# Bioconductor/SparseArray

Hardware: AMD Instinct MI355X
Metric: GNZ/s, SVT crossprod(svt, dense) 1e6x1e4 @1% nnz (higher is better)
Workload: dtype f64

## Files before the change

### sparsearray_amd/csrc/kernels_mult_pbc.hip

```cpp
#include "svt_common.h"

#include <string.h>

#include <mutex>

#include "svt_scan.h"

typedef double d16 __attribute__((ext_vector_type(16)));
typedef double d8 __attribute__((ext_vector_type(8)));

struct svt_dev_pbc {
	int64_t nrow, ncol, nnz, nrec;
	int CBW, WPB, logR;
	int kind;
	int64_t ngroups, nblocks, npanels;
	uint4 *rec;
	int64_t *tile_ptr;
	int *col_has_na;
	int64_t max_leaf_nnz;
	mutable hipStream_t use_s[4];
	mutable int nuse;
	mutable bool use_overflow;
	int device;
};
// ... 997 lines not shown
		bl = Lr % nblocks; kh = u % kt; split = nfull + u / kt;
	}
	const int b = bl + block0;
	const int64_t pa = (int64_t) split * panels_per_split;
	const int64_t pb = pa + panels_per_split < npanels ? pa + panels_per_split : npanels;
	if (pa >= pb)
		return;
	const int k0 = kh * 64;
	const int64_t wv = (int64_t) b * 16 + w;
	const int64_t *__restrict__ tb = tile_ptr + (wv * npanels + pa);

	d16 acc[NV > 2 ? 2 : NV];
	d8 acc8 = 0.0;
#pragma unroll
	for (int i = 0; i < (NV > 2 ? 2 : NV); i++) acc[i] = 0.0;
	const bool partial = (nrow & 127) != 0;

	const int wd = w;
	u32x4 PA;
	u32x16 PB;
	{
		const uint64_t recp = (uint64_t) (uintptr_t) rec + (uint64_t) tb[0] * 12u;
		PA[0] = (uint32_t) recp; PA[1] = (uint32_t) (recp >> 32);
		PA[2] = 0;
		PA[3] = (uint32_t) pa;
		PB[0] = (uint32_t) pb;
		PB[1] = PBC_DMA_BUF;
		PB[2] = (uint32_t) (wd * 4 * PBC_DMA_ROW + PBC_DMA_BUF);
		PB[3] = (uint32_t) (w >> 2);
		PB[4] = partial ? (uint32_t) (npanels - 1) : 0xFFFFFFFFu;
		PB[5] = partial ? (uint32_t) ((128 - (nrow & 127)) * 8) : 0u;
		PB[6] = 0;
		{
			const int chunk = (8192 + nblocks - 1) / nblocks;
			PB[7] = (uint32_t) ((chunk + 1023) / 1024 - 1);
		}
#pragma unroll
		for (int q = 0; q < 4; q++) {
			int kk = k0 + wd * 4 + q;
			if (kk > K - 1) kk = K - 1;
			const uint64_t src = (uint64_t) (uintptr_t) (Y + (int64_t) kk * ldY + pa * 128);
			PB[8 + 2 * q] = (uint32_t) src; PB[9 + 2 * q] = (uint32_t) (src >> 32);
		}
	}
	u32x16 V0 = 0, V1 = 0;
	u32x4 V2 = 0;
	{
		const int lane = tid & 63;
		V0[0] = (uint32_t) lane * PBC_DMA_ROW;
		V0[1] = (uint32_t) lane * 16u;
		V0[2] = (uint32_t) (lane < rt_lines ? lane : rt_lines - 1) * 128u + (uint32_t) rt_ahead;
		V0[11] = (uint32_t) lane * 16u + 1024u;
		const int chunk = (8192 + nblocks - 1) / nblocks;
		const int nit = (chunk + 1023) / 1024;
		int e0 = bl * chunk;
		if (e0 > 8192 - nit * 1024) e0 = 8192 - nit * 1024;
		const int e = e0 + tid;
		V0[3] = (uint32_t) ((e >> 7) * PBC_DMA_ROW + (e & 127) * 8);
		V0[7] = lane == 0 ? (uint32_t) nit :
			lane == 1 ? (partial ? (uint32_t) (npanels - 1) : 0xFFFFFFFFu) :
				    (partial ? (uint32_t) ((128 - (nrow & 127)) * 8) : 0u);
	}
	{
		const int lane = tid & 63;
		const bool clampme = partial && pa == npanels - 1;
#pragma unroll
		for (int q = 0; q < 4; q++) {
			int kk = k0 + wd * 4 + q;
			if (kk > K - 1) kk = K - 1;
			const int64_t r0 = clampme ? nrow - 128 : pa * 128;
			const double *src = Y + (int64_t) kk * ldY + r0 + lane * 2;
			double *dst = ylds + (wd * 4 + q) * 129;
			__builtin_amdgcn_global_load_lds((const __attribute__((address_space(1))) void *) src,
							 (__attribute__((address_space(3))) void *) dst, 16, 0, 0);
		}
		{
			uint32_t sink;
			const char *ptr = (const char *) rec + tb[0] * 12 + (int64_t) (lane < 32 ? lane : 31) * 128;
			asm volatile("global_load_dword %0, %1, off\n\ts_waitcnt vmcnt(0)"
				     : "=v"(sink) : "v"(ptr) : "memory");
		}
	}
#ifdef SVT_TUNING
	if (PROF) t_loop = __builtin_readcyclecounter();
#endif
#if PBC_DMA_YSETS == 2
	u32x8 V3 = 0;
#define PBC_DMA_STATE "+{v[0:15]}"(V0), "+{v[16:31]}"(V1), "+{v[32:39]}"(V3), "+{v[40:43]}"(V2), "+{s[8:11]}"(PA), "+{s[12:27]}"(PB)
#define PBC_ACC0 "+{v[44:75]}"
#define PBC_ACC1 "+{v[76:107]}"
#define PBC_ACC2 "+{v[108:123]}"
// ... 871 lines not shown
```

### sparsearray_amd/csrc/pbc_dma_asm.inc

```
#define PBC_DMA_ROW 1032
#define PBC_DMA_BUF 66048
#define PBC_DMA_BATCH_BYTES 96
#define PBC_DMA_YSETS 2
#define PBC_DMA_ASM_TEXT \
	"v_mov_b32 v10, 0x207\n\t" \
	"s_load_dwordx8 s[28:35], s[8:9], s10\n\t" \
	"s_load_dwordx16 s[36:51], s[8:9], s10 offset:32\n\t" \
	"s_load_dwordx8 s[52:59], s[8:9], s10 offset:96\n\t" \
	"s_load_dwordx16 s[60:75], s[8:9], s10 offset:128\n\t" \
	"s_add_u32 s10, s10, 192\n\t" \
	"s_waitcnt lgkmcnt(0)\n\t" \
	"s_branch 55f\n\t" \
	"20:\n" \
	"s_load_dwordx8 s[76:83], s[8:9], s10\n\t" \
	"s_load_dwordx16 s[84:99], s[8:9], s10 offset:32\n\t" \
	"s_and_b32 vcc_lo, s28, 0xc000\n\t" \
	"s_cbranch_scc1 70f\n\t" \
	"v_add_u32_sdwa v28, s52, v4 dst_sel:DWORD dst_unused:UNUSED_PAD src0_sel:WORD_1 src1_sel:DWORD\n\t" \
	"v_add_u32_sdwa v30, s53, v4 dst_sel:DWORD dst_unused:UNUSED_PAD src0_sel:WORD_1 src1_sel:DWORD\n\t" \
	"v_add_u32_sdwa v32, s54, v4 dst_sel:DWORD dst_unused:UNUSED_PAD src0_sel:WORD_1 src1_sel:DWORD\n\t" \
	"v_add_u32_sdwa v34, s55, v4 dst_sel:DWORD dst_unused:UNUSED_PAD src0_sel:WORD_1 src1_sel:DWORD\n\t" \
	"v_add_u32_sdwa v36, s56, v4 dst_sel:DWORD dst_unused:UNUSED_PAD src0_sel:WORD_1 src1_sel:DWORD\n\t" \
	"v_add_u32_sdwa v38, s57, v4 dst_sel:DWORD dst_unused:UNUSED_PAD src0_sel:WORD_1 src1_sel:DWORD\n\t" \
	"v_add_u32_sdwa v40, s58, v4 dst_sel:DWORD dst_unused:UNUSED_PAD src0_sel:WORD_1 src1_sel:DWORD\n\t" \
	"v_add_u32_sdwa v42, s59, v4 dst_sel:DWORD dst_unused:UNUSED_PAD src0_sel:WORD_1 src1_sel:DWORD\n\t" \
	"ds_read_b64 v[28:29], v28\n\t" \
	"ds_read_b64 v[30:31], v30\n\t" \
	"ds_read_b64 v[32:33], v32\n\t" \
	"ds_read_b64 v[34:35], v34\n\t" \
	"ds_read_b64 v[36:37], v36\n\t" \
	"ds_read_b64 v[38:39], v38\n\t" \
	"ds_read_b64 v[40:41], v40\n\t" \
	"ds_read_b64 v[42:43], v42\n\t" \
	"s_set_gpr_idx_on s28, gpr_idx(SRC2,DST)\n\t" \
	"v_fma_f64 v[44:45], s[36:37], v[12:13], v[44:45]\n\t" \
	"s_set_gpr_idx_idx s29\n\t" \
// ... 225 lines not shown
	"ds_read_b64 v[32:33], v32\n\t" \
	"ds_read_b64 v[34:35], v34\n\t" \
	"ds_read_b64 v[36:37], v36\n\t" \
	"ds_read_b64 v[38:39], v38\n\t" \
	"ds_read_b64 v[40:41], v40\n\t" \
	"ds_read_b64 v[42:43], v42\n\t" \
	"s_set_gpr_idx_on s28, gpr_idx(SRC2,DST)\n\t" \
	"v_fma_f64 v[44:45], s[36:37], v[12:13], v[44:45]\n\t" \
	"s_set_gpr_idx_idx s29\n\t" \
	"v_fma_f64 v[44:45], s[38:39], v[14:15], v[44:45]\n\t" \
	"s_set_gpr_idx_idx s30\n\t" \
	"v_fma_f64 v[44:45], s[40:41], v[16:17], v[44:45]\n\t" \
	"s_set_gpr_idx_idx s31\n\t" \
	"v_fma_f64 v[44:45], s[42:43], v[18:19], v[44:45]\n\t" \
	"s_set_gpr_idx_idx s32\n\t" \
	"v_fma_f64 v[44:45], s[44:45], v[20:21], v[44:45]\n\t" \
	"s_set_gpr_idx_idx s33\n\t" \
	"v_fma_f64 v[44:45], s[46:47], v[22:23], v[44:45]\n\t" \
	"s_set_gpr_idx_idx s34\n\t" \
	"v_fma_f64 v[44:45], s[48:49], v[24:25], v[44:45]\n\t" \
	"s_set_gpr_idx_idx s35\n\t" \
	"v_fma_f64 v[44:45], s[50:51], v[26:27], v[44:45]\n\t" \
	"s_set_gpr_idx_off\n\t" \
	"s_waitcnt lgkmcnt(0)\n\t" \
	"s_cmp_ge_u32 s11, s12\n\t" \
	"s_cbranch_scc1 61f\n\t" \
	"s_cmp_lg_u32 s11, s16\n\t" \
	"s_cbranch_scc1 15f\n\t" \
	"v_subrev_u32 v11, s17, v11\n\t" \
	"15:\n" \
	"s_sub_u32 m0, s14, s13\n\t" \
	"s_nop 0\n\t" \
	"global_load_lds_dwordx4 v11, s[20:21]\n\t" \
	"s_add_u32 m0, m0, 1032\n\t" \
	"s_nop 0\n\t" \
	"global_load_lds_dwordx4 v11, s[22:23]\n\t" \
	"s_add_u32 m0, m0, 1032\n\t" \
	"s_nop 0\n\t" \
	"global_load_lds_dwordx4 v11, s[24:25]\n\t" \
	"s_add_u32 m0, m0, 1032\n\t" \
	"s_nop 0\n\t" \
	"global_load_lds_dwordx4 v11, s[26:27]\n\t" \
	"s_nop 1\n\t" \
	"v_add_u32 v11, 1024, v11\n\t" \
	"v_add_u32 v6, s10, v2\n\t" \
	"global_load_dword v5, v6, s[8:9]\n\t" \
	"61:\n" \
	"s_branch 21b\n\t" \
	"80:\n" \
	"s_bitcmp1_b32 s28, 14\n\t" \
	"s_cbranch_scc0 30f\n\t" \
	"s_cmp_ge_u32 s11, s12\n\t" \
	"s_cbranch_scc1 61f\n\t" \
	"s_cmp_lg_u32 s11, s16\n\t" \
	"s_cbranch_scc1 15f\n\t" \
	"v_subrev_u32 v11, s17, v11\n\t" \
	"15:\n" \
	"s_sub_u32 m0, s14, s13\n\t" \
	"s_nop 0\n\t" \
	"global_load_lds_dwordx4 v11, s[20:21]\n\t" \
	"s_add_u32 m0, m0, 1032\n\t" \
	"s_nop 0\n\t" \
	"global_load_lds_dwordx4 v11, s[22:23]\n\t" \
	"s_add_u32 m0, m0, 1032\n\t" \
	"s_nop 0\n\t" \
	"global_load_lds_dwordx4 v11, s[24:25]\n\t" \
	"s_add_u32 m0, m0, 1032\n\t" \
	"s_nop 0\n\t" \
	"global_load_lds_dwordx4 v11, s[26:27]\n\t" \
	"s_nop 1\n\t" \
	"v_add_u32 v11, 1024, v11\n\t" \
	"v_add_u32 v6, s10, v2\n\t" \
	"global_load_dword v5, v6, s[8:9]\n\t" \
	"61:\n" \
	"s_branch 30f\n\t" \
	"71:\n" \
	"s_bitcmp1_b32 s52, 15\n\t" \
	"s_cbranch_scc1 81f\n\t" \
	"v_add_u32_sdwa v12, s76, v4 dst_sel:DWORD dst_unused:UNUSED_PAD src0_sel:WORD_1 src1_sel:DWORD\n\t" \
	"v_add_u32_sdwa v14, s77, v4 dst_sel:DWORD dst_unused:UNUSED_PAD src0_sel:WORD_1 src1_sel:DWORD\n\t" \
	"v_add_u32_sdwa v16, s78, v4 dst_sel:DWORD dst_unused:UNUSED_PAD src0_sel:WORD_1 src1_sel:DWORD\n\t" \
	"v_add_u32_sdwa v18, s79, v4 dst_sel:DWORD dst_unused:UNUSED_PAD src0_sel:WORD_1 src1_sel:DWORD\n\t" \
	"v_add_u32_sdwa v20, s80, v4 dst_sel:DWORD dst_unused:UNUSED_PAD src0_sel:WORD_1 src1_sel:DWORD\n\t" \
	"v_add_u32_sdwa v22, s81, v4 dst_sel:DWORD dst_unused:UNUSED_PAD src0_sel:WORD_1 src1_sel:DWORD\n\t" \
	"v_add_u32_sdwa v24, s82, v4 dst_sel:DWORD dst_unused:UNUSED_PAD src0_sel:WORD_1 src1_sel:DWORD\n\t" \
	"v_add_u32_sdwa v26, s83, v4 dst_sel:DWORD dst_unused:UNUSED_PAD src0_sel:WORD_1 src1_sel:DWORD\n\t" \
	"ds_read_b64 v[12:13], v12\n\t" \
	"ds_read_b64 v[14:15], v14\n\t" \
	"ds_read_b64 v[16:17], v16\n\t" \
	"ds_read_b64 v[18:19], v18\n\t" \
	"ds_read_b64 v[20:21], v20\n\t" \
	"ds_read_b64 v[22:23], v22\n\t" \
	"ds_read_b64 v[24:25], v24\n\t" \
	"ds_read_b64 v[26:27], v26\n\t" \
	"s_set_gpr_idx_on s52, gpr_idx(SRC2,DST)\n\t" \
	"v_fma_f64 v[44:45], s[60:61], v[28:29], v[44:45]\n\t" \
	"s_set_gpr_idx_idx s53\n\t" \
	"v_fma_f64 v[44:45], s[62:63], v[30:31], v[44:45]\n\t" \
	"s_set_gpr_idx_idx s54\n\t" \
	"v_fma_f64 v[44:45], s[64:65], v[32:33], v[44:45]\n\t" \
	"s_set_gpr_idx_idx s55\n\t" \
	"v_fma_f64 v[44:45], s[66:67], v[34:35], v[44:45]\n\t" \
	"s_set_gpr_idx_idx s56\n\t" \
	"v_fma_f64 v[44:45], s[68:69], v[36:37], v[44:45]\n\t" \
	"s_set_gpr_idx_idx s57\n\t" \
	"v_fma_f64 v[44:45], s[70:71], v[38:39], v[44:45]\n\t" \
	"s_set_gpr_idx_idx s58\n\t" \
	"v_fma_f64 v[44:45], s[72:73], v[40:41], v[44:45]\n\t" \
	"s_set_gpr_idx_idx s59\n\t" \
	"v_fma_f64 v[44:45], s[74:75], v[42:43], v[44:45]\n\t" \
	"s_set_gpr_idx_off\n\t" \
	"s_waitcnt lgkmcnt(0)\n\t" \
	"s_cmp_ge_u32 s11, s12\n\t" \
	"s_cbranch_scc1 61f\n\t" \
	"s_cmp_lg_u32 s11, s16\n\t" \
	"s_cbranch_scc1 15f\n\t" \
	"v_subrev_u32 v11, s17, v11\n\t" \
	"15:\n" \
	"s_sub_u32 m0, s14, s13\n\t" \
	"s_nop 0\n\t" \
	"global_load_lds_dwordx4 v11, s[20:21]\n\t" \
	"s_add_u32 m0, m0, 1032\n\t" \
	"s_nop 0\n\t" \
	"global_load_lds_dwordx4 v11, s[22:23]\n\t" \
	"s_add_u32 m0, m0, 1032\n\t" \
	"s_nop 0\n\t" \
	"global_load_lds_dwordx4 v11, s[24:25]\n\t" \
	"s_add_u32 m0, m0, 1032\n\t" \
	"s_nop 0\n\t" \
	"global_load_lds_dwordx4 v11, s[26:27]\n\t" \
	"s_nop 1\n\t" \
	"v_add_u32 v11, 1024, v11\n\t" \
	"v_add_u32 v6, s10, v2\n\t" \
	"global_load_dword v5, v6, s[8:9]\n\t" \
	"61:\n" \
	"s_branch 22b\n\t" \
	"81:\n" \
	"s_bitcmp1_b32 s52, 14\n\t" \
	"s_cbranch_scc0 31f\n\t" \
	"s_cmp_ge_u32 s11, s12\n\t" \
	"s_cbranch_scc1 61f\n\t" \
	"s_cmp_lg_u32 s11, s16\n\t" \
	"s_cbranch_scc1 15f\n\t" \
	"v_subrev_u32 v11, s17, v11\n\t" \
	"15:\n" \
	"s_sub_u32 m0, s14, s13\n\t" \
	"s_nop 0\n\t" \
	"global_load_lds_dwordx4 v11, s[20:21]\n\t" \
	"s_add_u32 m0, m0, 1032\n\t" \
	"s_nop 0\n\t" \
	"global_load_lds_dwordx4 v11, s[22:23]\n\t" \
	"s_add_u32 m0, m0, 1032\n\t" \
	"s_nop 0\n\t" \
	"global_load_lds_dwordx4 v11, s[24:25]\n\t" \
	"s_add_u32 m0, m0, 1032\n\t" \
	"s_nop 0\n\t" \
	"global_load_lds_dwordx4 v11, s[26:27]\n\t" \
	"s_nop 1\n\t" \
	"v_add_u32 v11, 1024, v11\n\t" \
	"v_add_u32 v6, s10, v2\n\t" \
	"global_load_dword v5, v6, s[8:9]\n\t" \
	"61:\n" \
	"s_branch 31f\n\t" \
	"72:\n" \
	"s_bitcmp1_b32 s76, 15\n\t" \
	"s_cbranch_scc1 82f\n\t" \
	"v_add_u32_sdwa v28, s28, v4 dst_sel:DWORD dst_unused:UNUSED_PAD src0_sel:WORD_1 src1_sel:DWORD\n\t" \
	"v_add_u32_sdwa v30, s29, v4 dst_sel:DWORD dst_unused:UNUSED_PAD src0_sel:WORD_1 src1_sel:DWORD\n\t" \
	"v_add_u32_sdwa v32, s30, v4 dst_sel:DWORD dst_unused:UNUSED_PAD src0_sel:WORD_1 src1_sel:DWORD\n\t" \
	"v_add_u32_sdwa v34, s31, v4 dst_sel:DWORD dst_unused:UNUSED_PAD src0_sel:WORD_1 src1_sel:DWORD\n\t" \
	"v_add_u32_sdwa v36, s32, v4 dst_sel:DWORD dst_unused:UNUSED_PAD src0_sel:WORD_1 src1_sel:DWORD\n\t" \
	"v_add_u32_sdwa v38, s33, v4 dst_sel:DWORD dst_unused:UNUSED_PAD src0_sel:WORD_1 src1_sel:DWORD\n\t" \
	"v_add_u32_sdwa v40, s34, v4 dst_sel:DWORD dst_unused:UNUSED_PAD src0_sel:WORD_1 src1_sel:DWORD\n\t" \
	"v_add_u32_sdwa v42, s35, v4 dst_sel:DWORD dst_unused:UNUSED_PAD src0_sel:WORD_1 src1_sel:DWORD\n\t" \
	"ds_read_b64 v[28:29], v28\n\t" \
	"ds_read_b64 v[30:31], v30\n\t" \
	"ds_read_b64 v[32:33], v32\n\t" \
	"ds_read_b64 v[34:35], v34\n\t" \
	"ds_read_b64 v[36:37], v36\n\t" \
	"ds_read_b64 v[38:39], v38\n\t" \
	"ds_read_b64 v[40:41], v40\n\t" \
	"ds_read_b64 v[42:43], v42\n\t" \
	"s_set_gpr_idx_on s76, gpr_idx(SRC2,DST)\n\t" \
	"v_fma_f64 v[44:45], s[84:85], v[12:13], v[44:45]\n\t" \
	"s_set_gpr_idx_idx s77\n\t" \
	"v_fma_f64 v[44:45], s[86:87], v[14:15], v[44:45]\n\t" \
	"s_set_gpr_idx_idx s78\n\t" \
	"v_fma_f64 v[44:45], s[88:89], v[16:17], v[44:45]\n\t" \
	"s_set_gpr_idx_idx s79\n\t" \
	"v_fma_f64 v[44:45], s[90:91], v[18:19], v[44:45]\n\t" \
	"s_set_gpr_idx_idx s80\n\t" \
	"v_fma_f64 v[44:45], s[92:93], v[20:21], v[44:45]\n\t" \
	"s_set_gpr_idx_idx s81\n\t" \
	"v_fma_f64 v[44:45], s[94:95], v[22:23], v[44:45]\n\t" \
	"s_set_gpr_idx_idx s82\n\t" \
	"v_fma_f64 v[44:45], s[96:97], v[24:25], v[44:45]\n\t" \
	"s_set_gpr_idx_idx s83\n\t" \
	"v_fma_f64 v[44:45], s[98:99], v[26:27], v[44:45]\n\t" \
	"s_set_gpr_idx_off\n\t" \
	"s_waitcnt lgkmcnt(0)\n\t" \
	"s_cmp_ge_u32 s11, s12\n\t" \
	"s_cbranch_scc1 61f\n\t" \
	"s_cmp_lg_u32 s11, s16\n\t" \
	"s_cbranch_scc1 15f\n\t" \
	"v_subrev_u32 v11, s17, v11\n\t" \
	"15:\n" \
	"s_sub_u32 m0, s14, s13\n\t" \
	"s_nop 0\n\t" \
	"global_load_lds_dwordx4 v11, s[20:21]\n\t" \
	"s_add_u32 m0, m0, 1032\n\t" \
	"s_nop 0\n\t" \
	"global_load_lds_dwordx4 v11, s[22:23]\n\t" \
	"s_add_u32 m0, m0, 1032\n\t" \
	"s_nop 0\n\t" \
	"global_load_lds_dwordx4 v11, s[24:25]\n\t" \
	"s_add_u32 m0, m0, 1032\n\t" \
	"s_nop 0\n\t" \
	"global_load_lds_dwordx4 v11, s[26:27]\n\t" \
	"s_nop 1\n\t" \
	"v_add_u32 v11, 1024, v11\n\t" \
	"v_add_u32 v6, s10, v2\n\t" \
	"global_load_dword v5, v6, s[8:9]\n\t" \
	"61:\n" \
	"s_branch 23b\n\t" \
	"82:\n" \
	"s_bitcmp1_b32 s76, 14\n\t" \
	"s_cbranch_scc0 32f\n\t" \
	"s_cmp_ge_u32 s11, s12\n\t" \
	"s_cbranch_scc1 61f\n\t" \
	"s_cmp_lg_u32 s11, s16\n\t" \
	"s_cbranch_scc1 15f\n\t" \
	"v_subrev_u32 v11, s17, v11\n\t" \
	"15:\n" \
	"s_sub_u32 m0, s14, s13\n\t" \
	"s_nop 0\n\t" \
	"global_load_lds_dwordx4 v11, s[20:21]\n\t" \
	"s_add_u32 m0, m0, 1032\n\t" \
	"s_nop 0\n\t" \
	"global_load_lds_dwordx4 v11, s[22:23]\n\t" \
	"s_add_u32 m0, m0, 1032\n\t" \
	"s_nop 0\n\t" \
	"global_load_lds_dwordx4 v11, s[24:25]\n\t" \
	"s_add_u32 m0, m0, 1032\n\t" \
	"s_nop 0\n\t" \
	"global_load_lds_dwordx4 v11, s[26:27]\n\t" \
	"s_nop 1\n\t" \
	"v_add_u32 v11, 1024, v11\n\t" \
	"v_add_u32 v6, s10, v2\n\t" \
	"global_load_dword v5, v6, s[8:9]\n\t" \
	"61:\n" \
	"s_branch 32f\n\t" \
	"73:\n" \
	"s_bitcmp1_b32 s28, 15\n\t" \
	"s_cbranch_scc1 83f\n\t" \
	"v_add_u32_sdwa v12, s52, v4 dst_sel:DWORD dst_unused:UNUSED_PAD src0_sel:WORD_1 src1_sel:DWORD\n\t" \
	"v_add_u32_sdwa v14, s53, v4 dst_sel:DWORD dst_unused:UNUSED_PAD src0_sel:WORD_1 src1_sel:DWORD\n\t" \
	"v_add_u32_sdwa v16, s54, v4 dst_sel:DWORD dst_unused:UNUSED_PAD src0_sel:WORD_1 src1_sel:DWORD\n\t" \
	"v_add_u32_sdwa v18, s55, v4 dst_sel:DWORD dst_unused:UNUSED_PAD src0_sel:WORD_1 src1_sel:DWORD\n\t" \
	"v_add_u32_sdwa v20, s56, v4 dst_sel:DWORD dst_unused:UNUSED_PAD src0_sel:WORD_1 src1_sel:DWORD\n\t" \
	"v_add_u32_sdwa v22, s57, v4 dst_sel:DWORD dst_unused:UNUSED_PAD src0_sel:WORD_1 src1_sel:DWORD\n\t" \
	"v_add_u32_sdwa v24, s58, v4 dst_sel:DWORD dst_unused:UNUSED_PAD src0_sel:WORD_1 src1_sel:DWORD\n\t" \
	"v_add_u32_sdwa v26, s59, v4 dst_sel:DWORD dst_unused:UNUSED_PAD src0_sel:WORD_1 src1_sel:DWORD\n\t" \
	"ds_read_b64 v[12:13], v12\n\t" \
	"ds_read_b64 v[14:15], v14\n\t" \
	"ds_read_b64 v[16:17], v16\n\t" \
	"ds_read_b64 v[18:19], v18\n\t" \
	"ds_read_b64 v[20:21], v20\n\t" \
	"ds_read_b64 v[22:23], v22\n\t" \
	"ds_read_b64 v[24:25], v24\n\t" \
	"ds_read_b64 v[26:27], v26\n\t" \
	"s_set_gpr_idx_on s28, gpr_idx(SRC2,DST)\n\t" \
	"v_fma_f64 v[44:45], s[36:37], v[28:29], v[44:45]\n\t" \
	"s_set_gpr_idx_idx s29\n\t" \
	"v_fma_f64 v[44:45], s[38:39], v[30:31], v[44:45]\n\t" \
	"s_set_gpr_idx_idx s30\n\t" \
	"v_fma_f64 v[44:45], s[40:41], v[32:33], v[44:45]\n\t" \
	"s_set_gpr_idx_idx s31\n\t" \
	"v_fma_f64 v[44:45], s[42:43], v[34:35], v[44:45]\n\t" \
	"s_set_gpr_idx_idx s32\n\t" \
	"v_fma_f64 v[44:45], s[44:45], v[36:37], v[44:45]\n\t" \
	"s_set_gpr_idx_idx s33\n\t" \
	"v_fma_f64 v[44:45], s[46:47], v[38:39], v[44:45]\n\t" \
	"s_set_gpr_idx_idx s34\n\t" \
	"v_fma_f64 v[44:45], s[48:49], v[40:41], v[44:45]\n\t" \
	"s_set_gpr_idx_idx s35\n\t" \
	"v_fma_f64 v[44:45], s[50:51], v[42:43], v[44:45]\n\t" \
	"s_set_gpr_idx_off\n\t" \
	"s_waitcnt lgkmcnt(0)\n\t" \
	"s_cmp_ge_u32 s11, s12\n\t" \
	"s_cbranch_scc1 61f\n\t" \
	"s_cmp_lg_u32 s11, s16\n\t" \
	"s_cbranch_scc1 15f\n\t" \
	"v_subrev_u32 v11, s17, v11\n\t" \
	"15:\n" \
	"s_sub_u32 m0, s14, s13\n\t" \
	"s_nop 0\n\t" \
	"global_load_lds_dwordx4 v11, s[20:21]\n\t" \
	"s_add_u32 m0, m0, 1032\n\t" \
	"s_nop 0\n\t" \
	"global_load_lds_dwordx4 v11, s[22:23]\n\t" \
	"s_add_u32 m0, m0, 1032\n\t" \
	"s_nop 0\n\t" \
	"global_load_lds_dwordx4 v11, s[24:25]\n\t" \
	"s_add_u32 m0, m0, 1032\n\t" \
	"s_nop 0\n\t" \
	"global_load_lds_dwordx4 v11, s[26:27]\n\t" \
	"s_nop 1\n\t" \
	"v_add_u32 v11, 1024, v11\n\t" \
	"v_add_u32 v6, s10, v2\n\t" \
	"global_load_dword v5, v6, s[8:9]\n\t" \
	"61:\n" \
	"s_branch 24b\n\t" \
	"83:\n" \
	"s_bitcmp1_b32 s28, 14\n\t" \
	"s_cbranch_scc0 33f\n\t" \
	"s_cmp_ge_u32 s11, s12\n\t" \
	"s_cbranch_scc1 61f\n\t" \
	"s_cmp_lg_u32 s11, s16\n\t" \
	"s_cbranch_scc1 15f\n\t" \
	"v_subrev_u32 v11, s17, v11\n\t" \
	"15:\n" \
	"s_sub_u32 m0, s14, s13\n\t" \
	"s_nop 0\n\t" \
	"global_load_lds_dwordx4 v11, s[20:21]\n\t" \
	"s_add_u32 m0, m0, 1032\n\t" \
	"s_nop 0\n\t" \
	"global_load_lds_dwordx4 v11, s[22:23]\n\t" \
	"s_add_u32 m0, m0, 1032\n\t" \
	"s_nop 0\n\t" \
	"global_load_lds_dwordx4 v11, s[24:25]\n\t" \
	"s_add_u32 m0, m0, 1032\n\t" \
	"s_nop 0\n\t" \
	"global_load_lds_dwordx4 v11, s[26:27]\n\t" \
	"s_nop 1\n\t" \
	"v_add_u32 v11, 1024, v11\n\t" \
	"v_add_u32 v6, s10, v2\n\t" \
	"global_load_dword v5, v6, s[8:9]\n\t" \
	"61:\n" \
	"s_branch 33f\n\t" \
	"74:\n" \
	"s_bitcmp1_b32 s52, 15\n\t" \
	"s_cbranch_scc1 84f\n\t" \
	"v_add_u32_sdwa v28, s76, v4 dst_sel:DWORD dst_unused:UNUSED_PAD src0_sel:WORD_1 src1_sel:DWORD\n\t" \
	"v_add_u32_sdwa v30, s77, v4 dst_sel:DWORD dst_unused:UNUSED_PAD src0_sel:WORD_1 src1_sel:DWORD\n\t" \
	"v_add_u32_sdwa v32, s78, v4 dst_sel:DWORD dst_unused:UNUSED_PAD src0_sel:WORD_1 src1_sel:DWORD\n\t" \
	"v_add_u32_sdwa v34, s79, v4 dst_sel:DWORD dst_unused:UNUSED_PAD src0_sel:WORD_1 src1_sel:DWORD\n\t" \
	"v_add_u32_sdwa v36, s80, v4 dst_sel:DWORD dst_unused:UNUSED_PAD src0_sel:WORD_1 src1_sel:DWORD\n\t" \
	"v_add_u32_sdwa v38, s81, v4 dst_sel:DWORD dst_unused:UNUSED_PAD src0_sel:WORD_1 src1_sel:DWORD\n\t" \
	"v_add_u32_sdwa v40, s82, v4 dst_sel:DWORD dst_unused:UNUSED_PAD src0_sel:WORD_1 src1_sel:DWORD\n\t" \
	"v_add_u32_sdwa v42, s83, v4 dst_sel:DWORD dst_unused:UNUSED_PAD src0_sel:WORD_1 src1_sel:DWORD\n\t" \
	"ds_read_b64 v[28:29], v28\n\t" \
	"ds_read_b64 v[30:31], v30\n\t" \
	"ds_read_b64 v[32:33], v32\n\t" \
	"ds_read_b64 v[34:35], v34\n\t" \
	"ds_read_b64 v[36:37], v36\n\t" \
	"ds_read_b64 v[38:39], v38\n\t" \
	"ds_read_b64 v[40:41], v40\n\t" \
	"ds_read_b64 v[42:43], v42\n\t" \
	"s_set_gpr_idx_on s52, gpr_idx(SRC2,DST)\n\t" \
	"v_fma_f64 v[44:45], s[60:61], v[12:13], v[44:45]\n\t" \
	"s_set_gpr_idx_idx s53\n\t" \
	"v_fma_f64 v[44:45], s[62:63], v[14:15], v[44:45]\n\t" \
	"s_set_gpr_idx_idx s54\n\t" \
	"v_fma_f64 v[44:45], s[64:65], v[16:17], v[44:45]\n\t" \
	"s_set_gpr_idx_idx s55\n\t" \
	"v_fma_f64 v[44:45], s[66:67], v[18:19], v[44:45]\n\t" \
	"s_set_gpr_idx_idx s56\n\t" \
	"v_fma_f64 v[44:45], s[68:69], v[20:21], v[44:45]\n\t" \
	"s_set_gpr_idx_idx s57\n\t" \
	"v_fma_f64 v[44:45], s[70:71], v[22:23], v[44:45]\n\t" \
	"s_set_gpr_idx_idx s58\n\t" \
	"v_fma_f64 v[44:45], s[72:73], v[24:25], v[44:45]\n\t" \
	"s_set_gpr_idx_idx s59\n\t" \
	"v_fma_f64 v[44:45], s[74:75], v[26:27], v[44:45]\n\t" \
	"s_set_gpr_idx_off\n\t" \
	"s_waitcnt lgkmcnt(0)\n\t" \
	"s_cmp_ge_u32 s11, s12\n\t" \
	"s_cbranch_scc1 61f\n\t" \
	"s_cmp_lg_u32 s11, s16\n\t" \
	"s_cbranch_scc1 15f\n\t" \
	"v_subrev_u32 v11, s17, v11\n\t" \
	"15:\n" \
	"s_sub_u32 m0, s14, s13\n\t" \
	"s_nop 0\n\t" \
	"global_load_lds_dwordx4 v11, s[20:21]\n\t" \
	"s_add_u32 m0, m0, 1032\n\t" \
	"s_nop 0\n\t" \
	"global_load_lds_dwordx4 v11, s[22:23]\n\t" \
	"s_add_u32 m0, m0, 1032\n\t" \
	"s_nop 0\n\t" \
	"global_load_lds_dwordx4 v11, s[24:25]\n\t" \
	"s_add_u32 m0, m0, 1032\n\t" \
	"s_nop 0\n\t" \
	"global_load_lds_dwordx4 v11, s[26:27]\n\t" \
	"s_nop 1\n\t" \
	"v_add_u32 v11, 1024, v11\n\t" \
	"v_add_u32 v6, s10, v2\n\t" \
	"global_load_dword v5, v6, s[8:9]\n\t" \
	"61:\n" \
	"s_branch 25b\n\t" \
	"84:\n" \
	"s_bitcmp1_b32 s52, 14\n\t" \
	"s_cbranch_scc0 34f\n\t" \
	"s_cmp_ge_u32 s11, s12\n\t" \
	"s_cbranch_scc1 61f\n\t" \
	"s_cmp_lg_u32 s11, s16\n\t" \
	"s_cbranch_scc1 15f\n\t" \
	"v_subrev_u32 v11, s17, v11\n\t" \
	"15:\n" \
	"s_sub_u32 m0, s14, s13\n\t" \
	"s_nop 0\n\t" \
	"global_load_lds_dwordx4 v11, s[20:21]\n\t" \
	"s_add_u32 m0, m0, 1032\n\t" \
	"s_nop 0\n\t" \
	"global_load_lds_dwordx4 v11, s[22:23]\n\t" \
	"s_add_u32 m0, m0, 1032\n\t" \
	"s_nop 0\n\t" \
	"global_load_lds_dwordx4 v11, s[24:25]\n\t" \
	"s_add_u32 m0, m0, 1032\n\t" \
	"s_nop 0\n\t" \
	"global_load_lds_dwordx4 v11, s[26:27]\n\t" \
	"s_nop 1\n\t" \
	"v_add_u32 v11, 1024, v11\n\t" \
	"v_add_u32 v6, s10, v2\n\t" \
	"global_load_dword v5, v6, s[8:9]\n\t" \
	"61:\n" \
	"s_branch 34f\n\t" \
	"75:\n" \
	"s_bitcmp1_b32 s76, 15\n\t" \
	"s_cbranch_scc1 85f\n\t" \
	"v_add_u32_sdwa v12, s28, v4 dst_sel:DWORD dst_unused:UNUSED_PAD src0_sel:WORD_1 src1_sel:DWORD\n\t" \
	"v_add_u32_sdwa v14, s29, v4 dst_sel:DWORD dst_unused:UNUSED_PAD src0_sel:WORD_1 src1_sel:DWORD\n\t" \
	"v_add_u32_sdwa v16, s30, v4 dst_sel:DWORD dst_unused:UNUSED_PAD src0_sel:WORD_1 src1_sel:DWORD\n\t" \
	"v_add_u32_sdwa v18, s31, v4 dst_sel:DWORD dst_unused:UNUSED_PAD src0_sel:WORD_1 src1_sel:DWORD\n\t" \
	"v_add_u32_sdwa v20, s32, v4 dst_sel:DWORD dst_unused:UNUSED_PAD src0_sel:WORD_1 src1_sel:DWORD\n\t" \
	"v_add_u32_sdwa v22, s33, v4 dst_sel:DWORD dst_unused:UNUSED_PAD src0_sel:WORD_1 src1_sel:DWORD\n\t" \
	"v_add_u32_sdwa v24, s34, v4 dst_sel:DWORD dst_unused:UNUSED_PAD src0_sel:WORD_1 src1_sel:DWORD\n\t" \
	"v_add_u32_sdwa v26, s35, v4 dst_sel:DWORD dst_unused:UNUSED_PAD src0_sel:WORD_1 src1_sel:DWORD\n\t" \
	"ds_read_b64 v[12:13], v12\n\t" \
	"ds_read_b64 v[14:15], v14\n\t" \
	"ds_read_b64 v[16:17], v16\n\t" \
	"ds_read_b64 v[18:19], v18\n\t" \
	"ds_read_b64 v[20:21], v20\n\t" \
	"ds_read_b64 v[22:23], v22\n\t" \
	"ds_read_b64 v[24:25], v24\n\t" \
	"ds_read_b64 v[26:27], v26\n\t" \
	"s_set_gpr_idx_on s76, gpr_idx(SRC2,DST)\n\t" \
	"v_fma_f64 v[44:45], s[84:85], v[28:29], v[44:45]\n\t" \
	"s_set_gpr_idx_idx s77\n\t" \
	"v_fma_f64 v[44:45], s[86:87], v[30:31], v[44:45]\n\t" \
	"s_set_gpr_idx_idx s78\n\t" \
	"v_fma_f64 v[44:45], s[88:89], v[32:33], v[44:45]\n\t" \
	"s_set_gpr_idx_idx s79\n\t" \
	"v_fma_f64 v[44:45], s[90:91], v[34:35], v[44:45]\n\t" \
	"s_set_gpr_idx_idx s80\n\t" \
	"v_fma_f64 v[44:45], s[92:93], v[36:37], v[44:45]\n\t" \
	"s_set_gpr_idx_idx s81\n\t" \
	"v_fma_f64 v[44:45], s[94:95], v[38:39], v[44:45]\n\t" \
	"s_set_gpr_idx_idx s82\n\t" \
	"v_fma_f64 v[44:45], s[96:97], v[40:41], v[44:45]\n\t" \
	"s_set_gpr_idx_idx s83\n\t" \
	"v_fma_f64 v[44:45], s[98:99], v[42:43], v[44:45]\n\t" \
	"s_set_gpr_idx_off\n\t" \
	"s_waitcnt lgkmcnt(0)\n\t" \
	"s_cmp_ge_u32 s11, s12\n\t" \
	"s_cbranch_scc1 61f\n\t" \
	"s_cmp_lg_u32 s11, s16\n\t" \
	"s_cbranch_scc1 15f\n\t" \
	"v_subrev_u32 v11, s17, v11\n\t" \
	"15:\n" \
	"s_sub_u32 m0, s14, s13\n\t" \
	"s_nop 0\n\t" \
	"global_load_lds_dwordx4 v11, s[20:21]\n\t" \
	"s_add_u32 m0, m0, 1032\n\t" \
	"s_nop 0\n\t" \
	"global_load_lds_dwordx4 v11, s[22:23]\n\t" \
	"s_add_u32 m0, m0, 1032\n\t" \
	"s_nop 0\n\t" \
	"global_load_lds_dwordx4 v11, s[24:25]\n\t" \
	"s_add_u32 m0, m0, 1032\n\t" \
	"s_nop 0\n\t" \
	"global_load_lds_dwordx4 v11, s[26:27]\n\t" \
	"s_nop 1\n\t" \
	"v_add_u32 v11, 1024, v11\n\t" \
	"v_add_u32 v6, s10, v2\n\t" \
	"global_load_dword v5, v6, s[8:9]\n\t" \
	"61:\n" \
	"s_branch 20b\n\t" \
	"85:\n" \
	"s_bitcmp1_b32 s76, 14\n\t" \
	"s_cbranch_scc0 35f\n\t" \
	"s_cmp_ge_u32 s11, s12\n\t" \
	"s_cbranch_scc1 61f\n\t" \
	"s_cmp_lg_u32 s11, s16\n\t" \
	"s_cbranch_scc1 15f\n\t" \
	"v_subrev_u32 v11, s17, v11\n\t" \
	"15:\n" \
	"s_sub_u32 m0, s14, s13\n\t" \
	"s_nop 0\n\t" \
	"global_load_lds_dwordx4 v11, s[20:21]\n\t" \
	"s_add_u32 m0, m0, 1032\n\t" \
	"s_nop 0\n\t" \
	"global_load_lds_dwordx4 v11, s[22:23]\n\t" \
	"s_add_u32 m0, m0, 1032\n\t" \
	"s_nop 0\n\t" \
	"global_load_lds_dwordx4 v11, s[24:25]\n\t" \
	"s_add_u32 m0, m0, 1032\n\t" \
	"s_nop 0\n\t" \
	"global_load_lds_dwordx4 v11, s[26:27]\n\t" \
	"s_nop 1\n\t" \
	"v_add_u32 v11, 1024, v11\n\t" \
	"v_add_u32 v6, s10, v2\n\t" \
	"global_load_dword v5, v6, s[8:9]\n\t" \
	"61:\n" \
	"s_branch 35f\n\t" \
	"30:\n" \
	"s_cmp_ge_u32 s11, s12\n\t" \
	"s_cbranch_scc1 40f\n\t" \
	"s_xor_b32 s13, s13, 66048\n\t" \
	"v_add_u32 v4, s13, v0\n\t" \
	"s_cmp_lg_u32 s11, s16\n\t" \
	"s_cbranch_scc1 16f\n\t" \
	"v_add_u32 v4, s17, v4\n\t" \
	"16:\n" \
	"s_add_u32 s11, s11, 1\n\t" \
	"v_add_u32 v6, s13, v3\n\t" \
	"v_add_u32_sdwa v28, s52, v4 dst_sel:DWORD dst_unused:UNUSED_PAD src0_sel:WORD_1 src1_sel:DWORD\n\t" \
	"v_add_u32_sdwa v30, s53, v4 dst_sel:DWORD dst_unused:UNUSED_PAD src0_sel:WORD_1 src1_sel:DWORD\n\t" \
	"v_add_u32_sdwa v32, s54, v4 dst_sel:DWORD dst_unused:UNUSED_PAD src0_sel:WORD_1 src1_sel:DWORD\n\t" \
	"v_add_u32_sdwa v34, s55, v4 dst_sel:DWORD dst_unused:UNUSED_PAD src0_sel:WORD_1 src1_sel:DWORD\n\t" \
	"v_add_u32_sdwa v36, s56, v4 dst_sel:DWORD dst_unused:UNUSED_PAD src0_sel:WORD_1 src1_sel:DWORD\n\t" \
	"v_add_u32_sdwa v38, s57, v4 dst_sel:DWORD dst_unused:UNUSED_PAD src0_sel:WORD_1 src1_sel:DWORD\n\t" \
	"v_add_u32_sdwa v40, s58, v4 dst_sel:DWORD dst_unused:UNUSED_PAD src0_sel:WORD_1 src1_sel:DWORD\n\t" \
	"v_add_u32_sdwa v42, s59, v4 dst_sel:DWORD dst_unused:UNUSED_PAD src0_sel:WORD_1 src1_sel:DWORD\n\t" \
	"s_waitcnt vmcnt(1)\n\t" \
	"s_barrier\n\t" \
	"ds_read_b64 v[28:29], v28\n\t" \
	"ds_read_b64 v[30:31], v30\n\t" \
	"ds_read_b64 v[32:33], v32\n\t" \
	"ds_read_b64 v[34:35], v34\n\t" \
	"ds_read_b64 v[36:37], v36\n\t" \
	"ds_read_b64 v[38:39], v38\n\t" \
	"ds_read_b64 v[40:41], v40\n\t" \
	"ds_read_b64 v[42:43], v42\n\t" \
	"s_set_gpr_idx_on s28, gpr_idx(SRC2,DST)\n\t" \
	"v_fma_f64 v[44:45], s[36:37], v[12:13], v[44:45]\n\t" \
	"s_set_gpr_idx_idx s29\n\t" \
	"v_fma_f64 v[44:45], s[38:39], v[14:15], v[44:45]\n\t" \
	"s_set_gpr_idx_idx s30\n\t" \
	"v_fma_f64 v[44:45], s[40:41], v[16:17], v[44:45]\n\t" \
	"s_set_gpr_idx_idx s31\n\t" \
	"v_fma_f64 v[44:45], s[42:43], v[18:19], v[44:45]\n\t" \
	"s_set_gpr_idx_idx s32\n\t" \
	"v_fma_f64 v[44:45], s[44:45], v[20:21], v[44:45]\n\t" \
	"s_set_gpr_idx_idx s33\n\t" \
	"v_fma_f64 v[44:45], s[46:47], v[22:23], v[44:45]\n\t" \
	"s_set_gpr_idx_idx s34\n\t" \
	"v_fma_f64 v[44:45], s[48:49], v[24:25], v[44:45]\n\t" \
	"s_set_gpr_idx_idx s35\n\t" \
	"v_fma_f64 v[44:45], s[50:51], v[26:27], v[44:45]\n\t" \
	"s_set_gpr_idx_off\n\t" \
	"s_mov_b32 m0, s19\n\t" \
	"12:\n" \
	"ds_read_b64 v[8:9], v6\n\t" \
	"v_add_u32 v6, 8256, v6\n\t" \
	"s_waitcnt lgkmcnt(0)\n\t" \
	"v_cmp_class_f64 vcc, v[8:9], v10\n\t" \
	"s_or_b32 s18, s18, vcc_lo\n\t" \
	"s_or_b32 s18, s18, vcc_hi\n\t" \
	"s_sub_u32 m0, m0, 1\n\t" \
	"s_cbranch_scc0 12b\n\t" \
	"s_branch 21b\n\t" \
	"31:\n" \
	"s_cmp_ge_u32 s11, s12\n\t" \
	"s_cbranch_scc1 41f\n\t" \
	"s_xor_b32 s13, s13, 66048\n\t" \
	"v_add_u32 v4, s13, v0\n\t" \
	"s_cmp_lg_u32 s11, s16\n\t" \
	"s_cbranch_scc1 16f\n\t" \
	"v_add_u32 v4, s17, v4\n\t" \
	"16:\n" \
	"s_add_u32 s11, s11, 1\n\t" \
	"v_add_u32 v6, s13, v3\n\t" \
	"v_add_u32_sdwa v12, s76, v4 dst_sel:DWORD dst_unused:UNUSED_PAD src0_sel:WORD_1 src1_sel:DWORD\n\t" \
	"v_add_u32_sdwa v14, s77, v4 dst_sel:DWORD dst_unused:UNUSED_PAD src0_sel:WORD_1 src1_sel:DWORD\n\t" \
	"v_add_u32_sdwa v16, s78, v4 dst_sel:DWORD dst_unused:UNUSED_PAD src0_sel:WORD_1 src1_sel:DWORD\n\t" \
	"v_add_u32_sdwa v18, s79, v4 dst_sel:DWORD dst_unused:UNUSED_PAD src0_sel:WORD_1 src1_sel:DWORD\n\t" \
	"v_add_u32_sdwa v20, s80, v4 dst_sel:DWORD dst_unused:UNUSED_PAD src0_sel:WORD_1 src1_sel:DWORD\n\t" \
	"v_add_u32_sdwa v22, s81, v4 dst_sel:DWORD dst_unused:UNUSED_PAD src0_sel:WORD_1 src1_sel:DWORD\n\t" \
	"v_add_u32_sdwa v24, s82, v4 dst_sel:DWORD dst_unused:UNUSED_PAD src0_sel:WORD_1 src1_sel:DWORD\n\t" \
	"v_add_u32_sdwa v26, s83, v4 dst_sel:DWORD dst_unused:UNUSED_PAD src0_sel:WORD_1 src1_sel:DWORD\n\t" \
	"s_waitcnt vmcnt(1)\n\t" \
	"s_barrier\n\t" \
	"ds_read_b64 v[12:13], v12\n\t" \
	"ds_read_b64 v[14:15], v14\n\t" \
	"ds_read_b64 v[16:17], v16\n\t" \
	"ds_read_b64 v[18:19], v18\n\t" \
	"ds_read_b64 v[20:21], v20\n\t" \
	"ds_read_b64 v[22:23], v22\n\t" \
	"ds_read_b64 v[24:25], v24\n\t" \
	"ds_read_b64 v[26:27], v26\n\t" \
	"s_set_gpr_idx_on s52, gpr_idx(SRC2,DST)\n\t" \
	"v_fma_f64 v[44:45], s[60:61], v[28:29], v[44:45]\n\t" \
	"s_set_gpr_idx_idx s53\n\t" \
	"v_fma_f64 v[44:45], s[62:63], v[30:31], v[44:45]\n\t" \
	"s_set_gpr_idx_idx s54\n\t" \
	"v_fma_f64 v[44:45], s[64:65], v[32:33], v[44:45]\n\t" \
	"s_set_gpr_idx_idx s55\n\t" \
	"v_fma_f64 v[44:45], s[66:67], v[34:35], v[44:45]\n\t" \
	"s_set_gpr_idx_idx s56\n\t" \
	"v_fma_f64 v[44:45], s[68:69], v[36:37], v[44:45]\n\t" \
	"s_set_gpr_idx_idx s57\n\t" \
	"v_fma_f64 v[44:45], s[70:71], v[38:39], v[44:45]\n\t" \
	"s_set_gpr_idx_idx s58\n\t" \
	"v_fma_f64 v[44:45], s[72:73], v[40:41], v[44:45]\n\t" \
	"s_set_gpr_idx_idx s59\n\t" \
	"v_fma_f64 v[44:45], s[74:75], v[42:43], v[44:45]\n\t" \
	"s_set_gpr_idx_off\n\t" \
	"s_mov_b32 m0, s19\n\t" \
	"12:\n" \
	"ds_read_b64 v[8:9], v6\n\t" \
	"v_add_u32 v6, 8256, v6\n\t" \
	"s_waitcnt lgkmcnt(0)\n\t" \
	"v_cmp_class_f64 vcc, v[8:9], v10\n\t" \
	"s_or_b32 s18, s18, vcc_lo\n\t" \
	"s_or_b32 s18, s18, vcc_hi\n\t" \
	"s_sub_u32 m0, m0, 1\n\t" \
	"s_cbranch_scc0 12b\n\t" \
	"s_branch 22b\n\t" \
	"32:\n" \
	"s_cmp_ge_u32 s11, s12\n\t" \
	"s_cbranch_scc1 42f\n\t" \
	"s_xor_b32 s13, s13, 66048\n\t" \
	"v_add_u32 v4, s13, v0\n\t" \
	"s_cmp_lg_u32 s11, s16\n\t" \
	"s_cbranch_scc1 16f\n\t" \
	"v_add_u32 v4, s17, v4\n\t" \
	"16:\n" \
	"s_add_u32 s11, s11, 1\n\t" \
	"v_add_u32 v6, s13, v3\n\t" \
	"v_add_u32_sdwa v28, s28, v4 dst_sel:DWORD dst_unused:UNUSED_PAD src0_sel:WORD_1 src1_sel:DWORD\n\t" \
	"v_add_u32_sdwa v30, s29, v4 dst_sel:DWORD dst_unused:UNUSED_PAD src0_sel:WORD_1 src1_sel:DWORD\n\t" \
	"v_add_u32_sdwa v32, s30, v4 dst_sel:DWORD dst_unused:UNUSED_PAD src0_sel:WORD_1 src1_sel:DWORD\n\t" \
	"v_add_u32_sdwa v34, s31, v4 dst_sel:DWORD dst_unused:UNUSED_PAD src0_sel:WORD_1 src1_sel:DWORD\n\t" \
	"v_add_u32_sdwa v36, s32, v4 dst_sel:DWORD dst_unused:UNUSED_PAD src0_sel:WORD_1 src1_sel:DWORD\n\t" \
	"v_add_u32_sdwa v38, s33, v4 dst_sel:DWORD dst_unused:UNUSED_PAD src0_sel:WORD_1 src1_sel:DWORD\n\t" \
	"v_add_u32_sdwa v40, s34, v4 dst_sel:DWORD dst_unused:UNUSED_PAD src0_sel:WORD_1 src1_sel:DWORD\n\t" \
	"v_add_u32_sdwa v42, s35, v4 dst_sel:DWORD dst_unused:UNUSED_PAD src0_sel:WORD_1 src1_sel:DWORD\n\t" \
	"s_waitcnt vmcnt(1)\n\t" \
	"s_barrier\n\t" \
	"ds_read_b64 v[28:29], v28\n\t" \
	"ds_read_b64 v[30:31], v30\n\t" \
	"ds_read_b64 v[32:33], v32\n\t" \
	"ds_read_b64 v[34:35], v34\n\t" \
	"ds_read_b64 v[36:37], v36\n\t" \
	"ds_read_b64 v[38:39], v38\n\t" \
	"ds_read_b64 v[40:41], v40\n\t" \
	"ds_read_b64 v[42:43], v42\n\t" \
	"s_set_gpr_idx_on s76, gpr_idx(SRC2,DST)\n\t" \
	"v_fma_f64 v[44:45], s[84:85], v[12:13], v[44:45]\n\t" \
	"s_set_gpr_idx_idx s77\n\t" \
	"v_fma_f64 v[44:45], s[86:87], v[14:15], v[44:45]\n\t" \
	"s_set_gpr_idx_idx s78\n\t" \
	"v_fma_f64 v[44:45], s[88:89], v[16:17], v[44:45]\n\t" \
	"s_set_gpr_idx_idx s79\n\t" \
	"v_fma_f64 v[44:45], s[90:91], v[18:19], v[44:45]\n\t" \
	"s_set_gpr_idx_idx s80\n\t" \
	"v_fma_f64 v[44:45], s[92:93], v[20:21], v[44:45]\n\t" \
	"s_set_gpr_idx_idx s81\n\t" \
	"v_fma_f64 v[44:45], s[94:95], v[22:23], v[44:45]\n\t" \
	"s_set_gpr_idx_idx s82\n\t" \
	"v_fma_f64 v[44:45], s[96:97], v[24:25], v[44:45]\n\t" \
	"s_set_gpr_idx_idx s83\n\t" \
	"v_fma_f64 v[44:45], s[98:99], v[26:27], v[44:45]\n\t" \
	"s_set_gpr_idx_off\n\t" \
	"s_mov_b32 m0, s19\n\t" \
	"12:\n" \
	"ds_read_b64 v[8:9], v6\n\t" \
	"v_add_u32 v6, 8256, v6\n\t" \
	"s_waitcnt lgkmcnt(0)\n\t" \
	"v_cmp_class_f64 vcc, v[8:9], v10\n\t" \
	"s_or_b32 s18, s18, vcc_lo\n\t" \
	"s_or_b32 s18, s18, vcc_hi\n\t" \
	"s_sub_u32 m0, m0, 1\n\t" \
	"s_cbranch_scc0 12b\n\t" \
	"s_branch 23b\n\t" \
	"33:\n" \
	"s_cmp_ge_u32 s11, s12\n\t" \
	"s_cbranch_scc1 43f\n\t" \
	"s_xor_b32 s13, s13, 66048\n\t" \
	"v_add_u32 v4, s13, v0\n\t" \
	"s_cmp_lg_u32 s11, s16\n\t" \
	"s_cbranch_scc1 16f\n\t" \
	"v_add_u32 v4, s17, v4\n\t" \
	"16:\n" \
	"s_add_u32 s11, s11, 1\n\t" \
	"v_add_u32 v6, s13, v3\n\t" \
	"v_add_u32_sdwa v12, s52, v4 dst_sel:DWORD dst_unused:UNUSED_PAD src0_sel:WORD_1 src1_sel:DWORD\n\t" \
	"v_add_u32_sdwa v14, s53, v4 dst_sel:DWORD dst_unused:UNUSED_PAD src0_sel:WORD_1 src1_sel:DWORD\n\t" \
	"v_add_u32_sdwa v16, s54, v4 dst_sel:DWORD dst_unused:UNUSED_PAD src0_sel:WORD_1 src1_sel:DWORD\n\t" \
	"v_add_u32_sdwa v18, s55, v4 dst_sel:DWORD dst_unused:UNUSED_PAD src0_sel:WORD_1 src1_sel:DWORD\n\t" \
	"v_add_u32_sdwa v20, s56, v4 dst_sel:DWORD dst_unused:UNUSED_PAD src0_sel:WORD_1 src1_sel:DWORD\n\t" \
	"v_add_u32_sdwa v22, s57, v4 dst_sel:DWORD dst_unused:UNUSED_PAD src0_sel:WORD_1 src1_sel:DWORD\n\t" \
	"v_add_u32_sdwa v24, s58, v4 dst_sel:DWORD dst_unused:UNUSED_PAD src0_sel:WORD_1 src1_sel:DWORD\n\t" \
	"v_add_u32_sdwa v26, s59, v4 dst_sel:DWORD dst_unused:UNUSED_PAD src0_sel:WORD_1 src1_sel:DWORD\n\t" \
	"s_waitcnt vmcnt(1)\n\t" \
	"s_barrier\n\t" \
	"ds_read_b64 v[12:13], v12\n\t" \
	"ds_read_b64 v[14:15], v14\n\t" \
	"ds_read_b64 v[16:17], v16\n\t" \
	"ds_read_b64 v[18:19], v18\n\t" \
	"ds_read_b64 v[20:21], v20\n\t" \
	"ds_read_b64 v[22:23], v22\n\t" \
	"ds_read_b64 v[24:25], v24\n\t" \
	"ds_read_b64 v[26:27], v26\n\t" \
	"s_set_gpr_idx_on s28, gpr_idx(SRC2,DST)\n\t" \
	"v_fma_f64 v[44:45], s[36:37], v[28:29], v[44:45]\n\t" \
	"s_set_gpr_idx_idx s29\n\t" \
	"v_fma_f64 v[44:45], s[38:39], v[30:31], v[44:45]\n\t" \
	"s_set_gpr_idx_idx s30\n\t" \
	"v_fma_f64 v[44:45], s[40:41], v[32:33], v[44:45]\n\t" \
	"s_set_gpr_idx_idx s31\n\t" \
	"v_fma_f64 v[44:45], s[42:43], v[34:35], v[44:45]\n\t" \
	"s_set_gpr_idx_idx s32\n\t" \
	"v_fma_f64 v[44:45], s[44:45], v[36:37], v[44:45]\n\t" \
	"s_set_gpr_idx_idx s33\n\t" \
	"v_fma_f64 v[44:45], s[46:47], v[38:39], v[44:45]\n\t" \
	"s_set_gpr_idx_idx s34\n\t" \
	"v_fma_f64 v[44:45], s[48:49], v[40:41], v[44:45]\n\t" \
	"s_set_gpr_idx_idx s35\n\t" \
	"v_fma_f64 v[44:45], s[50:51], v[42:43], v[44:45]\n\t" \
	"s_set_gpr_idx_off\n\t" \
	"s_mov_b32 m0, s19\n\t" \
	"12:\n" \
	"ds_read_b64 v[8:9], v6\n\t" \
	"v_add_u32 v6, 8256, v6\n\t" \
	"s_waitcnt lgkmcnt(0)\n\t" \
	"v_cmp_class_f64 vcc, v[8:9], v10\n\t" \
	"s_or_b32 s18, s18, vcc_lo\n\t" \
	"s_or_b32 s18, s18, vcc_hi\n\t" \
	"s_sub_u32 m0, m0, 1\n\t" \
	"s_cbranch_scc0 12b\n\t" \
	"s_branch 24b\n\t" \
	"34:\n" \
	"s_cmp_ge_u32 s11, s12\n\t" \
	"s_cbranch_scc1 44f\n\t" \
	"s_xor_b32 s13, s13, 66048\n\t" \
	"v_add_u32 v4, s13, v0\n\t" \
	"s_cmp_lg_u32 s11, s16\n\t" \
	"s_cbranch_scc1 16f\n\t" \
	"v_add_u32 v4, s17, v4\n\t" \
	"16:\n" \
	"s_add_u32 s11, s11, 1\n\t" \
	"v_add_u32 v6, s13, v3\n\t" \
	"v_add_u32_sdwa v28, s76, v4 dst_sel:DWORD dst_unused:UNUSED_PAD src0_sel:WORD_1 src1_sel:DWORD\n\t" \
	"v_add_u32_sdwa v30, s77, v4 dst_sel:DWORD dst_unused:UNUSED_PAD src0_sel:WORD_1 src1_sel:DWORD\n\t" \
	"v_add_u32_sdwa v32, s78, v4 dst_sel:DWORD dst_unused:UNUSED_PAD src0_sel:WORD_1 src1_sel:DWORD\n\t" \
	"v_add_u32_sdwa v34, s79, v4 dst_sel:DWORD dst_unused:UNUSED_PAD src0_sel:WORD_1 src1_sel:DWORD\n\t" \
	"v_add_u32_sdwa v36, s80, v4 dst_sel:DWORD dst_unused:UNUSED_PAD src0_sel:WORD_1 src1_sel:DWORD\n\t" \
	"v_add_u32_sdwa v38, s81, v4 dst_sel:DWORD dst_unused:UNUSED_PAD src0_sel:WORD_1 src1_sel:DWORD\n\t" \
	"v_add_u32_sdwa v40, s82, v4 dst_sel:DWORD dst_unused:UNUSED_PAD src0_sel:WORD_1 src1_sel:DWORD\n\t" \
	"v_add_u32_sdwa v42, s83, v4 dst_sel:DWORD dst_unused:UNUSED_PAD src0_sel:WORD_1 src1_sel:DWORD\n\t" \
	"s_waitcnt vmcnt(1)\n\t" \
	"s_barrier\n\t" \
	"ds_read_b64 v[28:29], v28\n\t" \
	"ds_read_b64 v[30:31], v30\n\t" \
	"ds_read_b64 v[32:33], v32\n\t" \
	"ds_read_b64 v[34:35], v34\n\t" \
	"ds_read_b64 v[36:37], v36\n\t" \
	"ds_read_b64 v[38:39], v38\n\t" \
	"ds_read_b64 v[40:41], v40\n\t" \
	"ds_read_b64 v[42:43], v42\n\t" \
	"s_set_gpr_idx_on s52, gpr_idx(SRC2,DST)\n\t" \
	"v_fma_f64 v[44:45], s[60:61], v[12:13], v[44:45]\n\t" \
	"s_set_gpr_idx_idx s53\n\t" \
	"v_fma_f64 v[44:45], s[62:63], v[14:15], v[44:45]\n\t" \
	"s_set_gpr_idx_idx s54\n\t" \
	"v_fma_f64 v[44:45], s[64:65], v[16:17], v[44:45]\n\t" \
	"s_set_gpr_idx_idx s55\n\t" \
	"v_fma_f64 v[44:45], s[66:67], v[18:19], v[44:45]\n\t" \
	"s_set_gpr_idx_idx s56\n\t" \
	"v_fma_f64 v[44:45], s[68:69], v[20:21], v[44:45]\n\t" \
	"s_set_gpr_idx_idx s57\n\t" \
	"v_fma_f64 v[44:45], s[70:71], v[22:23], v[44:45]\n\t" \
	"s_set_gpr_idx_idx s58\n\t" \
	"v_fma_f64 v[44:45], s[72:73], v[24:25], v[44:45]\n\t" \
	"s_set_gpr_idx_idx s59\n\t" \
	"v_fma_f64 v[44:45], s[74:75], v[26:27], v[44:45]\n\t" \
	"s_set_gpr_idx_off\n\t" \
	"s_mov_b32 m0, s19\n\t" \
	"12:\n" \
	"ds_read_b64 v[8:9], v6\n\t" \
	"v_add_u32 v6, 8256, v6\n\t" \
	"s_waitcnt lgkmcnt(0)\n\t" \
	"v_cmp_class_f64 vcc, v[8:9], v10\n\t" \
	"s_or_b32 s18, s18, vcc_lo\n\t" \
	"s_or_b32 s18, s18, vcc_hi\n\t" \
	"s_sub_u32 m0, m0, 1\n\t" \
	"s_cbranch_scc0 12b\n\t" \
	"s_branch 25b\n\t" \
	"35:\n" \
	"s_cmp_ge_u32 s11, s12\n\t" \
	"s_cbranch_scc1 45f\n\t" \
	"s_xor_b32 s13, s13, 66048\n\t" \
	"v_add_u32 v4, s13, v0\n\t" \
	"s_cmp_lg_u32 s11, s16\n\t" \
	"s_cbranch_scc1 16f\n\t" \
	"v_add_u32 v4, s17, v4\n\t" \
	"16:\n" \
	"s_add_u32 s11, s11, 1\n\t" \
	"v_add_u32 v6, s13, v3\n\t" \
	"v_add_u32_sdwa v12, s28, v4 dst_sel:DWORD dst_unused:UNUSED_PAD src0_sel:WORD_1 src1_sel:DWORD\n\t" \
	"v_add_u32_sdwa v14, s29, v4 dst_sel:DWORD dst_unused:UNUSED_PAD src0_sel:WORD_1 src1_sel:DWORD\n\t" \
	"v_add_u32_sdwa v16, s30, v4 dst_sel:DWORD dst_unused:UNUSED_PAD src0_sel:WORD_1 src1_sel:DWORD\n\t" \
	"v_add_u32_sdwa v18, s31, v4 dst_sel:DWORD dst_unused:UNUSED_PAD src0_sel:WORD_1 src1_sel:DWORD\n\t" \
	"v_add_u32_sdwa v20, s32, v4 dst_sel:DWORD dst_unused:UNUSED_PAD src0_sel:WORD_1 src1_sel:DWORD\n\t" \
	"v_add_u32_sdwa v22, s33, v4 dst_sel:DWORD dst_unused:UNUSED_PAD src0_sel:WORD_1 src1_sel:DWORD\n\t" \
	"v_add_u32_sdwa v24, s34, v4 dst_sel:DWORD dst_unused:UNUSED_PAD src0_sel:WORD_1 src1_sel:DWORD\n\t" \
	"v_add_u32_sdwa v26, s35, v4 dst_sel:DWORD dst_unused:UNUSED_PAD src0_sel:WORD_1 src1_sel:DWORD\n\t" \
	"s_waitcnt vmcnt(1)\n\t" \
	"s_barrier\n\t" \
	"ds_read_b64 v[12:13], v12\n\t" \
	"ds_read_b64 v[14:15], v14\n\t" \
	"ds_read_b64 v[16:17], v16\n\t" \
	"ds_read_b64 v[18:19], v18\n\t" \
	"ds_read_b64 v[20:21], v20\n\t" \
	"ds_read_b64 v[22:23], v22\n\t" \
	"ds_read_b64 v[24:25], v24\n\t" \
	"ds_read_b64 v[26:27], v26\n\t" \
	"s_set_gpr_idx_on s76, gpr_idx(SRC2,DST)\n\t" \
	"v_fma_f64 v[44:45], s[84:85], v[28:29], v[44:45]\n\t" \
	"s_set_gpr_idx_idx s77\n\t" \
	"v_fma_f64 v[44:45], s[86:87], v[30:31], v[44:45]\n\t" \
	"s_set_gpr_idx_idx s78\n\t" \
	"v_fma_f64 v[44:45], s[88:89], v[32:33], v[44:45]\n\t" \
	"s_set_gpr_idx_idx s79\n\t" \
	"v_fma_f64 v[44:45], s[90:91], v[34:35], v[44:45]\n\t" \
	"s_set_gpr_idx_idx s80\n\t" \
	"v_fma_f64 v[44:45], s[92:93], v[36:37], v[44:45]\n\t" \
	"s_set_gpr_idx_idx s81\n\t" \
	"v_fma_f64 v[44:45], s[94:95], v[38:39], v[44:45]\n\t" \
	"s_set_gpr_idx_idx s82\n\t" \
	"v_fma_f64 v[44:45], s[96:97], v[40:41], v[44:45]\n\t" \
	"s_set_gpr_idx_idx s83\n\t" \
	"v_fma_f64 v[44:45], s[98:99], v[42:43], v[44:45]\n\t" \
	"s_set_gpr_idx_off\n\t" \
	"s_mov_b32 m0, s19\n\t" \
	"12:\n" \
	"ds_read_b64 v[8:9], v6\n\t" \
	"v_add_u32 v6, 8256, v6\n\t" \
	"s_waitcnt lgkmcnt(0)\n\t" \
	"v_cmp_class_f64 vcc, v[8:9], v10\n\t" \
	"s_or_b32 s18, s18, vcc_lo\n\t" \
	"s_or_b32 s18, s18, vcc_hi\n\t" \
	"s_sub_u32 m0, m0, 1\n\t" \
	"s_cbranch_scc0 12b\n\t" \
	"s_branch 20b\n\t" \
	"55:\n" \
	"s_cmp_ge_u32 s11, s12\n\t" \
	"s_cbranch_scc1 90f\n\t" \
	"s_xor_b32 s13, s13, 66048\n\t" \
	"v_add_u32 v4, s13, v0\n\t" \
	"s_cmp_lg_u32 s11, s16\n\t" \
	"s_cbranch_scc1 16f\n\t" \
	"v_add_u32 v4, s17, v4\n\t" \
	"16:\n" \
	"s_add_u32 s11, s11, 1\n\t" \
	"v_add_u32 v6, s13, v3\n\t" \
	"v_add_u32_sdwa v12, s28, v4 dst_sel:DWORD dst_unused:UNUSED_PAD src0_sel:WORD_1 src1_sel:DWORD\n\t" \
	"v_add_u32_sdwa v14, s29, v4 dst_sel:DWORD dst_unused:UNUSED_PAD src0_sel:WORD_1 src1_sel:DWORD\n\t" \
	"v_add_u32_sdwa v16, s30, v4 dst_sel:DWORD dst_unused:UNUSED_PAD src0_sel:WORD_1 src1_sel:DWORD\n\t" \
	"v_add_u32_sdwa v18, s31, v4 dst_sel:DWORD dst_unused:UNUSED_PAD src0_sel:WORD_1 src1_sel:DWORD\n\t" \
	"v_add_u32_sdwa v20, s32, v4 dst_sel:DWORD dst_unused:UNUSED_PAD src0_sel:WORD_1 src1_sel:DWORD\n\t" \
	"v_add_u32_sdwa v22, s33, v4 dst_sel:DWORD dst_unused:UNUSED_PAD src0_sel:WORD_1 src1_sel:DWORD\n\t" \
	"v_add_u32_sdwa v24, s34, v4 dst_sel:DWORD dst_unused:UNUSED_PAD src0_sel:WORD_1 src1_sel:DWORD\n\t" \
	"v_add_u32_sdwa v26, s35, v4 dst_sel:DWORD dst_unused:UNUSED_PAD src0_sel:WORD_1 src1_sel:DWORD\n\t" \
	"s_waitcnt vmcnt(1)\n\t" \
	"s_barrier\n\t" \
	"ds_read_b64 v[12:13], v12\n\t" \
	"ds_read_b64 v[14:15], v14\n\t" \
	"ds_read_b64 v[16:17], v16\n\t" \
	"ds_read_b64 v[18:19], v18\n\t" \
	"ds_read_b64 v[20:21], v20\n\t" \
	"ds_read_b64 v[22:23], v22\n\t" \
	"ds_read_b64 v[24:25], v24\n\t" \
	"ds_read_b64 v[26:27], v26\n\t" \
	"s_mov_b32 m0, s19\n\t" \
	"12:\n" \
	"ds_read_b64 v[8:9], v6\n\t" \
	"v_add_u32 v6, 8256, v6\n\t" \
	"s_waitcnt lgkmcnt(0)\n\t" \
	"v_cmp_class_f64 vcc, v[8:9], v10\n\t" \
	"s_or_b32 s18, s18, vcc_lo\n\t" \
	"s_or_b32 s18, s18, vcc_hi\n\t" \
	"s_sub_u32 m0, m0, 1\n\t" \
	"s_cbranch_scc0 12b\n\t" \
	"s_branch 20b\n\t" \
	"40:\n" \
	"s_set_gpr_idx_on s28, gpr_idx(SRC2,DST)\n\t" \
	"v_fma_f64 v[44:45], s[36:37], v[12:13], v[44:45]\n\t" \
	"s_set_gpr_idx_idx s29\n\t" \
	"v_fma_f64 v[44:45], s[38:39], v[14:15], v[44:45]\n\t" \
	"s_set_gpr_idx_idx s30\n\t" \
	"v_fma_f64 v[44:45], s[40:41], v[16:17], v[44:45]\n\t" \
	"s_set_gpr_idx_idx s31\n\t" \
	"v_fma_f64 v[44:45], s[42:43], v[18:19], v[44:45]\n\t" \
	"s_set_gpr_idx_idx s32\n\t" \
	"v_fma_f64 v[44:45], s[44:45], v[20:21], v[44:45]\n\t" \
	"s_set_gpr_idx_idx s33\n\t" \
	"v_fma_f64 v[44:45], s[46:47], v[22:23], v[44:45]\n\t" \
	"s_set_gpr_idx_idx s34\n\t" \
	"v_fma_f64 v[44:45], s[48:49], v[24:25], v[44:45]\n\t" \
	"s_set_gpr_idx_idx s35\n\t" \
	"v_fma_f64 v[44:45], s[50:51], v[26:27], v[44:45]\n\t" \
	"s_set_gpr_idx_off\n\t" \
	"s_branch 90f\n\t" \
	"41:\n" \
	"s_set_gpr_idx_on s52, gpr_idx(SRC2,DST)\n\t" \
	"v_fma_f64 v[44:45], s[60:61], v[28:29], v[44:45]\n\t" \
	"s_set_gpr_idx_idx s53\n\t" \
	"v_fma_f64 v[44:45], s[62:63], v[30:31], v[44:45]\n\t" \
	"s_set_gpr_idx_idx s54\n\t" \
	"v_fma_f64 v[44:45], s[64:65], v[32:33], v[44:45]\n\t" \
	"s_set_gpr_idx_idx s55\n\t" \
	"v_fma_f64 v[44:45], s[66:67], v[34:35], v[44:45]\n\t" \
	"s_set_gpr_idx_idx s56\n\t" \
	"v_fma_f64 v[44:45], s[68:69], v[36:37], v[44:45]\n\t" \
	"s_set_gpr_idx_idx s57\n\t" \
	"v_fma_f64 v[44:45], s[70:71], v[38:39], v[44:45]\n\t" \
// ... 352 lines not shown
	"ds_read_b64 v[42:43], v42\n\t" \
	"s_set_gpr_idx_on s28, gpr_idx(SRC2,DST)\n\t" \
	"v_fma_f64 v[44:45], s[36:37], v[12:13], v[44:45]\n\t" \
	"s_set_gpr_idx_idx s29\n\t" \
	"v_fma_f64 v[44:45], s[38:39], v[14:15], v[44:45]\n\t" \
	"s_set_gpr_idx_idx s30\n\t" \
	"v_fma_f64 v[44:45], s[40:41], v[16:17], v[44:45]\n\t" \
	"s_set_gpr_idx_idx s31\n\t" \
	"v_fma_f64 v[44:45], s[42:43], v[18:19], v[44:45]\n\t" \
	"s_set_gpr_idx_idx s32\n\t" \
	"v_fma_f64 v[44:45], s[44:45], v[20:21], v[44:45]\n\t" \
	"s_set_gpr_idx_idx s33\n\t" \
	"v_fma_f64 v[44:45], s[46:47], v[22:23], v[44:45]\n\t" \
	"s_set_gpr_idx_idx s34\n\t" \
	"v_fma_f64 v[44:45], s[48:49], v[24:25], v[44:45]\n\t" \
	"s_set_gpr_idx_idx s35\n\t" \
	"v_fma_f64 v[44:45], s[50:51], v[26:27], v[44:45]\n\t" \
	"s_set_gpr_idx_off\n\t" \
	"s_waitcnt lgkmcnt(0)\n\t" \
	"s_memtime s[100:101]\n\t" \
	"s_waitcnt lgkmcnt(0)\n\t" \
	"v_sub_u32 v127, s100, v126\n\t" \
	"v_add_u32 v123, v127, v123\n\t" \
	"v_mov_b32 v126, s100\n\t" \
	"s_cmp_ge_u32 s11, s12\n\t" \
	"s_cbranch_scc1 61f\n\t" \
	"s_cmp_lg_u32 s11, s16\n\t" \
	"s_cbranch_scc1 15f\n\t" \
	"v_subrev_u32 v11, s17, v11\n\t" \
	"15:\n" \
	"s_sub_u32 m0, s14, s13\n\t" \
	"s_nop 0\n\t" \
	"global_load_lds_dwordx4 v11, s[20:21]\n\t" \
	"s_add_u32 m0, m0, 1032\n\t" \
	"s_nop 0\n\t" \
	"global_load_lds_dwordx4 v11, s[22:23]\n\t" \
	"s_add_u32 m0, m0, 1032\n\t" \
	"s_nop 0\n\t" \
	"global_load_lds_dwordx4 v11, s[24:25]\n\t" \
	"s_add_u32 m0, m0, 1032\n\t" \
	"s_nop 0\n\t" \
	"global_load_lds_dwordx4 v11, s[26:27]\n\t" \
	"s_nop 1\n\t" \
	"v_add_u32 v11, 1024, v11\n\t" \
	"v_add_u32 v6, s10, v2\n\t" \
	"global_load_dword v5, v6, s[8:9]\n\t" \
	"61:\n" \
	"s_memtime s[100:101]\n\t" \
	"s_waitcnt lgkmcnt(0)\n\t" \
	"v_sub_u32 v127, s100, v126\n\t" \
	"v_add_u32 v119, v127, v119\n\t" \
	"v_mov_b32 v126, s100\n\t" \
	"s_branch 21b\n\t" \
	"80:\n" \
	"s_bitcmp1_b32 s28, 14\n\t" \
	"s_cbranch_scc0 30f\n\t" \
	"s_memtime s[100:101]\n\t" \
	"s_waitcnt lgkmcnt(0)\n\t" \
	"v_sub_u32 v127, s100, v126\n\t" \
	"v_add_u32 v123, v127, v123\n\t" \
	"v_mov_b32 v126, s100\n\t" \
	"s_cmp_ge_u32 s11, s12\n\t" \
	"s_cbranch_scc1 61f\n\t" \
	"s_cmp_lg_u32 s11, s16\n\t" \
	"s_cbranch_scc1 15f\n\t" \
	"v_subrev_u32 v11, s17, v11\n\t" \
	"15:\n" \
	"s_sub_u32 m0, s14, s13\n\t" \
	"s_nop 0\n\t" \
	"global_load_lds_dwordx4 v11, s[20:21]\n\t" \
	"s_add_u32 m0, m0, 1032\n\t" \
	"s_nop 0\n\t" \
	"global_load_lds_dwordx4 v11, s[22:23]\n\t" \
	"s_add_u32 m0, m0, 1032\n\t" \
	"s_nop 0\n\t" \
	"global_load_lds_dwordx4 v11, s[24:25]\n\t" \
	"s_add_u32 m0, m0, 1032\n\t" \
	"s_nop 0\n\t" \
	"global_load_lds_dwordx4 v11, s[26:27]\n\t" \
	"s_nop 1\n\t" \
	"v_add_u32 v11, 1024, v11\n\t" \
	"v_add_u32 v6, s10, v2\n\t" \
	"global_load_dword v5, v6, s[8:9]\n\t" \
	"61:\n" \
	"s_memtime s[100:101]\n\t" \
	"s_waitcnt lgkmcnt(0)\n\t" \
	"v_sub_u32 v127, s100, v126\n\t" \
	"v_add_u32 v119, v127, v119\n\t" \
	"v_mov_b32 v126, s100\n\t" \
	"s_branch 30f\n\t" \
	"71:\n" \
	"s_bitcmp1_b32 s52, 15\n\t" \
	"s_cbranch_scc1 81f\n\t" \
	"v_add_u32_sdwa v12, s76, v4 dst_sel:DWORD dst_unused:UNUSED_PAD src0_sel:WORD_1 src1_sel:DWORD\n\t" \
	"v_add_u32_sdwa v14, s77, v4 dst_sel:DWORD dst_unused:UNUSED_PAD src0_sel:WORD_1 src1_sel:DWORD\n\t" \
	"v_add_u32_sdwa v16, s78, v4 dst_sel:DWORD dst_unused:UNUSED_PAD src0_sel:WORD_1 src1_sel:DWORD\n\t" \
	"v_add_u32_sdwa v18, s79, v4 dst_sel:DWORD dst_unused:UNUSED_PAD src0_sel:WORD_1 src1_sel:DWORD\n\t" \
	"v_add_u32_sdwa v20, s80, v4 dst_sel:DWORD dst_unused:UNUSED_PAD src0_sel:WORD_1 src1_sel:DWORD\n\t" \
	"v_add_u32_sdwa v22, s81, v4 dst_sel:DWORD dst_unused:UNUSED_PAD src0_sel:WORD_1 src1_sel:DWORD\n\t" \
	"v_add_u32_sdwa v24, s82, v4 dst_sel:DWORD dst_unused:UNUSED_PAD src0_sel:WORD_1 src1_sel:DWORD\n\t" \
	"v_add_u32_sdwa v26, s83, v4 dst_sel:DWORD dst_unused:UNUSED_PAD src0_sel:WORD_1 src1_sel:DWORD\n\t" \
	"ds_read_b64 v[12:13], v12\n\t" \
	"ds_read_b64 v[14:15], v14\n\t" \
	"ds_read_b64 v[16:17], v16\n\t" \
	"ds_read_b64 v[18:19], v18\n\t" \
	"ds_read_b64 v[20:21], v20\n\t" \
	"ds_read_b64 v[22:23], v22\n\t" \
	"ds_read_b64 v[24:25], v24\n\t" \
	"ds_read_b64 v[26:27], v26\n\t" \
	"s_set_gpr_idx_on s52, gpr_idx(SRC2,DST)\n\t" \
	"v_fma_f64 v[44:45], s[60:61], v[28:29], v[44:45]\n\t" \
	"s_set_gpr_idx_idx s53\n\t" \
	"v_fma_f64 v[44:45], s[62:63], v[30:31], v[44:45]\n\t" \
	"s_set_gpr_idx_idx s54\n\t" \
	"v_fma_f64 v[44:45], s[64:65], v[32:33], v[44:45]\n\t" \
	"s_set_gpr_idx_idx s55\n\t" \
	"v_fma_f64 v[44:45], s[66:67], v[34:35], v[44:45]\n\t" \
	"s_set_gpr_idx_idx s56\n\t" \
	"v_fma_f64 v[44:45], s[68:69], v[36:37], v[44:45]\n\t" \
	"s_set_gpr_idx_idx s57\n\t" \
	"v_fma_f64 v[44:45], s[70:71], v[38:39], v[44:45]\n\t" \
	"s_set_gpr_idx_idx s58\n\t" \
	"v_fma_f64 v[44:45], s[72:73], v[40:41], v[44:45]\n\t" \
	"s_set_gpr_idx_idx s59\n\t" \
	"v_fma_f64 v[44:45], s[74:75], v[42:43], v[44:45]\n\t" \
	"s_set_gpr_idx_off\n\t" \
	"s_waitcnt lgkmcnt(0)\n\t" \
	"s_memtime s[100:101]\n\t" \
	"s_waitcnt lgkmcnt(0)\n\t" \
	"v_sub_u32 v127, s100, v126\n\t" \
	"v_add_u32 v123, v127, v123\n\t" \
	"v_mov_b32 v126, s100\n\t" \
	"s_cmp_ge_u32 s11, s12\n\t" \
	"s_cbranch_scc1 61f\n\t" \
	"s_cmp_lg_u32 s11, s16\n\t" \
	"s_cbranch_scc1 15f\n\t" \
	"v_subrev_u32 v11, s17, v11\n\t" \
	"15:\n" \
	"s_sub_u32 m0, s14, s13\n\t" \
	"s_nop 0\n\t" \
	"global_load_lds_dwordx4 v11, s[20:21]\n\t" \
	"s_add_u32 m0, m0, 1032\n\t" \
	"s_nop 0\n\t" \
	"global_load_lds_dwordx4 v11, s[22:23]\n\t" \
	"s_add_u32 m0, m0, 1032\n\t" \
	"s_nop 0\n\t" \
	"global_load_lds_dwordx4 v11, s[24:25]\n\t" \
	"s_add_u32 m0, m0, 1032\n\t" \
	"s_nop 0\n\t" \
	"global_load_lds_dwordx4 v11, s[26:27]\n\t" \
	"s_nop 1\n\t" \
	"v_add_u32 v11, 1024, v11\n\t" \
	"v_add_u32 v6, s10, v2\n\t" \
	"global_load_dword v5, v6, s[8:9]\n\t" \
	"61:\n" \
	"s_memtime s[100:101]\n\t" \
	"s_waitcnt lgkmcnt(0)\n\t" \
	"v_sub_u32 v127, s100, v126\n\t" \
	"v_add_u32 v119, v127, v119\n\t" \
	"v_mov_b32 v126, s100\n\t" \
	"s_branch 22b\n\t" \
	"81:\n" \
	"s_bitcmp1_b32 s52, 14\n\t" \
	"s_cbranch_scc0 31f\n\t" \
	"s_memtime s[100:101]\n\t" \
	"s_waitcnt lgkmcnt(0)\n\t" \
	"v_sub_u32 v127, s100, v126\n\t" \
	"v_add_u32 v123, v127, v123\n\t" \
	"v_mov_b32 v126, s100\n\t" \
	"s_cmp_ge_u32 s11, s12\n\t" \
	"s_cbranch_scc1 61f\n\t" \
	"s_cmp_lg_u32 s11, s16\n\t" \
	"s_cbranch_scc1 15f\n\t" \
	"v_subrev_u32 v11, s17, v11\n\t" \
	"15:\n" \
	"s_sub_u32 m0, s14, s13\n\t" \
	"s_nop 0\n\t" \
	"global_load_lds_dwordx4 v11, s[20:21]\n\t" \
	"s_add_u32 m0, m0, 1032\n\t" \
	"s_nop 0\n\t" \
	"global_load_lds_dwordx4 v11, s[22:23]\n\t" \
	"s_add_u32 m0, m0, 1032\n\t" \
	"s_nop 0\n\t" \
	"global_load_lds_dwordx4 v11, s[24:25]\n\t" \
	"s_add_u32 m0, m0, 1032\n\t" \
	"s_nop 0\n\t" \
	"global_load_lds_dwordx4 v11, s[26:27]\n\t" \
	"s_nop 1\n\t" \
	"v_add_u32 v11, 1024, v11\n\t" \
	"v_add_u32 v6, s10, v2\n\t" \
	"global_load_dword v5, v6, s[8:9]\n\t" \
	"61:\n" \
	"s_memtime s[100:101]\n\t" \
	"s_waitcnt lgkmcnt(0)\n\t" \
	"v_sub_u32 v127, s100, v126\n\t" \
	"v_add_u32 v119, v127, v119\n\t" \
	"v_mov_b32 v126, s100\n\t" \
	"s_branch 31f\n\t" \
	"72:\n" \
	"s_bitcmp1_b32 s76, 15\n\t" \
	"s_cbranch_scc1 82f\n\t" \
	"v_add_u32_sdwa v28, s28, v4 dst_sel:DWORD dst_unused:UNUSED_PAD src0_sel:WORD_1 src1_sel:DWORD\n\t" \
	"v_add_u32_sdwa v30, s29, v4 dst_sel:DWORD dst_unused:UNUSED_PAD src0_sel:WORD_1 src1_sel:DWORD\n\t" \
	"v_add_u32_sdwa v32, s30, v4 dst_sel:DWORD dst_unused:UNUSED_PAD src0_sel:WORD_1 src1_sel:DWORD\n\t" \
	"v_add_u32_sdwa v34, s31, v4 dst_sel:DWORD dst_unused:UNUSED_PAD src0_sel:WORD_1 src1_sel:DWORD\n\t" \
	"v_add_u32_sdwa v36, s32, v4 dst_sel:DWORD dst_unused:UNUSED_PAD src0_sel:WORD_1 src1_sel:DWORD\n\t" \
	"v_add_u32_sdwa v38, s33, v4 dst_sel:DWORD dst_unused:UNUSED_PAD src0_sel:WORD_1 src1_sel:DWORD\n\t" \
	"v_add_u32_sdwa v40, s34, v4 dst_sel:DWORD dst_unused:UNUSED_PAD src0_sel:WORD_1 src1_sel:DWORD\n\t" \
	"v_add_u32_sdwa v42, s35, v4 dst_sel:DWORD dst_unused:UNUSED_PAD src0_sel:WORD_1 src1_sel:DWORD\n\t" \
	"ds_read_b64 v[28:29], v28\n\t" \
	"ds_read_b64 v[30:31], v30\n\t" \
	"ds_read_b64 v[32:33], v32\n\t" \
	"ds_read_b64 v[34:35], v34\n\t" \
	"ds_read_b64 v[36:37], v36\n\t" \
	"ds_read_b64 v[38:39], v38\n\t" \
	"ds_read_b64 v[40:41], v40\n\t" \
	"ds_read_b64 v[42:43], v42\n\t" \
	"s_set_gpr_idx_on s76, gpr_idx(SRC2,DST)\n\t" \
	"v_fma_f64 v[44:45], s[84:85], v[12:13], v[44:45]\n\t" \
	"s_set_gpr_idx_idx s77\n\t" \
	"v_fma_f64 v[44:45], s[86:87], v[14:15], v[44:45]\n\t" \
	"s_set_gpr_idx_idx s78\n\t" \
	"v_fma_f64 v[44:45], s[88:89], v[16:17], v[44:45]\n\t" \
	"s_set_gpr_idx_idx s79\n\t" \
	"v_fma_f64 v[44:45], s[90:91], v[18:19], v[44:45]\n\t" \
	"s_set_gpr_idx_idx s80\n\t" \
	"v_fma_f64 v[44:45], s[92:93], v[20:21], v[44:45]\n\t" \
	"s_set_gpr_idx_idx s81\n\t" \
	"v_fma_f64 v[44:45], s[94:95], v[22:23], v[44:45]\n\t" \
	"s_set_gpr_idx_idx s82\n\t" \
	"v_fma_f64 v[44:45], s[96:97], v[24:25], v[44:45]\n\t" \
	"s_set_gpr_idx_idx s83\n\t" \
	"v_fma_f64 v[44:45], s[98:99], v[26:27], v[44:45]\n\t" \
	"s_set_gpr_idx_off\n\t" \
	"s_waitcnt lgkmcnt(0)\n\t" \
	"s_memtime s[100:101]\n\t" \
	"s_waitcnt lgkmcnt(0)\n\t" \
	"v_sub_u32 v127, s100, v126\n\t" \
	"v_add_u32 v123, v127, v123\n\t" \
	"v_mov_b32 v126, s100\n\t" \
	"s_cmp_ge_u32 s11, s12\n\t" \
	"s_cbranch_scc1 61f\n\t" \
	"s_cmp_lg_u32 s11, s16\n\t" \
	"s_cbranch_scc1 15f\n\t" \
	"v_subrev_u32 v11, s17, v11\n\t" \
	"15:\n" \
	"s_sub_u32 m0, s14, s13\n\t" \
	"s_nop 0\n\t" \
	"global_load_lds_dwordx4 v11, s[20:21]\n\t" \
	"s_add_u32 m0, m0, 1032\n\t" \
	"s_nop 0\n\t" \
	"global_load_lds_dwordx4 v11, s[22:23]\n\t" \
	"s_add_u32 m0, m0, 1032\n\t" \
	"s_nop 0\n\t" \
	"global_load_lds_dwordx4 v11, s[24:25]\n\t" \
	"s_add_u32 m0, m0, 1032\n\t" \
	"s_nop 0\n\t" \
	"global_load_lds_dwordx4 v11, s[26:27]\n\t" \
	"s_nop 1\n\t" \
	"v_add_u32 v11, 1024, v11\n\t" \
	"v_add_u32 v6, s10, v2\n\t" \
	"global_load_dword v5, v6, s[8:9]\n\t" \
	"61:\n" \
	"s_memtime s[100:101]\n\t" \
	"s_waitcnt lgkmcnt(0)\n\t" \
	"v_sub_u32 v127, s100, v126\n\t" \
	"v_add_u32 v119, v127, v119\n\t" \
	"v_mov_b32 v126, s100\n\t" \
	"s_branch 23b\n\t" \
	"82:\n" \
	"s_bitcmp1_b32 s76, 14\n\t" \
	"s_cbranch_scc0 32f\n\t" \
	"s_memtime s[100:101]\n\t" \
	"s_waitcnt lgkmcnt(0)\n\t" \
	"v_sub_u32 v127, s100, v126\n\t" \
	"v_add_u32 v123, v127, v123\n\t" \
	"v_mov_b32 v126, s100\n\t" \
	"s_cmp_ge_u32 s11, s12\n\t" \
	"s_cbranch_scc1 61f\n\t" \
	"s_cmp_lg_u32 s11, s16\n\t" \
	"s_cbranch_scc1 15f\n\t" \
	"v_subrev_u32 v11, s17, v11\n\t" \
	"15:\n" \
	"s_sub_u32 m0, s14, s13\n\t" \
	"s_nop 0\n\t" \
	"global_load_lds_dwordx4 v11, s[20:21]\n\t" \
	"s_add_u32 m0, m0, 1032\n\t" \
	"s_nop 0\n\t" \
	"global_load_lds_dwordx4 v11, s[22:23]\n\t" \
	"s_add_u32 m0, m0, 1032\n\t" \
	"s_nop 0\n\t" \
	"global_load_lds_dwordx4 v11, s[24:25]\n\t" \
	"s_add_u32 m0, m0, 1032\n\t" \
	"s_nop 0\n\t" \
	"global_load_lds_dwordx4 v11, s[26:27]\n\t" \
	"s_nop 1\n\t" \
	"v_add_u32 v11, 1024, v11\n\t" \
	"v_add_u32 v6, s10, v2\n\t" \
	"global_load_dword v5, v6, s[8:9]\n\t" \
	"61:\n" \
	"s_memtime s[100:101]\n\t" \
	"s_waitcnt lgkmcnt(0)\n\t" \
	"v_sub_u32 v127, s100, v126\n\t" \
	"v_add_u32 v119, v127, v119\n\t" \
	"v_mov_b32 v126, s100\n\t" \
	"s_branch 32f\n\t" \
	"73:\n" \
	"s_bitcmp1_b32 s28, 15\n\t" \
	"s_cbranch_scc1 83f\n\t" \
	"v_add_u32_sdwa v12, s52, v4 dst_sel:DWORD dst_unused:UNUSED_PAD src0_sel:WORD_1 src1_sel:DWORD\n\t" \
	"v_add_u32_sdwa v14, s53, v4 dst_sel:DWORD dst_unused:UNUSED_PAD src0_sel:WORD_1 src1_sel:DWORD\n\t" \
	"v_add_u32_sdwa v16, s54, v4 dst_sel:DWORD dst_unused:UNUSED_PAD src0_sel:WORD_1 src1_sel:DWORD\n\t" \
	"v_add_u32_sdwa v18, s55, v4 dst_sel:DWORD dst_unused:UNUSED_PAD src0_sel:WORD_1 src1_sel:DWORD\n\t" \
	"v_add_u32_sdwa v20, s56, v4 dst_sel:DWORD dst_unused:UNUSED_PAD src0_sel:WORD_1 src1_sel:DWORD\n\t" \
	"v_add_u32_sdwa v22, s57, v4 dst_sel:DWORD dst_unused:UNUSED_PAD src0_sel:WORD_1 src1_sel:DWORD\n\t" \
	"v_add_u32_sdwa v24, s58, v4 dst_sel:DWORD dst_unused:UNUSED_PAD src0_sel:WORD_1 src1_sel:DWORD\n\t" \
	"v_add_u32_sdwa v26, s59, v4 dst_sel:DWORD dst_unused:UNUSED_PAD src0_sel:WORD_1 src1_sel:DWORD\n\t" \
	"ds_read_b64 v[12:13], v12\n\t" \
	"ds_read_b64 v[14:15], v14\n\t" \
	"ds_read_b64 v[16:17], v16\n\t" \
	"ds_read_b64 v[18:19], v18\n\t" \
	"ds_read_b64 v[20:21], v20\n\t" \
	"ds_read_b64 v[22:23], v22\n\t" \
	"ds_read_b64 v[24:25], v24\n\t" \
	"ds_read_b64 v[26:27], v26\n\t" \
	"s_set_gpr_idx_on s28, gpr_idx(SRC2,DST)\n\t" \
	"v_fma_f64 v[44:45], s[36:37], v[28:29], v[44:45]\n\t" \
	"s_set_gpr_idx_idx s29\n\t" \
	"v_fma_f64 v[44:45], s[38:39], v[30:31], v[44:45]\n\t" \
	"s_set_gpr_idx_idx s30\n\t" \
	"v_fma_f64 v[44:45], s[40:41], v[32:33], v[44:45]\n\t" \
	"s_set_gpr_idx_idx s31\n\t" \
	"v_fma_f64 v[44:45], s[42:43], v[34:35], v[44:45]\n\t" \
	"s_set_gpr_idx_idx s32\n\t" \
	"v_fma_f64 v[44:45], s[44:45], v[36:37], v[44:45]\n\t" \
	"s_set_gpr_idx_idx s33\n\t" \
	"v_fma_f64 v[44:45], s[46:47], v[38:39], v[44:45]\n\t" \
	"s_set_gpr_idx_idx s34\n\t" \
	"v_fma_f64 v[44:45], s[48:49], v[40:41], v[44:45]\n\t" \
	"s_set_gpr_idx_idx s35\n\t" \
	"v_fma_f64 v[44:45], s[50:51], v[42:43], v[44:45]\n\t" \
	"s_set_gpr_idx_off\n\t" \
	"s_waitcnt lgkmcnt(0)\n\t" \
	"s_memtime s[100:101]\n\t" \
	"s_waitcnt lgkmcnt(0)\n\t" \
	"v_sub_u32 v127, s100, v126\n\t" \
	"v_add_u32 v123, v127, v123\n\t" \
	"v_mov_b32 v126, s100\n\t" \
	"s_cmp_ge_u32 s11, s12\n\t" \
	"s_cbranch_scc1 61f\n\t" \
	"s_cmp_lg_u32 s11, s16\n\t" \
	"s_cbranch_scc1 15f\n\t" \
	"v_subrev_u32 v11, s17, v11\n\t" \
	"15:\n" \
	"s_sub_u32 m0, s14, s13\n\t" \
	"s_nop 0\n\t" \
	"global_load_lds_dwordx4 v11, s[20:21]\n\t" \
	"s_add_u32 m0, m0, 1032\n\t" \
	"s_nop 0\n\t" \
	"global_load_lds_dwordx4 v11, s[22:23]\n\t" \
	"s_add_u32 m0, m0, 1032\n\t" \
	"s_nop 0\n\t" \
	"global_load_lds_dwordx4 v11, s[24:25]\n\t" \
	"s_add_u32 m0, m0, 1032\n\t" \
	"s_nop 0\n\t" \
	"global_load_lds_dwordx4 v11, s[26:27]\n\t" \
	"s_nop 1\n\t" \
	"v_add_u32 v11, 1024, v11\n\t" \
	"v_add_u32 v6, s10, v2\n\t" \
	"global_load_dword v5, v6, s[8:9]\n\t" \
	"61:\n" \
	"s_memtime s[100:101]\n\t" \
	"s_waitcnt lgkmcnt(0)\n\t" \
	"v_sub_u32 v127, s100, v126\n\t" \
	"v_add_u32 v119, v127, v119\n\t" \
	"v_mov_b32 v126, s100\n\t" \
	"s_branch 24b\n\t" \
	"83:\n" \
	"s_bitcmp1_b32 s28, 14\n\t" \
	"s_cbranch_scc0 33f\n\t" \
	"s_memtime s[100:101]\n\t" \
	"s_waitcnt lgkmcnt(0)\n\t" \
	"v_sub_u32 v127, s100, v126\n\t" \
	"v_add_u32 v123, v127, v123\n\t" \
	"v_mov_b32 v126, s100\n\t" \
	"s_cmp_ge_u32 s11, s12\n\t" \
	"s_cbranch_scc1 61f\n\t" \
	"s_cmp_lg_u32 s11, s16\n\t" \
	"s_cbranch_scc1 15f\n\t" \
	"v_subrev_u32 v11, s17, v11\n\t" \
	"15:\n" \
	"s_sub_u32 m0, s14, s13\n\t" \
	"s_nop 0\n\t" \
	"global_load_lds_dwordx4 v11, s[20:21]\n\t" \
	"s_add_u32 m0, m0, 1032\n\t" \
	"s_nop 0\n\t" \
	"global_load_lds_dwordx4 v11, s[22:23]\n\t" \
	"s_add_u32 m0, m0, 1032\n\t" \
	"s_nop 0\n\t" \
	"global_load_lds_dwordx4 v11, s[24:25]\n\t" \
	"s_add_u32 m0, m0, 1032\n\t" \
	"s_nop 0\n\t" \
	"global_load_lds_dwordx4 v11, s[26:27]\n\t" \
	"s_nop 1\n\t" \
	"v_add_u32 v11, 1024, v11\n\t" \
	"v_add_u32 v6, s10, v2\n\t" \
	"global_load_dword v5, v6, s[8:9]\n\t" \
	"61:\n" \
	"s_memtime s[100:101]\n\t" \
	"s_waitcnt lgkmcnt(0)\n\t" \
	"v_sub_u32 v127, s100, v126\n\t" \
	"v_add_u32 v119, v127, v119\n\t" \
	"v_mov_b32 v126, s100\n\t" \
	"s_branch 33f\n\t" \
	"74:\n" \
	"s_bitcmp1_b32 s52, 15\n\t" \
	"s_cbranch_scc1 84f\n\t" \
	"v_add_u32_sdwa v28, s76, v4 dst_sel:DWORD dst_unused:UNUSED_PAD src0_sel:WORD_1 src1_sel:DWORD\n\t" \
	"v_add_u32_sdwa v30, s77, v4 dst_sel:DWORD dst_unused:UNUSED_PAD src0_sel:WORD_1 src1_sel:DWORD\n\t" \
	"v_add_u32_sdwa v32, s78, v4 dst_sel:DWORD dst_unused:UNUSED_PAD src0_sel:WORD_1 src1_sel:DWORD\n\t" \
	"v_add_u32_sdwa v34, s79, v4 dst_sel:DWORD dst_unused:UNUSED_PAD src0_sel:WORD_1 src1_sel:DWORD\n\t" \
	"v_add_u32_sdwa v36, s80, v4 dst_sel:DWORD dst_unused:UNUSED_PAD src0_sel:WORD_1 src1_sel:DWORD\n\t" \
	"v_add_u32_sdwa v38, s81, v4 dst_sel:DWORD dst_unused:UNUSED_PAD src0_sel:WORD_1 src1_sel:DWORD\n\t" \
	"v_add_u32_sdwa v40, s82, v4 dst_sel:DWORD dst_unused:UNUSED_PAD src0_sel:WORD_1 src1_sel:DWORD\n\t" \
	"v_add_u32_sdwa v42, s83, v4 dst_sel:DWORD dst_unused:UNUSED_PAD src0_sel:WORD_1 src1_sel:DWORD\n\t" \
	"ds_read_b64 v[28:29], v28\n\t" \
	"ds_read_b64 v[30:31], v30\n\t" \
	"ds_read_b64 v[32:33], v32\n\t" \
	"ds_read_b64 v[34:35], v34\n\t" \
	"ds_read_b64 v[36:37], v36\n\t" \
	"ds_read_b64 v[38:39], v38\n\t" \
	"ds_read_b64 v[40:41], v40\n\t" \
	"ds_read_b64 v[42:43], v42\n\t" \
	"s_set_gpr_idx_on s52, gpr_idx(SRC2,DST)\n\t" \
	"v_fma_f64 v[44:45], s[60:61], v[12:13], v[44:45]\n\t" \
	"s_set_gpr_idx_idx s53\n\t" \
	"v_fma_f64 v[44:45], s[62:63], v[14:15], v[44:45]\n\t" \
	"s_set_gpr_idx_idx s54\n\t" \
	"v_fma_f64 v[44:45], s[64:65], v[16:17], v[44:45]\n\t" \
	"s_set_gpr_idx_idx s55\n\t" \
	"v_fma_f64 v[44:45], s[66:67], v[18:19], v[44:45]\n\t" \
	"s_set_gpr_idx_idx s56\n\t" \
	"v_fma_f64 v[44:45], s[68:69], v[20:21], v[44:45]\n\t" \
	"s_set_gpr_idx_idx s57\n\t" \
	"v_fma_f64 v[44:45], s[70:71], v[22:23], v[44:45]\n\t" \
	"s_set_gpr_idx_idx s58\n\t" \
	"v_fma_f64 v[44:45], s[72:73], v[24:25], v[44:45]\n\t" \
	"s_set_gpr_idx_idx s59\n\t" \
	"v_fma_f64 v[44:45], s[74:75], v[26:27], v[44:45]\n\t" \
	"s_set_gpr_idx_off\n\t" \
	"s_waitcnt lgkmcnt(0)\n\t" \
	"s_memtime s[100:101]\n\t" \
	"s_waitcnt lgkmcnt(0)\n\t" \
	"v_sub_u32 v127, s100, v126\n\t" \
	"v_add_u32 v123, v127, v123\n\t" \
	"v_mov_b32 v126, s100\n\t" \
	"s_cmp_ge_u32 s11, s12\n\t" \
	"s_cbranch_scc1 61f\n\t" \
	"s_cmp_lg_u32 s11, s16\n\t" \
	"s_cbranch_scc1 15f\n\t" \
	"v_subrev_u32 v11, s17, v11\n\t" \
	"15:\n" \
	"s_sub_u32 m0, s14, s13\n\t" \
	"s_nop 0\n\t" \
	"global_load_lds_dwordx4 v11, s[20:21]\n\t" \
	"s_add_u32 m0, m0, 1032\n\t" \
	"s_nop 0\n\t" \
	"global_load_lds_dwordx4 v11, s[22:23]\n\t" \
	"s_add_u32 m0, m0, 1032\n\t" \
	"s_nop 0\n\t" \
	"global_load_lds_dwordx4 v11, s[24:25]\n\t" \
	"s_add_u32 m0, m0, 1032\n\t" \
	"s_nop 0\n\t" \
	"global_load_lds_dwordx4 v11, s[26:27]\n\t" \
	"s_nop 1\n\t" \
	"v_add_u32 v11, 1024, v11\n\t" \
	"v_add_u32 v6, s10, v2\n\t" \
	"global_load_dword v5, v6, s[8:9]\n\t" \
	"61:\n" \
	"s_memtime s[100:101]\n\t" \
	"s_waitcnt lgkmcnt(0)\n\t" \
	"v_sub_u32 v127, s100, v126\n\t" \
	"v_add_u32 v119, v127, v119\n\t" \
	"v_mov_b32 v126, s100\n\t" \
	"s_branch 25b\n\t" \
	"84:\n" \
	"s_bitcmp1_b32 s52, 14\n\t" \
	"s_cbranch_scc0 34f\n\t" \
	"s_memtime s[100:101]\n\t" \
	"s_waitcnt lgkmcnt(0)\n\t" \
	"v_sub_u32 v127, s100, v126\n\t" \
	"v_add_u32 v123, v127, v123\n\t" \
	"v_mov_b32 v126, s100\n\t" \
	"s_cmp_ge_u32 s11, s12\n\t" \
	"s_cbranch_scc1 61f\n\t" \
	"s_cmp_lg_u32 s11, s16\n\t" \
	"s_cbranch_scc1 15f\n\t" \
	"v_subrev_u32 v11, s17, v11\n\t" \
	"15:\n" \
	"s_sub_u32 m0, s14, s13\n\t" \
	"s_nop 0\n\t" \
	"global_load_lds_dwordx4 v11, s[20:21]\n\t" \
	"s_add_u32 m0, m0, 1032\n\t" \
	"s_nop 0\n\t" \
	"global_load_lds_dwordx4 v11, s[22:23]\n\t" \
	"s_add_u32 m0, m0, 1032\n\t" \
	"s_nop 0\n\t" \
	"global_load_lds_dwordx4 v11, s[24:25]\n\t" \
	"s_add_u32 m0, m0, 1032\n\t" \
	"s_nop 0\n\t" \
	"global_load_lds_dwordx4 v11, s[26:27]\n\t" \
	"s_nop 1\n\t" \
	"v_add_u32 v11, 1024, v11\n\t" \
	"v_add_u32 v6, s10, v2\n\t" \
	"global_load_dword v5, v6, s[8:9]\n\t" \
	"61:\n" \
	"s_memtime s[100:101]\n\t" \
	"s_waitcnt lgkmcnt(0)\n\t" \
	"v_sub_u32 v127, s100, v126\n\t" \
	"v_add_u32 v119, v127, v119\n\t" \
	"v_mov_b32 v126, s100\n\t" \
	"s_branch 34f\n\t" \
	"75:\n" \
	"s_bitcmp1_b32 s76, 15\n\t" \
	"s_cbranch_scc1 85f\n\t" \
	"v_add_u32_sdwa v12, s28, v4 dst_sel:DWORD dst_unused:UNUSED_PAD src0_sel:WORD_1 src1_sel:DWORD\n\t" \
	"v_add_u32_sdwa v14, s29, v4 dst_sel:DWORD dst_unused:UNUSED_PAD src0_sel:WORD_1 src1_sel:DWORD\n\t" \
	"v_add_u32_sdwa v16, s30, v4 dst_sel:DWORD dst_unused:UNUSED_PAD src0_sel:WORD_1 src1_sel:DWORD\n\t" \
	"v_add_u32_sdwa v18, s31, v4 dst_sel:DWORD dst_unused:UNUSED_PAD src0_sel:WORD_1 src1_sel:DWORD\n\t" \
	"v_add_u32_sdwa v20, s32, v4 dst_sel:DWORD dst_unused:UNUSED_PAD src0_sel:WORD_1 src1_sel:DWORD\n\t" \
	"v_add_u32_sdwa v22, s33, v4 dst_sel:DWORD dst_unused:UNUSED_PAD src0_sel:WORD_1 src1_sel:DWORD\n\t" \
	"v_add_u32_sdwa v24, s34, v4 dst_sel:DWORD dst_unused:UNUSED_PAD src0_sel:WORD_1 src1_sel:DWORD\n\t" \
	"v_add_u32_sdwa v26, s35, v4 dst_sel:DWORD dst_unused:UNUSED_PAD src0_sel:WORD_1 src1_sel:DWORD\n\t" \
	"ds_read_b64 v[12:13], v12\n\t" \
	"ds_read_b64 v[14:15], v14\n\t" \
	"ds_read_b64 v[16:17], v16\n\t" \
	"ds_read_b64 v[18:19], v18\n\t" \
	"ds_read_b64 v[20:21], v20\n\t" \
	"ds_read_b64 v[22:23], v22\n\t" \
	"ds_read_b64 v[24:25], v24\n\t" \
	"ds_read_b64 v[26:27], v26\n\t" \
	"s_set_gpr_idx_on s76, gpr_idx(SRC2,DST)\n\t" \
	"v_fma_f64 v[44:45], s[84:85], v[28:29], v[44:45]\n\t" \
	"s_set_gpr_idx_idx s77\n\t" \
	"v_fma_f64 v[44:45], s[86:87], v[30:31], v[44:45]\n\t" \
	"s_set_gpr_idx_idx s78\n\t" \
	"v_fma_f64 v[44:45], s[88:89], v[32:33], v[44:45]\n\t" \
	"s_set_gpr_idx_idx s79\n\t" \
	"v_fma_f64 v[44:45], s[90:91], v[34:35], v[44:45]\n\t" \
	"s_set_gpr_idx_idx s80\n\t" \
	"v_fma_f64 v[44:45], s[92:93], v[36:37], v[44:45]\n\t" \
	"s_set_gpr_idx_idx s81\n\t" \
	"v_fma_f64 v[44:45], s[94:95], v[38:39], v[44:45]\n\t" \
	"s_set_gpr_idx_idx s82\n\t" \
	"v_fma_f64 v[44:45], s[96:97], v[40:41], v[44:45]\n\t" \
	"s_set_gpr_idx_idx s83\n\t" \
	"v_fma_f64 v[44:45], s[98:99], v[42:43], v[44:45]\n\t" \
	"s_set_gpr_idx_off\n\t" \
	"s_waitcnt lgkmcnt(0)\n\t" \
	"s_memtime s[100:101]\n\t" \
	"s_waitcnt lgkmcnt(0)\n\t" \
	"v_sub_u32 v127, s100, v126\n\t" \
	"v_add_u32 v123, v127, v123\n\t" \
	"v_mov_b32 v126, s100\n\t" \
	"s_cmp_ge_u32 s11, s12\n\t" \
	"s_cbranch_scc1 61f\n\t" \
	"s_cmp_lg_u32 s11, s16\n\t" \
	"s_cbranch_scc1 15f\n\t" \
	"v_subrev_u32 v11, s17, v11\n\t" \
	"15:\n" \
	"s_sub_u32 m0, s14, s13\n\t" \
	"s_nop 0\n\t" \
	"global_load_lds_dwordx4 v11, s[20:21]\n\t" \
	"s_add_u32 m0, m0, 1032\n\t" \
	"s_nop 0\n\t" \
	"global_load_lds_dwordx4 v11, s[22:23]\n\t" \
	"s_add_u32 m0, m0, 1032\n\t" \
	"s_nop 0\n\t" \
	"global_load_lds_dwordx4 v11, s[24:25]\n\t" \
	"s_add_u32 m0, m0, 1032\n\t" \
	"s_nop 0\n\t" \
	"global_load_lds_dwordx4 v11, s[26:27]\n\t" \
	"s_nop 1\n\t" \
	"v_add_u32 v11, 1024, v11\n\t" \
	"v_add_u32 v6, s10, v2\n\t" \
	"global_load_dword v5, v6, s[8:9]\n\t" \
	"61:\n" \
	"s_memtime s[100:101]\n\t" \
	"s_waitcnt lgkmcnt(0)\n\t" \
	"v_sub_u32 v127, s100, v126\n\t" \
	"v_add_u32 v119, v127, v119\n\t" \
	"v_mov_b32 v126, s100\n\t" \
	"s_branch 20b\n\t" \
	"85:\n" \
	"s_bitcmp1_b32 s76, 14\n\t" \
	"s_cbranch_scc0 35f\n\t" \
	"s_memtime s[100:101]\n\t" \
	"s_waitcnt lgkmcnt(0)\n\t" \
	"v_sub_u32 v127, s100, v126\n\t" \
	"v_add_u32 v123, v127, v123\n\t" \
	"v_mov_b32 v126, s100\n\t" \
	"s_cmp_ge_u32 s11, s12\n\t" \
	"s_cbranch_scc1 61f\n\t" \
	"s_cmp_lg_u32 s11, s16\n\t" \
	"s_cbranch_scc1 15f\n\t" \
	"v_subrev_u32 v11, s17, v11\n\t" \
	"15:\n" \
	"s_sub_u32 m0, s14, s13\n\t" \
	"s_nop 0\n\t" \
	"global_load_lds_dwordx4 v11, s[20:21]\n\t" \
	"s_add_u32 m0, m0, 1032\n\t" \
	"s_nop 0\n\t" \
	"global_load_lds_dwordx4 v11, s[22:23]\n\t" \
	"s_add_u32 m0, m0, 1032\n\t" \
	"s_nop 0\n\t" \
	"global_load_lds_dwordx4 v11, s[24:25]\n\t" \
	"s_add_u32 m0, m0, 1032\n\t" \
	"s_nop 0\n\t" \
	"global_load_lds_dwordx4 v11, s[26:27]\n\t" \
	"s_nop 1\n\t" \
	"v_add_u32 v11, 1024, v11\n\t" \
	"v_add_u32 v6, s10, v2\n\t" \
	"global_load_dword v5, v6, s[8:9]\n\t" \
	"61:\n" \
	"s_memtime s[100:101]\n\t" \
	"s_waitcnt lgkmcnt(0)\n\t" \
	"v_sub_u32 v127, s100, v126\n\t" \
	"v_add_u32 v119, v127, v119\n\t" \
	"v_mov_b32 v126, s100\n\t" \
	"s_branch 35f\n\t" \
	"30:\n" \
	"s_memtime s[100:101]\n\t" \
	"s_waitcnt lgkmcnt(0)\n\t" \
	"v_sub_u32 v127, s100, v126\n\t" \
	"v_add_u32 v123, v127, v123\n\t" \
	"v_mov_b32 v126, s100\n\t" \
	"s_cmp_ge_u32 s11, s12\n\t" \
	"s_cbranch_scc1 40f\n\t" \
	"s_xor_b32 s13, s13, 66048\n\t" \
	"v_add_u32 v4, s13, v0\n\t" \
	"s_cmp_lg_u32 s11, s16\n\t" \
	"s_cbranch_scc1 16f\n\t" \
	"v_add_u32 v4, s17, v4\n\t" \
	"16:\n" \
	"s_add_u32 s11, s11, 1\n\t" \
	"v_add_u32 v6, s13, v3\n\t" \
	"s_memtime s[100:101]\n\t" \
	"s_waitcnt lgkmcnt(0)\n\t" \
	"v_sub_u32 v127, s100, v126\n\t" \
	"v_add_u32 v120, v127, v120\n\t" \
	"v_mov_b32 v126, s100\n\t" \
	"v_add_u32_sdwa v28, s52, v4 dst_sel:DWORD dst_unused:UNUSED_PAD src0_sel:WORD_1 src1_sel:DWORD\n\t" \
	"v_add_u32_sdwa v30, s53, v4 dst_sel:DWORD dst_unused:UNUSED_PAD src0_sel:WORD_1 src1_sel:DWORD\n\t" \
	"v_add_u32_sdwa v32, s54, v4 dst_sel:DWORD dst_unused:UNUSED_PAD src0_sel:WORD_1 src1_sel:DWORD\n\t" \
	"v_add_u32_sdwa v34, s55, v4 dst_sel:DWORD dst_unused:UNUSED_PAD src0_sel:WORD_1 src1_sel:DWORD\n\t" \
	"v_add_u32_sdwa v36, s56, v4 dst_sel:DWORD dst_unused:UNUSED_PAD src0_sel:WORD_1 src1_sel:DWORD\n\t" \
	"v_add_u32_sdwa v38, s57, v4 dst_sel:DWORD dst_unused:UNUSED_PAD src0_sel:WORD_1 src1_sel:DWORD\n\t" \
	"v_add_u32_sdwa v40, s58, v4 dst_sel:DWORD dst_unused:UNUSED_PAD src0_sel:WORD_1 src1_sel:DWORD\n\t" \
	"v_add_u32_sdwa v42, s59, v4 dst_sel:DWORD dst_unused:UNUSED_PAD src0_sel:WORD_1 src1_sel:DWORD\n\t" \
	"s_waitcnt vmcnt(1)\n\t" \
	"s_memtime s[100:101]\n\t" \
	"s_waitcnt lgkmcnt(0)\n\t" \
	"v_sub_u32 v127, s100, v126\n\t" \
	"v_add_u32 v117, v127, v117\n\t" \
	"v_mov_b32 v126, s100\n\t" \
	"s_barrier\n\t" \
	"s_memtime s[100:101]\n\t" \
	"s_waitcnt lgkmcnt(0)\n\t" \
	"v_sub_u32 v127, s100, v126\n\t" \
	"v_add_u32 v118, v127, v118\n\t" \
	"v_mov_b32 v126, s100\n\t" \
	"ds_read_b64 v[28:29], v28\n\t" \
	"ds_read_b64 v[30:31], v30\n\t" \
	"ds_read_b64 v[32:33], v32\n\t" \
	"ds_read_b64 v[34:35], v34\n\t" \
	"ds_read_b64 v[36:37], v36\n\t" \
	"ds_read_b64 v[38:39], v38\n\t" \
	"ds_read_b64 v[40:41], v40\n\t" \
	"ds_read_b64 v[42:43], v42\n\t" \
	"s_set_gpr_idx_on s28, gpr_idx(SRC2,DST)\n\t" \
	"v_fma_f64 v[44:45], s[36:37], v[12:13], v[44:45]\n\t" \
	"s_set_gpr_idx_idx s29\n\t" \
	"v_fma_f64 v[44:45], s[38:39], v[14:15], v[44:45]\n\t" \
	"s_set_gpr_idx_idx s30\n\t" \
	"v_fma_f64 v[44:45], s[40:41], v[16:17], v[44:45]\n\t" \
	"s_set_gpr_idx_idx s31\n\t" \
	"v_fma_f64 v[44:45], s[42:43], v[18:19], v[44:45]\n\t" \
	"s_set_gpr_idx_idx s32\n\t" \
	"v_fma_f64 v[44:45], s[44:45], v[20:21], v[44:45]\n\t" \
	"s_set_gpr_idx_idx s33\n\t" \
	"v_fma_f64 v[44:45], s[46:47], v[22:23], v[44:45]\n\t" \
	"s_set_gpr_idx_idx s34\n\t" \
	"v_fma_f64 v[44:45], s[48:49], v[24:25], v[44:45]\n\t" \
	"s_set_gpr_idx_idx s35\n\t" \
	"v_fma_f64 v[44:45], s[50:51], v[26:27], v[44:45]\n\t" \
	"s_set_gpr_idx_off\n\t" \
	"s_mov_b32 m0, s19\n\t" \
	"s_memtime s[100:101]\n\t" \
	"s_waitcnt lgkmcnt(0)\n\t" \
	"v_sub_u32 v127, s100, v126\n\t" \
	"v_add_u32 v121, v127, v121\n\t" \
	"v_mov_b32 v126, s100\n\t" \
	"12:\n" \
	"ds_read_b64 v[8:9], v6\n\t" \
	"v_add_u32 v6, 8256, v6\n\t" \
	"s_waitcnt lgkmcnt(0)\n\t" \
	"v_cmp_class_f64 vcc, v[8:9], v10\n\t" \
	"s_or_b32 s18, s18, vcc_lo\n\t" \
	"s_or_b32 s18, s18, vcc_hi\n\t" \
	"s_sub_u32 m0, m0, 1\n\t" \
	"s_cbranch_scc0 12b\n\t" \
	"s_memtime s[100:101]\n\t" \
	"s_waitcnt lgkmcnt(0)\n\t" \
	"v_sub_u32 v127, s100, v126\n\t" \
	"v_add_u32 v122, v127, v122\n\t" \
	"v_mov_b32 v126, s100\n\t" \
	"s_branch 21b\n\t" \
	"31:\n" \
	"s_memtime s[100:101]\n\t" \
	"s_waitcnt lgkmcnt(0)\n\t" \
	"v_sub_u32 v127, s100, v126\n\t" \
	"v_add_u32 v123, v127, v123\n\t" \
	"v_mov_b32 v126, s100\n\t" \
	"s_cmp_ge_u32 s11, s12\n\t" \
	"s_cbranch_scc1 41f\n\t" \
	"s_xor_b32 s13, s13, 66048\n\t" \
	"v_add_u32 v4, s13, v0\n\t" \
	"s_cmp_lg_u32 s11, s16\n\t" \
	"s_cbranch_scc1 16f\n\t" \
	"v_add_u32 v4, s17, v4\n\t" \
	"16:\n" \
	"s_add_u32 s11, s11, 1\n\t" \
	"v_add_u32 v6, s13, v3\n\t" \
	"s_memtime s[100:101]\n\t" \
	"s_waitcnt lgkmcnt(0)\n\t" \
	"v_sub_u32 v127, s100, v126\n\t" \
	"v_add_u32 v120, v127, v120\n\t" \
	"v_mov_b32 v126, s100\n\t" \
	"v_add_u32_sdwa v12, s76, v4 dst_sel:DWORD dst_unused:UNUSED_PAD src0_sel:WORD_1 src1_sel:DWORD\n\t" \
	"v_add_u32_sdwa v14, s77, v4 dst_sel:DWORD dst_unused:UNUSED_PAD src0_sel:WORD_1 src1_sel:DWORD\n\t" \
	"v_add_u32_sdwa v16, s78, v4 dst_sel:DWORD dst_unused:UNUSED_PAD src0_sel:WORD_1 src1_sel:DWORD\n\t" \
	"v_add_u32_sdwa v18, s79, v4 dst_sel:DWORD dst_unused:UNUSED_PAD src0_sel:WORD_1 src1_sel:DWORD\n\t" \
	"v_add_u32_sdwa v20, s80, v4 dst_sel:DWORD dst_unused:UNUSED_PAD src0_sel:WORD_1 src1_sel:DWORD\n\t" \
	"v_add_u32_sdwa v22, s81, v4 dst_sel:DWORD dst_unused:UNUSED_PAD src0_sel:WORD_1 src1_sel:DWORD\n\t" \
	"v_add_u32_sdwa v24, s82, v4 dst_sel:DWORD dst_unused:UNUSED_PAD src0_sel:WORD_1 src1_sel:DWORD\n\t" \
	"v_add_u32_sdwa v26, s83, v4 dst_sel:DWORD dst_unused:UNUSED_PAD src0_sel:WORD_1 src1_sel:DWORD\n\t" \
	"s_waitcnt vmcnt(1)\n\t" \
	"s_memtime s[100:101]\n\t" \
	"s_waitcnt lgkmcnt(0)\n\t" \
	"v_sub_u32 v127, s100, v126\n\t" \
	"v_add_u32 v117, v127, v117\n\t" \
	"v_mov_b32 v126, s100\n\t" \
	"s_barrier\n\t" \
	"s_memtime s[100:101]\n\t" \
	"s_waitcnt lgkmcnt(0)\n\t" \
	"v_sub_u32 v127, s100, v126\n\t" \
	"v_add_u32 v118, v127, v118\n\t" \
	"v_mov_b32 v126, s100\n\t" \
	"ds_read_b64 v[12:13], v12\n\t" \
	"ds_read_b64 v[14:15], v14\n\t" \
	"ds_read_b64 v[16:17], v16\n\t" \
	"ds_read_b64 v[18:19], v18\n\t" \
	"ds_read_b64 v[20:21], v20\n\t" \
	"ds_read_b64 v[22:23], v22\n\t" \
	"ds_read_b64 v[24:25], v24\n\t" \
	"ds_read_b64 v[26:27], v26\n\t" \
	"s_set_gpr_idx_on s52, gpr_idx(SRC2,DST)\n\t" \
	"v_fma_f64 v[44:45], s[60:61], v[28:29], v[44:45]\n\t" \
	"s_set_gpr_idx_idx s53\n\t" \
	"v_fma_f64 v[44:45], s[62:63], v[30:31], v[44:45]\n\t" \
	"s_set_gpr_idx_idx s54\n\t" \
	"v_fma_f64 v[44:45], s[64:65], v[32:33], v[44:45]\n\t" \
	"s_set_gpr_idx_idx s55\n\t" \
	"v_fma_f64 v[44:45], s[66:67], v[34:35], v[44:45]\n\t" \
	"s_set_gpr_idx_idx s56\n\t" \
	"v_fma_f64 v[44:45], s[68:69], v[36:37], v[44:45]\n\t" \
	"s_set_gpr_idx_idx s57\n\t" \
	"v_fma_f64 v[44:45], s[70:71], v[38:39], v[44:45]\n\t" \
	"s_set_gpr_idx_idx s58\n\t" \
	"v_fma_f64 v[44:45], s[72:73], v[40:41], v[44:45]\n\t" \
	"s_set_gpr_idx_idx s59\n\t" \
	"v_fma_f64 v[44:45], s[74:75], v[42:43], v[44:45]\n\t" \
	"s_set_gpr_idx_off\n\t" \
	"s_mov_b32 m0, s19\n\t" \
	"s_memtime s[100:101]\n\t" \
	"s_waitcnt lgkmcnt(0)\n\t" \
	"v_sub_u32 v127, s100, v126\n\t" \
	"v_add_u32 v121, v127, v121\n\t" \
	"v_mov_b32 v126, s100\n\t" \
	"12:\n" \
	"ds_read_b64 v[8:9], v6\n\t" \
	"v_add_u32 v6, 8256, v6\n\t" \
	"s_waitcnt lgkmcnt(0)\n\t" \
	"v_cmp_class_f64 vcc, v[8:9], v10\n\t" \
	"s_or_b32 s18, s18, vcc_lo\n\t" \
	"s_or_b32 s18, s18, vcc_hi\n\t" \
	"s_sub_u32 m0, m0, 1\n\t" \
	"s_cbranch_scc0 12b\n\t" \
	"s_memtime s[100:101]\n\t" \
	"s_waitcnt lgkmcnt(0)\n\t" \
	"v_sub_u32 v127, s100, v126\n\t" \
	"v_add_u32 v122, v127, v122\n\t" \
	"v_mov_b32 v126, s100\n\t" \
	"s_branch 22b\n\t" \
	"32:\n" \
	"s_memtime s[100:101]\n\t" \
	"s_waitcnt lgkmcnt(0)\n\t" \
	"v_sub_u32 v127, s100, v126\n\t" \
	"v_add_u32 v123, v127, v123\n\t" \
	"v_mov_b32 v126, s100\n\t" \
	"s_cmp_ge_u32 s11, s12\n\t" \
	"s_cbranch_scc1 42f\n\t" \
	"s_xor_b32 s13, s13, 66048\n\t" \
	"v_add_u32 v4, s13, v0\n\t" \
	"s_cmp_lg_u32 s11, s16\n\t" \
	"s_cbranch_scc1 16f\n\t" \
	"v_add_u32 v4, s17, v4\n\t" \
	"16:\n" \
	"s_add_u32 s11, s11, 1\n\t" \
	"v_add_u32 v6, s13, v3\n\t" \
	"s_memtime s[100:101]\n\t" \
	"s_waitcnt lgkmcnt(0)\n\t" \
	"v_sub_u32 v127, s100, v126\n\t" \
	"v_add_u32 v120, v127, v120\n\t" \
	"v_mov_b32 v126, s100\n\t" \
	"v_add_u32_sdwa v28, s28, v4 dst_sel:DWORD dst_unused:UNUSED_PAD src0_sel:WORD_1 src1_sel:DWORD\n\t" \
	"v_add_u32_sdwa v30, s29, v4 dst_sel:DWORD dst_unused:UNUSED_PAD src0_sel:WORD_1 src1_sel:DWORD\n\t" \
	"v_add_u32_sdwa v32, s30, v4 dst_sel:DWORD dst_unused:UNUSED_PAD src0_sel:WORD_1 src1_sel:DWORD\n\t" \
	"v_add_u32_sdwa v34, s31, v4 dst_sel:DWORD dst_unused:UNUSED_PAD src0_sel:WORD_1 src1_sel:DWORD\n\t" \
	"v_add_u32_sdwa v36, s32, v4 dst_sel:DWORD dst_unused:UNUSED_PAD src0_sel:WORD_1 src1_sel:DWORD\n\t" \
	"v_add_u32_sdwa v38, s33, v4 dst_sel:DWORD dst_unused:UNUSED_PAD src0_sel:WORD_1 src1_sel:DWORD\n\t" \
	"v_add_u32_sdwa v40, s34, v4 dst_sel:DWORD dst_unused:UNUSED_PAD src0_sel:WORD_1 src1_sel:DWORD\n\t" \
	"v_add_u32_sdwa v42, s35, v4 dst_sel:DWORD dst_unused:UNUSED_PAD src0_sel:WORD_1 src1_sel:DWORD\n\t" \
	"s_waitcnt vmcnt(1)\n\t" \
	"s_memtime s[100:101]\n\t" \
	"s_waitcnt lgkmcnt(0)\n\t" \
	"v_sub_u32 v127, s100, v126\n\t" \
	"v_add_u32 v117, v127, v117\n\t" \
	"v_mov_b32 v126, s100\n\t" \
	"s_barrier\n\t" \
	"s_memtime s[100:101]\n\t" \
	"s_waitcnt lgkmcnt(0)\n\t" \
	"v_sub_u32 v127, s100, v126\n\t" \
	"v_add_u32 v118, v127, v118\n\t" \
	"v_mov_b32 v126, s100\n\t" \
	"ds_read_b64 v[28:29], v28\n\t" \
	"ds_read_b64 v[30:31], v30\n\t" \
	"ds_read_b64 v[32:33], v32\n\t" \
	"ds_read_b64 v[34:35], v34\n\t" \
	"ds_read_b64 v[36:37], v36\n\t" \
	"ds_read_b64 v[38:39], v38\n\t" \
	"ds_read_b64 v[40:41], v40\n\t" \
	"ds_read_b64 v[42:43], v42\n\t" \
	"s_set_gpr_idx_on s76, gpr_idx(SRC2,DST)\n\t" \
	"v_fma_f64 v[44:45], s[84:85], v[12:13], v[44:45]\n\t" \
	"s_set_gpr_idx_idx s77\n\t" \
	"v_fma_f64 v[44:45], s[86:87], v[14:15], v[44:45]\n\t" \
	"s_set_gpr_idx_idx s78\n\t" \
	"v_fma_f64 v[44:45], s[88:89], v[16:17], v[44:45]\n\t" \
	"s_set_gpr_idx_idx s79\n\t" \
	"v_fma_f64 v[44:45], s[90:91], v[18:19], v[44:45]\n\t" \
	"s_set_gpr_idx_idx s80\n\t" \
	"v_fma_f64 v[44:45], s[92:93], v[20:21], v[44:45]\n\t" \
	"s_set_gpr_idx_idx s81\n\t" \
	"v_fma_f64 v[44:45], s[94:95], v[22:23], v[44:45]\n\t" \
	"s_set_gpr_idx_idx s82\n\t" \
	"v_fma_f64 v[44:45], s[96:97], v[24:25], v[44:45]\n\t" \
	"s_set_gpr_idx_idx s83\n\t" \
	"v_fma_f64 v[44:45], s[98:99], v[26:27], v[44:45]\n\t" \
	"s_set_gpr_idx_off\n\t" \
	"s_mov_b32 m0, s19\n\t" \
	"s_memtime s[100:101]\n\t" \
	"s_waitcnt lgkmcnt(0)\n\t" \
	"v_sub_u32 v127, s100, v126\n\t" \
	"v_add_u32 v121, v127, v121\n\t" \
	"v_mov_b32 v126, s100\n\t" \
	"12:\n" \
	"ds_read_b64 v[8:9], v6\n\t" \
	"v_add_u32 v6, 8256, v6\n\t" \
	"s_waitcnt lgkmcnt(0)\n\t" \
	"v_cmp_class_f64 vcc, v[8:9], v10\n\t" \
	"s_or_b32 s18, s18, vcc_lo\n\t" \
	"s_or_b32 s18, s18, vcc_hi\n\t" \
	"s_sub_u32 m0, m0, 1\n\t" \
	"s_cbranch_scc0 12b\n\t" \
	"s_memtime s[100:101]\n\t" \
	"s_waitcnt lgkmcnt(0)\n\t" \
	"v_sub_u32 v127, s100, v126\n\t" \
	"v_add_u32 v122, v127, v122\n\t" \
	"v_mov_b32 v126, s100\n\t" \
	"s_branch 23b\n\t" \
	"33:\n" \
	"s_memtime s[100:101]\n\t" \
	"s_waitcnt lgkmcnt(0)\n\t" \
	"v_sub_u32 v127, s100, v126\n\t" \
	"v_add_u32 v123, v127, v123\n\t" \
	"v_mov_b32 v126, s100\n\t" \
	"s_cmp_ge_u32 s11, s12\n\t" \
	"s_cbranch_scc1 43f\n\t" \
	"s_xor_b32 s13, s13, 66048\n\t" \
	"v_add_u32 v4, s13, v0\n\t" \
	"s_cmp_lg_u32 s11, s16\n\t" \
	"s_cbranch_scc1 16f\n\t" \
	"v_add_u32 v4, s17, v4\n\t" \
	"16:\n" \
	"s_add_u32 s11, s11, 1\n\t" \
	"v_add_u32 v6, s13, v3\n\t" \
	"s_memtime s[100:101]\n\t" \
	"s_waitcnt lgkmcnt(0)\n\t" \
	"v_sub_u32 v127, s100, v126\n\t" \
	"v_add_u32 v120, v127, v120\n\t" \
	"v_mov_b32 v126, s100\n\t" \
	"v_add_u32_sdwa v12, s52, v4 dst_sel:DWORD dst_unused:UNUSED_PAD src0_sel:WORD_1 src1_sel:DWORD\n\t" \
	"v_add_u32_sdwa v14, s53, v4 dst_sel:DWORD dst_unused:UNUSED_PAD src0_sel:WORD_1 src1_sel:DWORD\n\t" \
	"v_add_u32_sdwa v16, s54, v4 dst_sel:DWORD dst_unused:UNUSED_PAD src0_sel:WORD_1 src1_sel:DWORD\n\t" \
	"v_add_u32_sdwa v18, s55, v4 dst_sel:DWORD dst_unused:UNUSED_PAD src0_sel:WORD_1 src1_sel:DWORD\n\t" \
	"v_add_u32_sdwa v20, s56, v4 dst_sel:DWORD dst_unused:UNUSED_PAD src0_sel:WORD_1 src1_sel:DWORD\n\t" \
	"v_add_u32_sdwa v22, s57, v4 dst_sel:DWORD dst_unused:UNUSED_PAD src0_sel:WORD_1 src1_sel:DWORD\n\t" \
	"v_add_u32_sdwa v24, s58, v4 dst_sel:DWORD dst_unused:UNUSED_PAD src0_sel:WORD_1 src1_sel:DWORD\n\t" \
	"v_add_u32_sdwa v26, s59, v4 dst_sel:DWORD dst_unused:UNUSED_PAD src0_sel:WORD_1 src1_sel:DWORD\n\t" \
	"s_waitcnt vmcnt(1)\n\t" \
	"s_memtime s[100:101]\n\t" \
	"s_waitcnt lgkmcnt(0)\n\t" \
	"v_sub_u32 v127, s100, v126\n\t" \
	"v_add_u32 v117, v127, v117\n\t" \
	"v_mov_b32 v126, s100\n\t" \
	"s_barrier\n\t" \
	"s_memtime s[100:101]\n\t" \
	"s_waitcnt lgkmcnt(0)\n\t" \
	"v_sub_u32 v127, s100, v126\n\t" \
	"v_add_u32 v118, v127, v118\n\t" \
	"v_mov_b32 v126, s100\n\t" \
	"ds_read_b64 v[12:13], v12\n\t" \
	"ds_read_b64 v[14:15], v14\n\t" \
	"ds_read_b64 v[16:17], v16\n\t" \
	"ds_read_b64 v[18:19], v18\n\t" \
	"ds_read_b64 v[20:21], v20\n\t" \
	"ds_read_b64 v[22:23], v22\n\t" \
	"ds_read_b64 v[24:25], v24\n\t" \
	"ds_read_b64 v[26:27], v26\n\t" \
	"s_set_gpr_idx_on s28, gpr_idx(SRC2,DST)\n\t" \
	"v_fma_f64 v[44:45], s[36:37], v[28:29], v[44:45]\n\t" \
	"s_set_gpr_idx_idx s29\n\t" \
	"v_fma_f64 v[44:45], s[38:39], v[30:31], v[44:45]\n\t" \
	"s_set_gpr_idx_idx s30\n\t" \
	"v_fma_f64 v[44:45], s[40:41], v[32:33], v[44:45]\n\t" \
	"s_set_gpr_idx_idx s31\n\t" \
	"v_fma_f64 v[44:45], s[42:43], v[34:35], v[44:45]\n\t" \
	"s_set_gpr_idx_idx s32\n\t" \
	"v_fma_f64 v[44:45], s[44:45], v[36:37], v[44:45]\n\t" \
	"s_set_gpr_idx_idx s33\n\t" \
	"v_fma_f64 v[44:45], s[46:47], v[38:39], v[44:45]\n\t" \
	"s_set_gpr_idx_idx s34\n\t" \
	"v_fma_f64 v[44:45], s[48:49], v[40:41], v[44:45]\n\t" \
	"s_set_gpr_idx_idx s35\n\t" \
	"v_fma_f64 v[44:45], s[50:51], v[42:43], v[44:45]\n\t" \
	"s_set_gpr_idx_off\n\t" \
	"s_mov_b32 m0, s19\n\t" \
	"s_memtime s[100:101]\n\t" \
	"s_waitcnt lgkmcnt(0)\n\t" \
	"v_sub_u32 v127, s100, v126\n\t" \
	"v_add_u32 v121, v127, v121\n\t" \
	"v_mov_b32 v126, s100\n\t" \
	"12:\n" \
	"ds_read_b64 v[8:9], v6\n\t" \
	"v_add_u32 v6, 8256, v6\n\t" \
	"s_waitcnt lgkmcnt(0)\n\t" \
	"v_cmp_class_f64 vcc, v[8:9], v10\n\t" \
	"s_or_b32 s18, s18, vcc_lo\n\t" \
	"s_or_b32 s18, s18, vcc_hi\n\t" \
	"s_sub_u32 m0, m0, 1\n\t" \
	"s_cbranch_scc0 12b\n\t" \
	"s_memtime s[100:101]\n\t" \
	"s_waitcnt lgkmcnt(0)\n\t" \
	"v_sub_u32 v127, s100, v126\n\t" \
	"v_add_u32 v122, v127, v122\n\t" \
	"v_mov_b32 v126, s100\n\t" \
	"s_branch 24b\n\t" \
	"34:\n" \
	"s_memtime s[100:101]\n\t" \
	"s_waitcnt lgkmcnt(0)\n\t" \
	"v_sub_u32 v127, s100, v126\n\t" \
	"v_add_u32 v123, v127, v123\n\t" \
	"v_mov_b32 v126, s100\n\t" \
	"s_cmp_ge_u32 s11, s12\n\t" \
	"s_cbranch_scc1 44f\n\t" \
	"s_xor_b32 s13, s13, 66048\n\t" \
	"v_add_u32 v4, s13, v0\n\t" \
	"s_cmp_lg_u32 s11, s16\n\t" \
	"s_cbranch_scc1 16f\n\t" \
	"v_add_u32 v4, s17, v4\n\t" \
	"16:\n" \
	"s_add_u32 s11, s11, 1\n\t" \
	"v_add_u32 v6, s13, v3\n\t" \
	"s_memtime s[100:101]\n\t" \
	"s_waitcnt lgkmcnt(0)\n\t" \
	"v_sub_u32 v127, s100, v126\n\t" \
	"v_add_u32 v120, v127, v120\n\t" \
	"v_mov_b32 v126, s100\n\t" \
	"v_add_u32_sdwa v28, s76, v4 dst_sel:DWORD dst_unused:UNUSED_PAD src0_sel:WORD_1 src1_sel:DWORD\n\t" \
	"v_add_u32_sdwa v30, s77, v4 dst_sel:DWORD dst_unused:UNUSED_PAD src0_sel:WORD_1 src1_sel:DWORD\n\t" \
	"v_add_u32_sdwa v32, s78, v4 dst_sel:DWORD dst_unused:UNUSED_PAD src0_sel:WORD_1 src1_sel:DWORD\n\t" \
	"v_add_u32_sdwa v34, s79, v4 dst_sel:DWORD dst_unused:UNUSED_PAD src0_sel:WORD_1 src1_sel:DWORD\n\t" \
	"v_add_u32_sdwa v36, s80, v4 dst_sel:DWORD dst_unused:UNUSED_PAD src0_sel:WORD_1 src1_sel:DWORD\n\t" \
	"v_add_u32_sdwa v38, s81, v4 dst_sel:DWORD dst_unused:UNUSED_PAD src0_sel:WORD_1 src1_sel:DWORD\n\t" \
	"v_add_u32_sdwa v40, s82, v4 dst_sel:DWORD dst_unused:UNUSED_PAD src0_sel:WORD_1 src1_sel:DWORD\n\t" \
	"v_add_u32_sdwa v42, s83, v4 dst_sel:DWORD dst_unused:UNUSED_PAD src0_sel:WORD_1 src1_sel:DWORD\n\t" \
	"s_waitcnt vmcnt(1)\n\t" \
	"s_memtime s[100:101]\n\t" \
	"s_waitcnt lgkmcnt(0)\n\t" \
	"v_sub_u32 v127, s100, v126\n\t" \
	"v_add_u32 v117, v127, v117\n\t" \
	"v_mov_b32 v126, s100\n\t" \
	"s_barrier\n\t" \
	"s_memtime s[100:101]\n\t" \
	"s_waitcnt lgkmcnt(0)\n\t" \
	"v_sub_u32 v127, s100, v126\n\t" \
	"v_add_u32 v118, v127, v118\n\t" \
	"v_mov_b32 v126, s100\n\t" \
	"ds_read_b64 v[28:29], v28\n\t" \
	"ds_read_b64 v[30:31], v30\n\t" \
	"ds_read_b64 v[32:33], v32\n\t" \
	"ds_read_b64 v[34:35], v34\n\t" \
	"ds_read_b64 v[36:37], v36\n\t" \
	"ds_read_b64 v[38:39], v38\n\t" \
	"ds_read_b64 v[40:41], v40\n\t" \
	"ds_read_b64 v[42:43], v42\n\t" \
	"s_set_gpr_idx_on s52, gpr_idx(SRC2,DST)\n\t" \
	"v_fma_f64 v[44:45], s[60:61], v[12:13], v[44:45]\n\t" \
	"s_set_gpr_idx_idx s53\n\t" \
	"v_fma_f64 v[44:45], s[62:63], v[14:15], v[44:45]\n\t" \
	"s_set_gpr_idx_idx s54\n\t" \
	"v_fma_f64 v[44:45], s[64:65], v[16:17], v[44:45]\n\t" \
	"s_set_gpr_idx_idx s55\n\t" \
	"v_fma_f64 v[44:45], s[66:67], v[18:19], v[44:45]\n\t" \
	"s_set_gpr_idx_idx s56\n\t" \
	"v_fma_f64 v[44:45], s[68:69], v[20:21], v[44:45]\n\t" \
	"s_set_gpr_idx_idx s57\n\t" \
	"v_fma_f64 v[44:45], s[70:71], v[22:23], v[44:45]\n\t" \
	"s_set_gpr_idx_idx s58\n\t" \
	"v_fma_f64 v[44:45], s[72:73], v[24:25], v[44:45]\n\t" \
	"s_set_gpr_idx_idx s59\n\t" \
	"v_fma_f64 v[44:45], s[74:75], v[26:27], v[44:45]\n\t" \
	"s_set_gpr_idx_off\n\t" \
	"s_mov_b32 m0, s19\n\t" \
	"s_memtime s[100:101]\n\t" \
	"s_waitcnt lgkmcnt(0)\n\t" \
	"v_sub_u32 v127, s100, v126\n\t" \
	"v_add_u32 v121, v127, v121\n\t" \
	"v_mov_b32 v126, s100\n\t" \
	"12:\n" \
	"ds_read_b64 v[8:9], v6\n\t" \
	"v_add_u32 v6, 8256, v6\n\t" \
	"s_waitcnt lgkmcnt(0)\n\t" \
	"v_cmp_class_f64 vcc, v[8:9], v10\n\t" \
	"s_or_b32 s18, s18, vcc_lo\n\t" \
	"s_or_b32 s18, s18, vcc_hi\n\t" \
	"s_sub_u32 m0, m0, 1\n\t" \
	"s_cbranch_scc0 12b\n\t" \
	"s_memtime s[100:101]\n\t" \
	"s_waitcnt lgkmcnt(0)\n\t" \
	"v_sub_u32 v127, s100, v126\n\t" \
	"v_add_u32 v122, v127, v122\n\t" \
	"v_mov_b32 v126, s100\n\t" \
	"s_branch 25b\n\t" \
	"35:\n" \
	"s_memtime s[100:101]\n\t" \
	"s_waitcnt lgkmcnt(0)\n\t" \
	"v_sub_u32 v127, s100, v126\n\t" \
	"v_add_u32 v123, v127, v123\n\t" \
	"v_mov_b32 v126, s100\n\t" \
	"s_cmp_ge_u32 s11, s12\n\t" \
	"s_cbranch_scc1 45f\n\t" \
	"s_xor_b32 s13, s13, 66048\n\t" \
	"v_add_u32 v4, s13, v0\n\t" \
	"s_cmp_lg_u32 s11, s16\n\t" \
	"s_cbranch_scc1 16f\n\t" \
	"v_add_u32 v4, s17, v4\n\t" \
	"16:\n" \
	"s_add_u32 s11, s11, 1\n\t" \
	"v_add_u32 v6, s13, v3\n\t" \
	"s_memtime s[100:101]\n\t" \
	"s_waitcnt lgkmcnt(0)\n\t" \
	"v_sub_u32 v127, s100, v126\n\t" \
	"v_add_u32 v120, v127, v120\n\t" \
	"v_mov_b32 v126, s100\n\t" \
	"v_add_u32_sdwa v12, s28, v4 dst_sel:DWORD dst_unused:UNUSED_PAD src0_sel:WORD_1 src1_sel:DWORD\n\t" \
	"v_add_u32_sdwa v14, s29, v4 dst_sel:DWORD dst_unused:UNUSED_PAD src0_sel:WORD_1 src1_sel:DWORD\n\t" \
	"v_add_u32_sdwa v16, s30, v4 dst_sel:DWORD dst_unused:UNUSED_PAD src0_sel:WORD_1 src1_sel:DWORD\n\t" \
	"v_add_u32_sdwa v18, s31, v4 dst_sel:DWORD dst_unused:UNUSED_PAD src0_sel:WORD_1 src1_sel:DWORD\n\t" \
	"v_add_u32_sdwa v20, s32, v4 dst_sel:DWORD dst_unused:UNUSED_PAD src0_sel:WORD_1 src1_sel:DWORD\n\t" \
	"v_add_u32_sdwa v22, s33, v4 dst_sel:DWORD dst_unused:UNUSED_PAD src0_sel:WORD_1 src1_sel:DWORD\n\t" \
	"v_add_u32_sdwa v24, s34, v4 dst_sel:DWORD dst_unused:UNUSED_PAD src0_sel:WORD_1 src1_sel:DWORD\n\t" \
	"v_add_u32_sdwa v26, s35, v4 dst_sel:DWORD dst_unused:UNUSED_PAD src0_sel:WORD_1 src1_sel:DWORD\n\t" \
	"s_waitcnt vmcnt(1)\n\t" \
	"s_memtime s[100:101]\n\t" \
	"s_waitcnt lgkmcnt(0)\n\t" \
	"v_sub_u32 v127, s100, v126\n\t" \
	"v_add_u32 v117, v127, v117\n\t" \
	"v_mov_b32 v126, s100\n\t" \
	"s_barrier\n\t" \
	"s_memtime s[100:101]\n\t" \
	"s_waitcnt lgkmcnt(0)\n\t" \
	"v_sub_u32 v127, s100, v126\n\t" \
	"v_add_u32 v118, v127, v118\n\t" \
	"v_mov_b32 v126, s100\n\t" \
	"ds_read_b64 v[12:13], v12\n\t" \
	"ds_read_b64 v[14:15], v14\n\t" \
	"ds_read_b64 v[16:17], v16\n\t" \
	"ds_read_b64 v[18:19], v18\n\t" \
	"ds_read_b64 v[20:21], v20\n\t" \
	"ds_read_b64 v[22:23], v22\n\t" \
	"ds_read_b64 v[24:25], v24\n\t" \
	"ds_read_b64 v[26:27], v26\n\t" \
	"s_set_gpr_idx_on s76, gpr_idx(SRC2,DST)\n\t" \
	"v_fma_f64 v[44:45], s[84:85], v[28:29], v[44:45]\n\t" \
	"s_set_gpr_idx_idx s77\n\t" \
	"v_fma_f64 v[44:45], s[86:87], v[30:31], v[44:45]\n\t" \
	"s_set_gpr_idx_idx s78\n\t" \
	"v_fma_f64 v[44:45], s[88:89], v[32:33], v[44:45]\n\t" \
	"s_set_gpr_idx_idx s79\n\t" \
	"v_fma_f64 v[44:45], s[90:91], v[34:35], v[44:45]\n\t" \
	"s_set_gpr_idx_idx s80\n\t" \
	"v_fma_f64 v[44:45], s[92:93], v[36:37], v[44:45]\n\t" \
	"s_set_gpr_idx_idx s81\n\t" \
	"v_fma_f64 v[44:45], s[94:95], v[38:39], v[44:45]\n\t" \
	"s_set_gpr_idx_idx s82\n\t" \
	"v_fma_f64 v[44:45], s[96:97], v[40:41], v[44:45]\n\t" \
	"s_set_gpr_idx_idx s83\n\t" \
	"v_fma_f64 v[44:45], s[98:99], v[42:43], v[44:45]\n\t" \
	"s_set_gpr_idx_off\n\t" \
	"s_mov_b32 m0, s19\n\t" \
	"s_memtime s[100:101]\n\t" \
	"s_waitcnt lgkmcnt(0)\n\t" \
	"v_sub_u32 v127, s100, v126\n\t" \
	"v_add_u32 v121, v127, v121\n\t" \
	"v_mov_b32 v126, s100\n\t" \
	"12:\n" \
	"ds_read_b64 v[8:9], v6\n\t" \
	"v_add_u32 v6, 8256, v6\n\t" \
	"s_waitcnt lgkmcnt(0)\n\t" \
	"v_cmp_class_f64 vcc, v[8:9], v10\n\t" \
	"s_or_b32 s18, s18, vcc_lo\n\t" \
	"s_or_b32 s18, s18, vcc_hi\n\t" \
	"s_sub_u32 m0, m0, 1\n\t" \
	"s_cbranch_scc0 12b\n\t" \
	"s_memtime s[100:101]\n\t" \
	"s_waitcnt lgkmcnt(0)\n\t" \
	"v_sub_u32 v127, s100, v126\n\t" \
	"v_add_u32 v122, v127, v122\n\t" \
	"v_mov_b32 v126, s100\n\t" \
	"s_branch 20b\n\t" \
	"55:\n" \
	"s_memtime s[100:101]\n\t" \
	"s_waitcnt lgkmcnt(0)\n\t" \
	"v_sub_u32 v127, s100, v126\n\t" \
	"v_add_u32 v123, v127, v123\n\t" \
	"v_mov_b32 v126, s100\n\t" \
	"s_cmp_ge_u32 s11, s12\n\t" \
	"s_cbranch_scc1 90f\n\t" \
	"s_xor_b32 s13, s13, 66048\n\t" \
	"v_add_u32 v4, s13, v0\n\t" \
	"s_cmp_lg_u32 s11, s16\n\t" \
	"s_cbranch_scc1 16f\n\t" \
	"v_add_u32 v4, s17, v4\n\t" \
	"16:\n" \
	"s_add_u32 s11, s11, 1\n\t" \
	"v_add_u32 v6, s13, v3\n\t" \
	"s_memtime s[100:101]\n\t" \
	"s_waitcnt lgkmcnt(0)\n\t" \
	"v_sub_u32 v127, s100, v126\n\t" \
	"v_add_u32 v120, v127, v120\n\t" \
	"v_mov_b32 v126, s100\n\t" \
	"v_add_u32_sdwa v12, s28, v4 dst_sel:DWORD dst_unused:UNUSED_PAD src0_sel:WORD_1 src1_sel:DWORD\n\t" \
	"v_add_u32_sdwa v14, s29, v4 dst_sel:DWORD dst_unused:UNUSED_PAD src0_sel:WORD_1 src1_sel:DWORD\n\t" \
	"v_add_u32_sdwa v16, s30, v4 dst_sel:DWORD dst_unused:UNUSED_PAD src0_sel:WORD_1 src1_sel:DWORD\n\t" \
	"v_add_u32_sdwa v18, s31, v4 dst_sel:DWORD dst_unused:UNUSED_PAD src0_sel:WORD_1 src1_sel:DWORD\n\t" \
	"v_add_u32_sdwa v20, s32, v4 dst_sel:DWORD dst_unused:UNUSED_PAD src0_sel:WORD_1 src1_sel:DWORD\n\t" \
	"v_add_u32_sdwa v22, s33, v4 dst_sel:DWORD dst_unused:UNUSED_PAD src0_sel:WORD_1 src1_sel:DWORD\n\t" \
	"v_add_u32_sdwa v24, s34, v4 dst_sel:DWORD dst_unused:UNUSED_PAD src0_sel:WORD_1 src1_sel:DWORD\n\t" \
	"v_add_u32_sdwa v26, s35, v4 dst_sel:DWORD dst_unused:UNUSED_PAD src0_sel:WORD_1 src1_sel:DWORD\n\t" \
	"s_waitcnt vmcnt(1)\n\t" \
	"s_memtime s[100:101]\n\t" \
	"s_waitcnt lgkmcnt(0)\n\t" \
	"v_sub_u32 v127, s100, v126\n\t" \
	"v_add_u32 v117, v127, v117\n\t" \
	"v_mov_b32 v126, s100\n\t" \
	"s_barrier\n\t" \
	"s_memtime s[100:101]\n\t" \
	"s_waitcnt lgkmcnt(0)\n\t" \
	"v_sub_u32 v127, s100, v126\n\t" \
	"v_add_u32 v118, v127, v118\n\t" \
	"v_mov_b32 v126, s100\n\t" \
	"ds_read_b64 v[12:13], v12\n\t" \
	"ds_read_b64 v[14:15], v14\n\t" \
	"ds_read_b64 v[16:17], v16\n\t" \
	"ds_read_b64 v[18:19], v18\n\t" \
	"ds_read_b64 v[20:21], v20\n\t" \
	"ds_read_b64 v[22:23], v22\n\t" \
	"ds_read_b64 v[24:25], v24\n\t" \
	"ds_read_b64 v[26:27], v26\n\t" \
	"s_mov_b32 m0, s19\n\t" \
	"s_memtime s[100:101]\n\t" \
	"s_waitcnt lgkmcnt(0)\n\t" \
	"v_sub_u32 v127, s100, v126\n\t" \
	"v_add_u32 v121, v127, v121\n\t" \
	"v_mov_b32 v126, s100\n\t" \
	"12:\n" \
	"ds_read_b64 v[8:9], v6\n\t" \
	"v_add_u32 v6, 8256, v6\n\t" \
	"s_waitcnt lgkmcnt(0)\n\t" \
	"v_cmp_class_f64 vcc, v[8:9], v10\n\t" \
	"s_or_b32 s18, s18, vcc_lo\n\t" \
	"s_or_b32 s18, s18, vcc_hi\n\t" \
	"s_sub_u32 m0, m0, 1\n\t" \
	"s_cbranch_scc0 12b\n\t" \
	"s_memtime s[100:101]\n\t" \
	"s_waitcnt lgkmcnt(0)\n\t" \
	"v_sub_u32 v127, s100, v126\n\t" \
	"v_add_u32 v122, v127, v122\n\t" \
	"v_mov_b32 v126, s100\n\t" \
	"s_branch 20b\n\t" \
	"40:\n" \
	"s_set_gpr_idx_on s28, gpr_idx(SRC2,DST)\n\t" \
	"v_fma_f64 v[44:45], s[36:37], v[12:13], v[44:45]\n\t" \
	"s_set_gpr_idx_idx s29\n\t" \
	"v_fma_f64 v[44:45], s[38:39], v[14:15], v[44:45]\n\t" \
	"s_set_gpr_idx_idx s30\n\t" \
	"v_fma_f64 v[44:45], s[40:41], v[16:17], v[44:45]\n\t" \
	"s_set_gpr_idx_idx s31\n\t" \
	"v_fma_f64 v[44:45], s[42:43], v[18:19], v[44:45]\n\t" \
	"s_set_gpr_idx_idx s32\n\t" \
	"v_fma_f64 v[44:45], s[44:45], v[20:21], v[44:45]\n\t" \
	"s_set_gpr_idx_idx s33\n\t" \
	"v_fma_f64 v[44:45], s[46:47], v[22:23], v[44:45]\n\t" \
	"s_set_gpr_idx_idx s34\n\t" \
	"v_fma_f64 v[44:45], s[48:49], v[24:25], v[44:45]\n\t" \
	"s_set_gpr_idx_idx s35\n\t" \
	"v_fma_f64 v[44:45], s[50:51], v[26:27], v[44:45]\n\t" \
	"s_set_gpr_idx_off\n\t" \
	"s_branch 90f\n\t" \
	"41:\n" \
	"s_set_gpr_idx_on s52, gpr_idx(SRC2,DST)\n\t" \
	"v_fma_f64 v[44:45], s[60:61], v[28:29], v[44:45]\n\t" \
	"s_set_gpr_idx_idx s53\n\t" \
	"v_fma_f64 v[44:45], s[62:63], v[30:31], v[44:45]\n\t" \
	"s_set_gpr_idx_idx s54\n\t" \
	"v_fma_f64 v[44:45], s[64:65], v[32:33], v[44:45]\n\t" \
	"s_set_gpr_idx_idx s55\n\t" \
	"v_fma_f64 v[44:45], s[66:67], v[34:35], v[44:45]\n\t" \
	"s_set_gpr_idx_idx s56\n\t" \
	"v_fma_f64 v[44:45], s[68:69], v[36:37], v[44:45]\n\t" \
	"s_set_gpr_idx_idx s57\n\t" \
// ... 88 lines not shown
```

Measured before the change: 57.92.

## Prescan own Y rows for NaN before barrier and fold DMA LDS offsets

The NaN/Inf prescan of the staged dense Y panel now runs before the barrier and covers each wave's own freshly DMA'd rows, using a strided 16-row share per block. Before, it scanned the whole tile after the FMA batch. The four global_load_lds issues now use immediate offsets with pre-biased source addresses instead of m0 increments and nops, which shortens the issue sequence. The intent is to trim scalar overhead and move the check off the post-FMA path. The cost is extra work before the barrier, and the new addressing relies on the immediate offset acting on both the global and LDS addresses.

```diff
diff --git a/sparsearray_amd/csrc/kernels_mult_pbc.hip b/sparsearray_amd/csrc/kernels_mult_pbc.hip
--- a/sparsearray_amd/csrc/kernels_mult_pbc.hip
+++ b/sparsearray_amd/csrc/kernels_mult_pbc.hip
@@ -1053,14 +1053,19 @@
 		PB[5] = partial ? (uint32_t) ((128 - (nrow & 127)) * 8) : 0u;
 		PB[6] = 0;
 		{
+#if PBC_DMA_PRESCAN_OWN
+			const int rshare = (128 + nblocks - 1) / nblocks;
+			PB[7] = (uint32_t) ((rshare + 15) / 16 - 1);
+#else
 			const int chunk = (8192 + nblocks - 1) / nblocks;
 			PB[7] = (uint32_t) ((chunk + 1023) / 1024 - 1);
+#endif
 		}
 #pragma unroll
 		for (int q = 0; q < 4; q++) {
 			int kk = k0 + wd * 4 + q;
 			if (kk > K - 1) kk = K - 1;
-			const uint64_t src = (uint64_t) (uintptr_t) (Y + (int64_t) kk * ldY + pa * 128);
+			const uint64_t src = (uint64_t) (uintptr_t) (Y + (int64_t) kk * ldY + pa * 128) - (uint64_t) (q * PBC_DMA_PIECE_OFF);
 			PB[8 + 2 * q] = (uint32_t) src; PB[9 + 2 * q] = (uint32_t) (src >> 32);
 		}
 	}
@@ -1072,12 +1077,20 @@
 		V0[1] = (uint32_t) lane * 16u;
 		V0[2] = (uint32_t) (lane < rt_lines ? lane : rt_lines - 1) * 128u + (uint32_t) rt_ahead;
 		V0[11] = (uint32_t) lane * 16u + 1024u;
+#if PBC_DMA_PRESCAN_OWN
+		const int rshare = (128 + nblocks - 1) / nblocks;
+		const int nit = (rshare + 15) / 16;
+		int r0 = bl * rshare;
+		if (r0 > 128 - nit * 16) r0 = 128 - nit * 16;
+		V0[3] = (uint32_t) ((wd * 4 + (lane >> 4)) * PBC_DMA_ROW + (r0 + (lane & 15)) * 8);
+#else
 		const int chunk = (8192 + nblocks - 1) / nblocks;
 		const int nit = (chunk + 1023) / 1024;
 		int e0 = bl * chunk;
 		if (e0 > 8192 - nit * 1024) e0 = 8192 - nit * 1024;
 		const int e = e0 + tid;
 		V0[3] = (uint32_t) ((e >> 7) * PBC_DMA_ROW + (e & 127) * 8);
+#endif
 		V0[7] = lane == 0 ? (uint32_t) nit :
 			lane == 1 ? (partial ? (uint32_t) (npanels - 1) : 0xFFFFFFFFu) :
 				    (partial ? (uint32_t) ((128 - (nrow & 127)) * 8) : 0u);
diff --git a/sparsearray_amd/csrc/pbc_dma_asm.inc b/sparsearray_amd/csrc/pbc_dma_asm.inc
--- a/sparsearray_amd/csrc/pbc_dma_asm.inc
+++ b/sparsearray_amd/csrc/pbc_dma_asm.inc
@@ -2,6 +2,8 @@
 #define PBC_DMA_BUF 66048
 #define PBC_DMA_BATCH_BYTES 96
 #define PBC_DMA_YSETS 2
+#define PBC_DMA_PIECE_OFF 1032
+#define PBC_DMA_PRESCAN_OWN 1
 #define PBC_DMA_ASM_TEXT \
 	"v_mov_b32 v10, 0x207\n\t" \
 	"s_load_dwordx8 s[28:35], s[8:9], s10\n\t" \
@@ -293,15 +295,9 @@
 	"s_sub_u32 m0, s14, s13\n\t" \
 	"s_nop 0\n\t" \
 	"global_load_lds_dwordx4 v11, s[20:21]\n\t" \
-	"s_add_u32 m0, m0, 1032\n\t" \
-	"s_nop 0\n\t" \
-	"global_load_lds_dwordx4 v11, s[22:23]\n\t" \
-	"s_add_u32 m0, m0, 1032\n\t" \
-	"s_nop 0\n\t" \
-	"global_load_lds_dwordx4 v11, s[24:25]\n\t" \
-	"s_add_u32 m0, m0, 1032\n\t" \
-	"s_nop 0\n\t" \
-	"global_load_lds_dwordx4 v11, s[26:27]\n\t" \
+	"global_load_lds_dwordx4 v11, s[22:23] offset:1032\n\t" \
+	"global_load_lds_dwordx4 v11, s[24:25] offset:2064\n\t" \
+	"global_load_lds_dwordx4 v11, s[26:27] offset:3096\n\t" \
 	"s_nop 1\n\t" \
 	"v_add_u32 v11, 1024, v11\n\t" \
 	"v_add_u32 v6, s10, v2\n\t" \
@@ -320,15 +316,9 @@
 	"s_sub_u32 m0, s14, s13\n\t" \
 	"s_nop 0\n\t" \
 	"global_load_lds_dwordx4 v11, s[20:21]\n\t" \
-	"s_add_u32 m0, m0, 1032\n\t" \
-	"s_nop 0\n\t" \
-	"global_load_lds_dwordx4 v11, s[22:23]\n\t" \
-	"s_add_u32 m0, m0, 1032\n\t" \
-	"s_nop 0\n\t" \
-	"global_load_lds_dwordx4 v11, s[24:25]\n\t" \
-	"s_add_u32 m0, m0, 1032\n\t" \
-	"s_nop 0\n\t" \
-	"global_load_lds_dwordx4 v11, s[26:27]\n\t" \
+	"global_load_lds_dwordx4 v11, s[22:23] offset:1032\n\t" \
+	"global_load_lds_dwordx4 v11, s[24:25] offset:2064\n\t" \
+	"global_load_lds_dwordx4 v11, s[26:27] offset:3096\n\t" \
 	"s_nop 1\n\t" \
 	"v_add_u32 v11, 1024, v11\n\t" \
 	"v_add_u32 v6, s10, v2\n\t" \
@@ -381,15 +371,9 @@
 	"s_sub_u32 m0, s14, s13\n\t" \
 	"s_nop 0\n\t" \
 	"global_load_lds_dwordx4 v11, s[20:21]\n\t" \
-	"s_add_u32 m0, m0, 1032\n\t" \
-	"s_nop 0\n\t" \
-	"global_load_lds_dwordx4 v11, s[22:23]\n\t" \
-	"s_add_u32 m0, m0, 1032\n\t" \
-	"s_nop 0\n\t" \
-	"global_load_lds_dwordx4 v11, s[24:25]\n\t" \
-	"s_add_u32 m0, m0, 1032\n\t" \
-	"s_nop 0\n\t" \
-	"global_load_lds_dwordx4 v11, s[26:27]\n\t" \
+	"global_load_lds_dwordx4 v11, s[22:23] offset:1032\n\t" \
+	"global_load_lds_dwordx4 v11, s[24:25] offset:2064\n\t" \
+	"global_load_lds_dwordx4 v11, s[26:27] offset:3096\n\t" \
 	"s_nop 1\n\t" \
 	"v_add_u32 v11, 1024, v11\n\t" \
 	"v_add_u32 v6, s10, v2\n\t" \
@@ -408,15 +392,9 @@
 	"s_sub_u32 m0, s14, s13\n\t" \
 	"s_nop 0\n\t" \
 	"global_load_lds_dwordx4 v11, s[20:21]\n\t" \
-	"s_add_u32 m0, m0, 1032\n\t" \
-	"s_nop 0\n\t" \
-	"global_load_lds_dwordx4 v11, s[22:23]\n\t" \
-	"s_add_u32 m0, m0, 1032\n\t" \
-	"s_nop 0\n\t" \
-	"global_load_lds_dwordx4 v11, s[24:25]\n\t" \
-	"s_add_u32 m0, m0, 1032\n\t" \
-	"s_nop 0\n\t" \
-	"global_load_lds_dwordx4 v11, s[26:27]\n\t" \
+	"global_load_lds_dwordx4 v11, s[22:23] offset:1032\n\t" \
+	"global_load_lds_dwordx4 v11, s[24:25] offset:2064\n\t" \
+	"global_load_lds_dwordx4 v11, s[26:27] offset:3096\n\t" \
 	"s_nop 1\n\t" \
 	"v_add_u32 v11, 1024, v11\n\t" \
 	"v_add_u32 v6, s10, v2\n\t" \
@@ -469,15 +447,9 @@
 	"s_sub_u32 m0, s14, s13\n\t" \
 	"s_nop 0\n\t" \
 	"global_load_lds_dwordx4 v11, s[20:21]\n\t" \
-	"s_add_u32 m0, m0, 1032\n\t" \
-	"s_nop 0\n\t" \
-	"global_load_lds_dwordx4 v11, s[22:23]\n\t" \
-	"s_add_u32 m0, m0, 1032\n\t" \
-	"s_nop 0\n\t" \
-	"global_load_lds_dwordx4 v11, s[24:25]\n\t" \
-	"s_add_u32 m0, m0, 1032\n\t" \
-	"s_nop 0\n\t" \
-	"global_load_lds_dwordx4 v11, s[26:27]\n\t" \
+	"global_load_lds_dwordx4 v11, s[22:23] offset:1032\n\t" \
+	"global_load_lds_dwordx4 v11, s[24:25] offset:2064\n\t" \
+	"global_load_lds_dwordx4 v11, s[26:27] offset:3096\n\t" \
 	"s_nop 1\n\t" \
 	"v_add_u32 v11, 1024, v11\n\t" \
 	"v_add_u32 v6, s10, v2\n\t" \
@@ -496,15 +468,9 @@
 	"s_sub_u32 m0, s14, s13\n\t" \
 	"s_nop 0\n\t" \
 	"global_load_lds_dwordx4 v11, s[20:21]\n\t" \
-	"s_add_u32 m0, m0, 1032\n\t" \
-	"s_nop 0\n\t" \
-	"global_load_lds_dwordx4 v11, s[22:23]\n\t" \
-	"s_add_u32 m0, m0, 1032\n\t" \
-	"s_nop 0\n\t" \
-	"global_load_lds_dwordx4 v11, s[24:25]\n\t" \
-	"s_add_u32 m0, m0, 1032\n\t" \
-	"s_nop 0\n\t" \
-	"global_load_lds_dwordx4 v11, s[26:27]\n\t" \
+	"global_load_lds_dwordx4 v11, s[22:23] offset:1032\n\t" \
+	"global_load_lds_dwordx4 v11, s[24:25] offset:2064\n\t" \
+	"global_load_lds_dwordx4 v11, s[26:27] offset:3096\n\t" \
 	"s_nop 1\n\t" \
 	"v_add_u32 v11, 1024, v11\n\t" \
 	"v_add_u32 v6, s10, v2\n\t" \
@@ -557,15 +523,9 @@
 	"s_sub_u32 m0, s14, s13\n\t" \
 	"s_nop 0\n\t" \
 	"global_load_lds_dwordx4 v11, s[20:21]\n\t" \
-	"s_add_u32 m0, m0, 1032\n\t" \
-	"s_nop 0\n\t" \
-	"global_load_lds_dwordx4 v11, s[22:23]\n\t" \
-	"s_add_u32 m0, m0, 1032\n\t" \
-	"s_nop 0\n\t" \
-	"global_load_lds_dwordx4 v11, s[24:25]\n\t" \
-	"s_add_u32 m0, m0, 1032\n\t" \
-	"s_nop 0\n\t" \
-	"global_load_lds_dwordx4 v11, s[26:27]\n\t" \
+	"global_load_lds_dwordx4 v11, s[22:23] offset:1032\n\t" \
+	"global_load_lds_dwordx4 v11, s[24:25] offset:2064\n\t" \
+	"global_load_lds_dwordx4 v11, s[26:27] offset:3096\n\t" \
 	"s_nop 1\n\t" \
 	"v_add_u32 v11, 1024, v11\n\t" \
 	"v_add_u32 v6, s10, v2\n\t" \
@@ -584,15 +544,9 @@
 	"s_sub_u32 m0, s14, s13\n\t" \
 	"s_nop 0\n\t" \
 	"global_load_lds_dwordx4 v11, s[20:21]\n\t" \
-	"s_add_u32 m0, m0, 1032\n\t" \
-	"s_nop 0\n\t" \
-	"global_load_lds_dwordx4 v11, s[22:23]\n\t" \
-	"s_add_u32 m0, m0, 1032\n\t" \
-	"s_nop 0\n\t" \
-	"global_load_lds_dwordx4 v11, s[24:25]\n\t" \
-	"s_add_u32 m0, m0, 1032\n\t" \
-	"s_nop 0\n\t" \
-	"global_load_lds_dwordx4 v11, s[26:27]\n\t" \
+	"global_load_lds_dwordx4 v11, s[22:23] offset:1032\n\t" \
+	"global_load_lds_dwordx4 v11, s[24:25] offset:2064\n\t" \
+	"global_load_lds_dwordx4 v11, s[26:27] offset:3096\n\t" \
 	"s_nop 1\n\t" \
 	"v_add_u32 v11, 1024, v11\n\t" \
 	"v_add_u32 v6, s10, v2\n\t" \
@@ -645,15 +599,9 @@
 	"s_sub_u32 m0, s14, s13\n\t" \
 	"s_nop 0\n\t" \
 	"global_load_lds_dwordx4 v11, s[20:21]\n\t" \
-	"s_add_u32 m0, m0, 1032\n\t" \
-	"s_nop 0\n\t" \
-	"global_load_lds_dwordx4 v11, s[22:23]\n\t" \
-	"s_add_u32 m0, m0, 1032\n\t" \
-	"s_nop 0\n\t" \
-	"global_load_lds_dwordx4 v11, s[24:25]\n\t" \
-	"s_add_u32 m0, m0, 1032\n\t" \
-	"s_nop 0\n\t" \
-	"global_load_lds_dwordx4 v11, s[26:27]\n\t" \
+	"global_load_lds_dwordx4 v11, s[22:23] offset:1032\n\t" \
+	"global_load_lds_dwordx4 v11, s[24:25] offset:2064\n\t" \
+	"global_load_lds_dwordx4 v11, s[26:27] offset:3096\n\t" \
 	"s_nop 1\n\t" \
 	"v_add_u32 v11, 1024, v11\n\t" \
 	"v_add_u32 v6, s10, v2\n\t" \
@@ -672,15 +620,9 @@
 	"s_sub_u32 m0, s14, s13\n\t" \
 	"s_nop 0\n\t" \
 	"global_load_lds_dwordx4 v11, s[20:21]\n\t" \
-	"s_add_u32 m0, m0, 1032\n\t" \
-	"s_nop 0\n\t" \
-	"global_load_lds_dwordx4 v11, s[22:23]\n\t" \
-	"s_add_u32 m0, m0, 1032\n\t" \
-	"s_nop 0\n\t" \
-	"global_load_lds_dwordx4 v11, s[24:25]\n\t" \
-	"s_add_u32 m0, m0, 1032\n\t" \
-	"s_nop 0\n\t" \
-	"global_load_lds_dwordx4 v11, s[26:27]\n\t" \
+	"global_load_lds_dwordx4 v11, s[22:23] offset:1032\n\t" \
+	"global_load_lds_dwordx4 v11, s[24:25] offset:2064\n\t" \
+	"global_load_lds_dwordx4 v11, s[26:27] offset:3096\n\t" \
 	"s_nop 1\n\t" \
 	"v_add_u32 v11, 1024, v11\n\t" \
 	"v_add_u32 v6, s10, v2\n\t" \
@@ -733,15 +675,9 @@
 	"s_sub_u32 m0, s14, s13\n\t" \
 	"s_nop 0\n\t" \
 	"global_load_lds_dwordx4 v11, s[20:21]\n\t" \
-	"s_add_u32 m0, m0, 1032\n\t" \
-	"s_nop 0\n\t" \
-	"global_load_lds_dwordx4 v11, s[22:23]\n\t" \
-	"s_add_u32 m0, m0, 1032\n\t" \
-	"s_nop 0\n\t" \
-	"global_load_lds_dwordx4 v11, s[24:25]\n\t" \
-	"s_add_u32 m0, m0, 1032\n\t" \
-	"s_nop 0\n\t" \
-	"global_load_lds_dwordx4 v11, s[26:27]\n\t" \
+	"global_load_lds_dwordx4 v11, s[22:23] offset:1032\n\t" \
+	"global_load_lds_dwordx4 v11, s[24:25] offset:2064\n\t" \
+	"global_load_lds_dwordx4 v11, s[26:27] offset:3096\n\t" \
 	"s_nop 1\n\t" \
 	"v_add_u32 v11, 1024, v11\n\t" \
 	"v_add_u32 v6, s10, v2\n\t" \
@@ -760,15 +696,9 @@
 	"s_sub_u32 m0, s14, s13\n\t" \
 	"s_nop 0\n\t" \
 	"global_load_lds_dwordx4 v11, s[20:21]\n\t" \
-	"s_add_u32 m0, m0, 1032\n\t" \
-	"s_nop 0\n\t" \
-	"global_load_lds_dwordx4 v11, s[22:23]\n\t" \
-	"s_add_u32 m0, m0, 1032\n\t" \
-	"s_nop 0\n\t" \
-	"global_load_lds_dwordx4 v11, s[24:25]\n\t" \
-	"s_add_u32 m0, m0, 1032\n\t" \
-	"s_nop 0\n\t" \
-	"global_load_lds_dwordx4 v11, s[26:27]\n\t" \
+	"global_load_lds_dwordx4 v11, s[22:23] offset:1032\n\t" \
+	"global_load_lds_dwordx4 v11, s[24:25] offset:2064\n\t" \
+	"global_load_lds_dwordx4 v11, s[26:27] offset:3096\n\t" \
 	"s_nop 1\n\t" \
 	"v_add_u32 v11, 1024, v11\n\t" \
 	"v_add_u32 v6, s10, v2\n\t" \
@@ -795,6 +725,16 @@
 	"v_add_u32_sdwa v40, s58, v4 dst_sel:DWORD dst_unused:UNUSED_PAD src0_sel:WORD_1 src1_sel:DWORD\n\t" \
 	"v_add_u32_sdwa v42, s59, v4 dst_sel:DWORD dst_unused:UNUSED_PAD src0_sel:WORD_1 src1_sel:DWORD\n\t" \
 	"s_waitcnt vmcnt(1)\n\t" \
+	"s_mov_b32 m0, s19\n\t" \
+	"12:\n" \
+	"ds_read_b64 v[8:9], v6\n\t" \
+	"v_add_u32 v6, 128, v6\n\t" \
+	"s_waitcnt lgkmcnt(0)\n\t" \
+	"v_cmp_class_f64 vcc, v[8:9], v10\n\t" \
+	"s_or_b32 s18, s18, vcc_lo\n\t" \
+	"s_or_b32 s18, s18, vcc_hi\n\t" \
+	"s_sub_u32 m0, m0, 1\n\t" \
+	"s_cbranch_scc0 12b\n\t" \
 	"s_barrier\n\t" \
 	"ds_read_b64 v[28:29], v28\n\t" \
 	"ds_read_b64 v[30:31], v30\n\t" \
@@ -821,16 +761,7 @@
 	"s_set_gpr_idx_idx s35\n\t" \
 	"v_fma_f64 v[44:45], s[50:51], v[26:27], v[44:45]\n\t" \
 	"s_set_gpr_idx_off\n\t" \
-	"s_mov_b32 m0, s19\n\t" \
-	"12:\n" \
-	"ds_read_b64 v[8:9], v6\n\t" \
-	"v_add_u32 v6, 8256, v6\n\t" \
-	"s_waitcnt lgkmcnt(0)\n\t" \
-	"v_cmp_class_f64 vcc, v[8:9], v10\n\t" \
-	"s_or_b32 s18, s18, vcc_lo\n\t" \
-	"s_or_b32 s18, s18, vcc_hi\n\t" \
-	"s_sub_u32 m0, m0, 1\n\t" \
-	"s_cbranch_scc0 12b\n\t" \
+	"s_waitcnt lgkmcnt(0)\n\t" \
 	"s_branch 21b\n\t" \
 	"31:\n" \
 	"s_cmp_ge_u32 s11, s12\n\t" \
@@ -852,6 +783,16 @@
 	"v_add_u32_sdwa v24, s82, v4 dst_sel:DWORD dst_unused:UNUSED_PAD src0_sel:WORD_1 src1_sel:DWORD\n\t" \
 	"v_add_u32_sdwa v26, s83, v4 dst_sel:DWORD dst_unused:UNUSED_PAD src0_sel:WORD_1 src1_sel:DWORD\n\t" \
 	"s_waitcnt vmcnt(1)\n\t" \
+	"s_mov_b32 m0, s19\n\t" \
+	"12:\n" \
+	"ds_read_b64 v[8:9], v6\n\t" \
+	"v_add_u32 v6, 128, v6\n\t" \
+	"s_waitcnt lgkmcnt(0)\n\t" \
+	"v_cmp_class_f64 vcc, v[8:9], v10\n\t" \
+	"s_or_b32 s18, s18, vcc_lo\n\t" \
+	"s_or_b32 s18, s18, vcc_hi\n\t" \
+	"s_sub_u32 m0, m0, 1\n\t" \
+	"s_cbranch_scc0 12b\n\t" \
 	"s_barrier\n\t" \
 	"ds_read_b64 v[12:13], v12\n\t" \
 	"ds_read_b64 v[14:15], v14\n\t" \
@@ -878,16 +819,7 @@
 	"s_set_gpr_idx_idx s59\n\t" \
 	"v_fma_f64 v[44:45], s[74:75], v[42:43], v[44:45]\n\t" \
 	"s_set_gpr_idx_off\n\t" \
-	"s_mov_b32 m0, s19\n\t" \
-	"12:\n" \
-	"ds_read_b64 v[8:9], v6\n\t" \
-	"v_add_u32 v6, 8256, v6\n\t" \
-	"s_waitcnt lgkmcnt(0)\n\t" \
-	"v_cmp_class_f64 vcc, v[8:9], v10\n\t" \
-	"s_or_b32 s18, s18, vcc_lo\n\t" \
-	"s_or_b32 s18, s18, vcc_hi\n\t" \
-	"s_sub_u32 m0, m0, 1\n\t" \
-	"s_cbranch_scc0 12b\n\t" \
+	"s_waitcnt lgkmcnt(0)\n\t" \
 	"s_branch 22b\n\t" \
 	"32:\n" \
 	"s_cmp_ge_u32 s11, s12\n\t" \
@@ -909,6 +841,16 @@
 	"v_add_u32_sdwa v40, s34, v4 dst_sel:DWORD dst_unused:UNUSED_PAD src0_sel:WORD_1 src1_sel:DWORD\n\t" \
 	"v_add_u32_sdwa v42, s35, v4 dst_sel:DWORD dst_unused:UNUSED_PAD src0_sel:WORD_1 src1_sel:DWORD\n\t" \
 	"s_waitcnt vmcnt(1)\n\t" \
+	"s_mov_b32 m0, s19\n\t" \
+	"12:\n" \
+	"ds_read_b64 v[8:9], v6\n\t" \
+	"v_add_u32 v6, 128, v6\n\t" \
+	"s_waitcnt lgkmcnt(0)\n\t" \
+	"v_cmp_class_f64 vcc, v[8:9], v10\n\t" \
+	"s_or_b32 s18, s18, vcc_lo\n\t" \
+	"s_or_b32 s18, s18, vcc_hi\n\t" \
+	"s_sub_u32 m0, m0, 1\n\t" \
+	"s_cbranch_scc0 12b\n\t" \
 	"s_barrier\n\t" \
 	"ds_read_b64 v[28:29], v28\n\t" \
 	"ds_read_b64 v[30:31], v30\n\t" \
@@ -935,16 +877,7 @@
 	"s_set_gpr_idx_idx s83\n\t" \
 	"v_fma_f64 v[44:45], s[98:99], v[26:27], v[44:45]\n\t" \
 	"s_set_gpr_idx_off\n\t" \
-	"s_mov_b32 m0, s19\n\t" \
-	"12:\n" \
-	"ds_read_b64 v[8:9], v6\n\t" \
-	"v_add_u32 v6, 8256, v6\n\t" \
-	"s_waitcnt lgkmcnt(0)\n\t" \
-	"v_cmp_class_f64 vcc, v[8:9], v10\n\t" \
-	"s_or_b32 s18, s18, vcc_lo\n\t" \
-	"s_or_b32 s18, s18, vcc_hi\n\t" \
-	"s_sub_u32 m0, m0, 1\n\t" \
-	"s_cbranch_scc0 12b\n\t" \
+	"s_waitcnt lgkmcnt(0)\n\t" \
 	"s_branch 23b\n\t" \
 	"33:\n" \
 	"s_cmp_ge_u32 s11, s12\n\t" \
@@ -966,6 +899,16 @@
 	"v_add_u32_sdwa v24, s58, v4 dst_sel:DWORD dst_unused:UNUSED_PAD src0_sel:WORD_1 src1_sel:DWORD\n\t" \
 	"v_add_u32_sdwa v26, s59, v4 dst_sel:DWORD dst_unused:UNUSED_PAD src0_sel:WORD_1 src1_sel:DWORD\n\t" \
 	"s_waitcnt vmcnt(1)\n\t" \
+	"s_mov_b32 m0, s19\n\t" \
+	"12:\n" \
+	"ds_read_b64 v[8:9], v6\n\t" \
+	"v_add_u32 v6, 128, v6\n\t" \
+	"s_waitcnt lgkmcnt(0)\n\t" \
+	"v_cmp_class_f64 vcc, v[8:9], v10\n\t" \
+	"s_or_b32 s18, s18, vcc_lo\n\t" \
+	"s_or_b32 s18, s18, vcc_hi\n\t" \
+	"s_sub_u32 m0, m0, 1\n\t" \
+	"s_cbranch_scc0 12b\n\t" \
 	"s_barrier\n\t" \
 	"ds_read_b64 v[12:13], v12\n\t" \
 	"ds_read_b64 v[14:15], v14\n\t" \
@@ -992,16 +935,7 @@
 	"s_set_gpr_idx_idx s35\n\t" \
 	"v_fma_f64 v[44:45], s[50:51], v[42:43], v[44:45]\n\t" \
 	"s_set_gpr_idx_off\n\t" \
-	"s_mov_b32 m0, s19\n\t" \
-	"12:\n" \
-	"ds_read_b64 v[8:9], v6\n\t" \
-	"v_add_u32 v6, 8256, v6\n\t" \
-	"s_waitcnt lgkmcnt(0)\n\t" \
-	"v_cmp_class_f64 vcc, v[8:9], v10\n\t" \
-	"s_or_b32 s18, s18, vcc_lo\n\t" \
-	"s_or_b32 s18, s18, vcc_hi\n\t" \
-	"s_sub_u32 m0, m0, 1\n\t" \
-	"s_cbranch_scc0 12b\n\t" \
+	"s_waitcnt lgkmcnt(0)\n\t" \
 	"s_branch 24b\n\t" \
 	"34:\n" \
 	"s_cmp_ge_u32 s11, s12\n\t" \
@@ -1023,6 +957,16 @@
 	"v_add_u32_sdwa v40, s82, v4 dst_sel:DWORD dst_unused:UNUSED_PAD src0_sel:WORD_1 src1_sel:DWORD\n\t" \
 	"v_add_u32_sdwa v42, s83, v4 dst_sel:DWORD dst_unused:UNUSED_PAD src0_sel:WORD_1 src1_sel:DWORD\n\t" \
 	"s_waitcnt vmcnt(1)\n\t" \
+	"s_mov_b32 m0, s19\n\t" \
+	"12:\n" \
+	"ds_read_b64 v[8:9], v6\n\t" \
+	"v_add_u32 v6, 128, v6\n\t" \
+	"s_waitcnt lgkmcnt(0)\n\t" \
+	"v_cmp_class_f64 vcc, v[8:9], v10\n\t" \
+	"s_or_b32 s18, s18, vcc_lo\n\t" \
+	"s_or_b32 s18, s18, vcc_hi\n\t" \
+	"s_sub_u32 m0, m0, 1\n\t" \
+	"s_cbranch_scc0 12b\n\t" \
 	"s_barrier\n\t" \
 	"ds_read_b64 v[28:29], v28\n\t" \
 	"ds_read_b64 v[30:31], v30\n\t" \
@@ -1049,16 +993,7 @@
 	"s_set_gpr_idx_idx s59\n\t" \
 	"v_fma_f64 v[44:45], s[74:75], v[26:27], v[44:45]\n\t" \
 	"s_set_gpr_idx_off\n\t" \
-	"s_mov_b32 m0, s19\n\t" \
-	"12:\n" \
-	"ds_read_b64 v[8:9], v6\n\t" \
-	"v_add_u32 v6, 8256, v6\n\t" \
-	"s_waitcnt lgkmcnt(0)\n\t" \
-	"v_cmp_class_f64 vcc, v[8:9], v10\n\t" \
-	"s_or_b32 s18, s18, vcc_lo\n\t" \
-	"s_or_b32 s18, s18, vcc_hi\n\t" \
-	"s_sub_u32 m0, m0, 1\n\t" \
-	"s_cbranch_scc0 12b\n\t" \
+	"s_waitcnt lgkmcnt(0)\n\t" \
 	"s_branch 25b\n\t" \
 	"35:\n" \
 	"s_cmp_ge_u32 s11, s12\n\t" \
@@ -1080,6 +1015,16 @@
 	"v_add_u32_sdwa v24, s34, v4 dst_sel:DWORD dst_unused:UNUSED_PAD src0_sel:WORD_1 src1_sel:DWORD\n\t" \
 	"v_add_u32_sdwa v26, s35, v4 dst_sel:DWORD dst_unused:UNUSED_PAD src0_sel:WORD_1 src1_sel:DWORD\n\t" \
 	"s_waitcnt vmcnt(1)\n\t" \
+	"s_mov_b32 m0, s19\n\t" \
+	"12:\n" \
+	"ds_read_b64 v[8:9], v6\n\t" \
+	"v_add_u32 v6, 128, v6\n\t" \
+	"s_waitcnt lgkmcnt(0)\n\t" \
+	"v_cmp_class_f64 vcc, v[8:9], v10\n\t" \
+	"s_or_b32 s18, s18, vcc_lo\n\t" \
+	"s_or_b32 s18, s18, vcc_hi\n\t" \
+	"s_sub_u32 m0, m0, 1\n\t" \
+	"s_cbranch_scc0 12b\n\t" \
 	"s_barrier\n\t" \
 	"ds_read_b64 v[12:13], v12\n\t" \
 	"ds_read_b64 v[14:15], v14\n\t" \
@@ -1106,16 +1051,7 @@
 	"s_set_gpr_idx_idx s83\n\t" \
 	"v_fma_f64 v[44:45], s[98:99], v[42:43], v[44:45]\n\t" \
 	"s_set_gpr_idx_off\n\t" \
-	"s_mov_b32 m0, s19\n\t" \
-	"12:\n" \
-	"ds_read_b64 v[8:9], v6\n\t" \
-	"v_add_u32 v6, 8256, v6\n\t" \
-	"s_waitcnt lgkmcnt(0)\n\t" \
-	"v_cmp_class_f64 vcc, v[8:9], v10\n\t" \
-	"s_or_b32 s18, s18, vcc_lo\n\t" \
-	"s_or_b32 s18, s18, vcc_hi\n\t" \
-	"s_sub_u32 m0, m0, 1\n\t" \
-	"s_cbranch_scc0 12b\n\t" \
+	"s_waitcnt lgkmcnt(0)\n\t" \
 	"s_branch 20b\n\t" \
 	"55:\n" \
 	"s_cmp_ge_u32 s11, s12\n\t" \
@@ -1137,6 +1073,16 @@
 	"v_add_u32_sdwa v24, s34, v4 dst_sel:DWORD dst_unused:UNUSED_PAD src0_sel:WORD_1 src1_sel:DWORD\n\t" \
 	"v_add_u32_sdwa v26, s35, v4 dst_sel:DWORD dst_unused:UNUSED_PAD src0_sel:WORD_1 src1_sel:DWORD\n\t" \
 	"s_waitcnt vmcnt(1)\n\t" \
+	"s_mov_b32 m0, s19\n\t" \
+	"12:\n" \
+	"ds_read_b64 v[8:9], v6\n\t" \
+	"v_add_u32 v6, 128, v6\n\t" \
+	"s_waitcnt lgkmcnt(0)\n\t" \
+	"v_cmp_class_f64 vcc, v[8:9], v10\n\t" \
+	"s_or_b32 s18, s18, vcc_lo\n\t" \
+	"s_or_b32 s18, s18, vcc_hi\n\t" \
+	"s_sub_u32 m0, m0, 1\n\t" \
+	"s_cbranch_scc0 12b\n\t" \
 	"s_barrier\n\t" \
 	"ds_read_b64 v[12:13], v12\n\t" \
 	"ds_read_b64 v[14:15], v14\n\t" \
@@ -1146,16 +1092,7 @@
 	"ds_read_b64 v[22:23], v22\n\t" \
 	"ds_read_b64 v[24:25], v24\n\t" \
 	"ds_read_b64 v[26:27], v26\n\t" \
-	"s_mov_b32 m0, s19\n\t" \
-	"12:\n" \
-	"ds_read_b64 v[8:9], v6\n\t" \
-	"v_add_u32 v6, 8256, v6\n\t" \
-	"s_waitcnt lgkmcnt(0)\n\t" \
-	"v_cmp_class_f64 vcc, v[8:9], v10\n\t" \
-	"s_or_b32 s18, s18, vcc_lo\n\t" \
-	"s_or_b32 s18, s18, vcc_hi\n\t" \
-	"s_sub_u32 m0, m0, 1\n\t" \
-	"s_cbranch_scc0 12b\n\t" \
+	"s_waitcnt lgkmcnt(0)\n\t" \
 	"s_branch 20b\n\t" \
 	"40:\n" \
 	"s_set_gpr_idx_on s28, gpr_idx(SRC2,DST)\n\t" \
@@ -1574,15 +1511,9 @@
 	"s_sub_u32 m0, s14, s13\n\t" \
 	"s_nop 0\n\t" \
 	"global_load_lds_dwordx4 v11, s[20:21]\n\t" \
-	"s_add_u32 m0, m0, 1032\n\t" \
-	"s_nop 0\n\t" \
-	"global_load_lds_dwordx4 v11, s[22:23]\n\t" \
-	"s_add_u32 m0, m0, 1032\n\t" \
-	"s_nop 0\n\t" \
-	"global_load_lds_dwordx4 v11, s[24:25]\n\t" \
-	"s_add_u32 m0, m0, 1032\n\t" \
-	"s_nop 0\n\t" \
-	"global_load_lds_dwordx4 v11, s[26:27]\n\t" \
+	"global_load_lds_dwordx4 v11, s[22:23] offset:1032\n\t" \
+	"global_load_lds_dwordx4 v11, s[24:25] offset:2064\n\t" \
+	"global_load_lds_dwordx4 v11, s[26:27] offset:3096\n\t" \
 	"s_nop 1\n\t" \
 	"v_add_u32 v11, 1024, v11\n\t" \
 	"v_add_u32 v6, s10, v2\n\t" \
@@ -1611,15 +1542,9 @@
 	"s_sub_u32 m0, s14, s13\n\t" \
 	"s_nop 0\n\t" \
 	"global_load_lds_dwordx4 v11, s[20:21]\n\t" \
-	"s_add_u32 m0, m0, 1032\n\t" \
-	"s_nop 0\n\t" \
-	"global_load_lds_dwordx4 v11, s[22:23]\n\t" \
-	"s_add_u32 m0, m0, 1032\n\t" \
-	"s_nop 0\n\t" \
-	"global_load_lds_dwordx4 v11, s[24:25]\n\t" \
-	"s_add_u32 m0, m0, 1032\n\t" \
-	"s_nop 0\n\t" \
-	"global_load_lds_dwordx4 v11, s[26:27]\n\t" \
+	"global_load_lds_dwordx4 v11, s[22:23] offset:1032\n\t" \
+	"global_load_lds_dwordx4 v11, s[24:25] offset:2064\n\t" \
+	"global_load_lds_dwordx4 v11, s[26:27] offset:3096\n\t" \
 	"s_nop 1\n\t" \
 	"v_add_u32 v11, 1024, v11\n\t" \
 	"v_add_u32 v6, s10, v2\n\t" \
@@ -1682,15 +1607,9 @@
 	"s_sub_u32 m0, s14, s13\n\t" \
 	"s_nop 0\n\t" \
 	"global_load_lds_dwordx4 v11, s[20:21]\n\t" \
-	"s_add_u32 m0, m0, 1032\n\t" \
-	"s_nop 0\n\t" \
-	"global_load_lds_dwordx4 v11, s[22:23]\n\t" \
-	"s_add_u32 m0, m0, 1032\n\t" \
-	"s_nop 0\n\t" \
-	"global_load_lds_dwordx4 v11, s[24:25]\n\t" \
-	"s_add_u32 m0, m0, 1032\n\t" \
-	"s_nop 0\n\t" \
-	"global_load_lds_dwordx4 v11, s[26:27]\n\t" \
+	"global_load_lds_dwordx4 v11, s[22:23] offset:1032\n\t" \
+	"global_load_lds_dwordx4 v11, s[24:25] offset:2064\n\t" \
+	"global_load_lds_dwordx4 v11, s[26:27] offset:3096\n\t" \
 	"s_nop 1\n\t" \
 	"v_add_u32 v11, 1024, v11\n\t" \
 	"v_add_u32 v6, s10, v2\n\t" \
@@ -1719,15 +1638,9 @@
 	"s_sub_u32 m0, s14, s13\n\t" \
 	"s_nop 0\n\t" \
 	"global_load_lds_dwordx4 v11, s[20:21]\n\t" \
-	"s_add_u32 m0, m0, 1032\n\t" \
-	"s_nop 0\n\t" \
-	"global_load_lds_dwordx4 v11, s[22:23]\n\t" \
-	"s_add_u32 m0, m0, 1032\n\t" \
-	"s_nop 0\n\t" \
-	"global_load_lds_dwordx4 v11, s[24:25]\n\t" \
-	"s_add_u32 m0, m0, 1032\n\t" \
-	"s_nop 0\n\t" \
-	"global_load_lds_dwordx4 v11, s[26:27]\n\t" \
+	"global_load_lds_dwordx4 v11, s[22:23] offset:1032\n\t" \
+	"global_load_lds_dwordx4 v11, s[24:25] offset:2064\n\t" \
+	"global_load_lds_dwordx4 v11, s[26:27] offset:3096\n\t" \
 	"s_nop 1\n\t" \
 	"v_add_u32 v11, 1024, v11\n\t" \
 	"v_add_u32 v6, s10, v2\n\t" \
@@ -1790,15 +1703,9 @@
 	"s_sub_u32 m0, s14, s13\n\t" \
 	"s_nop 0\n\t" \
 	"global_load_lds_dwordx4 v11, s[20:21]\n\t" \
-	"s_add_u32 m0, m0, 1032\n\t" \
-	"s_nop 0\n\t" \
-	"global_load_lds_dwordx4 v11, s[22:23]\n\t" \
-	"s_add_u32 m0, m0, 1032\n\t" \
-	"s_nop 0\n\t" \
-	"global_load_lds_dwordx4 v11, s[24:25]\n\t" \
-	"s_add_u32 m0, m0, 1032\n\t" \
-	"s_nop 0\n\t" \
-	"global_load_lds_dwordx4 v11, s[26:27]\n\t" \
+	"global_load_lds_dwordx4 v11, s[22:23] offset:1032\n\t" \
+	"global_load_lds_dwordx4 v11, s[24:25] offset:2064\n\t" \
+	"global_load_lds_dwordx4 v11, s[26:27] offset:3096\n\t" \
 	"s_nop 1\n\t" \
 	"v_add_u32 v11, 1024, v11\n\t" \
 	"v_add_u32 v6, s10, v2\n\t" \
@@ -1827,15 +1734,9 @@
 	"s_sub_u32 m0, s14, s13\n\t" \
 	"s_nop 0\n\t" \
 	"global_load_lds_dwordx4 v11, s[20:21]\n\t" \
-	"s_add_u32 m0, m0, 1032\n\t" \
-	"s_nop 0\n\t" \
-	"global_load_lds_dwordx4 v11, s[22:23]\n\t" \
-	"s_add_u32 m0, m0, 1032\n\t" \
-	"s_nop 0\n\t" \
-	"global_load_lds_dwordx4 v11, s[24:25]\n\t" \
-	"s_add_u32 m0, m0, 1032\n\t" \
-	"s_nop 0\n\t" \
-	"global_load_lds_dwordx4 v11, s[26:27]\n\t" \
+	"global_load_lds_dwordx4 v11, s[22:23] offset:1032\n\t" \
+	"global_load_lds_dwordx4 v11, s[24:25] offset:2064\n\t" \
+	"global_load_lds_dwordx4 v11, s[26:27] offset:3096\n\t" \
 	"s_nop 1\n\t" \
 	"v_add_u32 v11, 1024, v11\n\t" \
 	"v_add_u32 v6, s10, v2\n\t" \
@@ -1898,15 +1799,9 @@
 	"s_sub_u32 m0, s14, s13\n\t" \
 	"s_nop 0\n\t" \
 	"global_load_lds_dwordx4 v11, s[20:21]\n\t" \
-	"s_add_u32 m0, m0, 1032\n\t" \
-	"s_nop 0\n\t" \
-	"global_load_lds_dwordx4 v11, s[22:23]\n\t" \
-	"s_add_u32 m0, m0, 1032\n\t" \
-	"s_nop 0\n\t" \
-	"global_load_lds_dwordx4 v11, s[24:25]\n\t" \
-	"s_add_u32 m0, m0, 1032\n\t" \
-	"s_nop 0\n\t" \
-	"global_load_lds_dwordx4 v11, s[26:27]\n\t" \
+	"global_load_lds_dwordx4 v11, s[22:23] offset:1032\n\t" \
+	"global_load_lds_dwordx4 v11, s[24:25] offset:2064\n\t" \
+	"global_load_lds_dwordx4 v11, s[26:27] offset:3096\n\t" \
 	"s_nop 1\n\t" \
 	"v_add_u32 v11, 1024, v11\n\t" \
 	"v_add_u32 v6, s10, v2\n\t" \
@@ -1935,15 +1830,9 @@
 	"s_sub_u32 m0, s14, s13\n\t" \
 	"s_nop 0\n\t" \
 	"global_load_lds_dwordx4 v11, s[20:21]\n\t" \
-	"s_add_u32 m0, m0, 1032\n\t" \
-	"s_nop 0\n\t" \
-	"global_load_lds_dwordx4 v11, s[22:23]\n\t" \
-	"s_add_u32 m0, m0, 1032\n\t" \
-	"s_nop 0\n\t" \
-	"global_load_lds_dwordx4 v11, s[24:25]\n\t" \
-	"s_add_u32 m0, m0, 1032\n\t" \
-	"s_nop 0\n\t" \
-	"global_load_lds_dwordx4 v11, s[26:27]\n\t" \
+	"global_load_lds_dwordx4 v11, s[22:23] offset:1032\n\t" \
+	"global_load_lds_dwordx4 v11, s[24:25] offset:2064\n\t" \
+	"global_load_lds_dwordx4 v11, s[26:27] offset:3096\n\t" \
 	"s_nop 1\n\t" \
 	"v_add_u32 v11, 1024, v11\n\t" \
 	"v_add_u32 v6, s10, v2\n\t" \
@@ -2006,15 +1895,9 @@
 	"s_sub_u32 m0, s14, s13\n\t" \
 	"s_nop 0\n\t" \
 	"global_load_lds_dwordx4 v11, s[20:21]\n\t" \
-	"s_add_u32 m0, m0, 1032\n\t" \
-	"s_nop 0\n\t" \
-	"global_load_lds_dwordx4 v11, s[22:23]\n\t" \
-	"s_add_u32 m0, m0, 1032\n\t" \
-	"s_nop 0\n\t" \
-	"global_load_lds_dwordx4 v11, s[24:25]\n\t" \
-	"s_add_u32 m0, m0, 1032\n\t" \
-	"s_nop 0\n\t" \
-	"global_load_lds_dwordx4 v11, s[26:27]\n\t" \
+	"global_load_lds_dwordx4 v11, s[22:23] offset:1032\n\t" \
+	"global_load_lds_dwordx4 v11, s[24:25] offset:2064\n\t" \
+	"global_load_lds_dwordx4 v11, s[26:27] offset:3096\n\t" \
 	"s_nop 1\n\t" \
 	"v_add_u32 v11, 1024, v11\n\t" \
 	"v_add_u32 v6, s10, v2\n\t" \
@@ -2043,15 +1926,9 @@
 	"s_sub_u32 m0, s14, s13\n\t" \
 	"s_nop 0\n\t" \
 	"global_load_lds_dwordx4 v11, s[20:21]\n\t" \
-	"s_add_u32 m0, m0, 1032\n\t" \
-	"s_nop 0\n\t" \
-	"global_load_lds_dwordx4 v11, s[22:23]\n\t" \
-	"s_add_u32 m0, m0, 1032\n\t" \
-	"s_nop 0\n\t" \
-	"global_load_lds_dwordx4 v11, s[24:25]\n\t" \
-	"s_add_u32 m0, m0, 1032\n\t" \
-	"s_nop 0\n\t" \
-	"global_load_lds_dwordx4 v11, s[26:27]\n\t" \
+	"global_load_lds_dwordx4 v11, s[22:23] offset:1032\n\t" \
+	"global_load_lds_dwordx4 v11, s[24:25] offset:2064\n\t" \
+	"global_load_lds_dwordx4 v11, s[26:27] offset:3096\n\t" \
 	"s_nop 1\n\t" \
 	"v_add_u32 v11, 1024, v11\n\t" \
 	"v_add_u32 v6, s10, v2\n\t" \
@@ -2114,15 +1991,9 @@
 	"s_sub_u32 m0, s14, s13\n\t" \
 	"s_nop 0\n\t" \
 	"global_load_lds_dwordx4 v11, s[20:21]\n\t" \
-	"s_add_u32 m0, m0, 1032\n\t" \
-	"s_nop 0\n\t" \
-	"global_load_lds_dwordx4 v11, s[22:23]\n\t" \
-	"s_add_u32 m0, m0, 1032\n\t" \
-	"s_nop 0\n\t" \
-	"global_load_lds_dwordx4 v11, s[24:25]\n\t" \
-	"s_add_u32 m0, m0, 1032\n\t" \
-	"s_nop 0\n\t" \
-	"global_load_lds_dwordx4 v11, s[26:27]\n\t" \
+	"global_load_lds_dwordx4 v11, s[22:23] offset:1032\n\t" \
+	"global_load_lds_dwordx4 v11, s[24:25] offset:2064\n\t" \
+	"global_load_lds_dwordx4 v11, s[26:27] offset:3096\n\t" \
 	"s_nop 1\n\t" \
 	"v_add_u32 v11, 1024, v11\n\t" \
 	"v_add_u32 v6, s10, v2\n\t" \
@@ -2151,15 +2022,9 @@
 	"s_sub_u32 m0, s14, s13\n\t" \
 	"s_nop 0\n\t" \
 	"global_load_lds_dwordx4 v11, s[20:21]\n\t" \
-	"s_add_u32 m0, m0, 1032\n\t" \
-	"s_nop 0\n\t" \
-	"global_load_lds_dwordx4 v11, s[22:23]\n\t" \
-	"s_add_u32 m0, m0, 1032\n\t" \
-	"s_nop 0\n\t" \
-	"global_load_lds_dwordx4 v11, s[24:25]\n\t" \
-	"s_add_u32 m0, m0, 1032\n\t" \
-	"s_nop 0\n\t" \
-	"global_load_lds_dwordx4 v11, s[26:27]\n\t" \
+	"global_load_lds_dwordx4 v11, s[22:23] offset:1032\n\t" \
+	"global_load_lds_dwordx4 v11, s[24:25] offset:2064\n\t" \
+	"global_load_lds_dwordx4 v11, s[26:27] offset:3096\n\t" \
 	"s_nop 1\n\t" \
 	"v_add_u32 v11, 1024, v11\n\t" \
 	"v_add_u32 v6, s10, v2\n\t" \
@@ -2205,6 +2070,21 @@
 	"s_waitcnt lgkmcnt(0)\n\t" \
 	"v_sub_u32 v127, s100, v126\n\t" \
 	"v_add_u32 v117, v127, v117\n\t" \
+	"v_mov_b32 v126, s100\n\t" \
+	"s_mov_b32 m0, s19\n\t" \
+	"12:\n" \
+	"ds_read_b64 v[8:9], v6\n\t" \
+	"v_add_u32 v6, 128, v6\n\t" \
+	"s_waitcnt lgkmcnt(0)\n\t" \
+	"v_cmp_class_f64 vcc, v[8:9], v10\n\t" \
+	"s_or_b32 s18, s18, vcc_lo\n\t" \
+	"s_or_b32 s18, s18, vcc_hi\n\t" \
+	"s_sub_u32 m0, m0, 1\n\t" \
+	"s_cbranch_scc0 12b\n\t" \
+	"s_memtime s[100:101]\n\t" \
+	"s_waitcnt lgkmcnt(0)\n\t" \
+	"v_sub_u32 v127, s100, v126\n\t" \
+	"v_add_u32 v122, v127, v122\n\t" \
 	"v_mov_b32 v126, s100\n\t" \
 	"s_barrier\n\t" \
 	"s_memtime s[100:101]\n\t" \
@@ -2237,25 +2117,11 @@
 	"s_set_gpr_idx_idx s35\n\t" \
 	"v_fma_f64 v[44:45], s[50:51], v[26:27], v[44:45]\n\t" \
 	"s_set_gpr_idx_off\n\t" \
-	"s_mov_b32 m0, s19\n\t" \
+	"s_waitcnt lgkmcnt(0)\n\t" \
 	"s_memtime s[100:101]\n\t" \
 	"s_waitcnt lgkmcnt(0)\n\t" \
 	"v_sub_u32 v127, s100, v126\n\t" \
 	"v_add_u32 v121, v127, v121\n\t" \
-	"v_mov_b32 v126, s100\n\t" \
-	"12:\n" \
-	"ds_read_b64 v[8:9], v6\n\t" \
-	"v_add_u32 v6, 8256, v6\n\t" \
-	"s_waitcnt lgkmcnt(0)\n\t" \
-	"v_cmp_class_f64 vcc, v[8:9], v10\n\t" \
-	"s_or_b32 s18, s18, vcc_lo\n\t" \
-	"s_or_b32 s18, s18, vcc_hi\n\t" \
-	"s_sub_u32 m0, m0, 1\n\t" \
-	"s_cbranch_scc0 12b\n\t" \
-	"s_memtime s[100:101]\n\t" \
-	"s_waitcnt lgkmcnt(0)\n\t" \
-	"v_sub_u32 v127, s100, v126\n\t" \
-	"v_add_u32 v122, v127, v122\n\t" \
 	"v_mov_b32 v126, s100\n\t" \
 	"s_branch 21b\n\t" \
 	"31:\n" \
@@ -2292,6 +2158,21 @@
 	"s_waitcnt lgkmcnt(0)\n\t" \
 	"v_sub_u32 v127, s100, v126\n\t" \
 	"v_add_u32 v117, v127, v117\n\t" \
+	"v_mov_b32 v126, s100\n\t" \
+	"s_mov_b32 m0, s19\n\t" \
+	"12:\n" \
+	"ds_read_b64 v[8:9], v6\n\t" \
+	"v_add_u32 v6, 128, v6\n\t" \
+	"s_waitcnt lgkmcnt(0)\n\t" \
+	"v_cmp_class_f64 vcc, v[8:9], v10\n\t" \
+	"s_or_b32 s18, s18, vcc_lo\n\t" \
+	"s_or_b32 s18, s18, vcc_hi\n\t" \
+	"s_sub_u32 m0, m0, 1\n\t" \
+	"s_cbranch_scc0 12b\n\t" \
+	"s_memtime s[100:101]\n\t" \
+	"s_waitcnt lgkmcnt(0)\n\t" \
+	"v_sub_u32 v127, s100, v126\n\t" \
+	"v_add_u32 v122, v127, v122\n\t" \
 	"v_mov_b32 v126, s100\n\t" \
 	"s_barrier\n\t" \
 	"s_memtime s[100:101]\n\t" \
@@ -2324,25 +2205,11 @@
 	"s_set_gpr_idx_idx s59\n\t" \
 	"v_fma_f64 v[44:45], s[74:75], v[42:43], v[44:45]\n\t" \
 	"s_set_gpr_idx_off\n\t" \
-	"s_mov_b32 m0, s19\n\t" \
+	"s_waitcnt lgkmcnt(0)\n\t" \
 	"s_memtime s[100:101]\n\t" \
 	"s_waitcnt lgkmcnt(0)\n\t" \
 	"v_sub_u32 v127, s100, v126\n\t" \
 	"v_add_u32 v121, v127, v121\n\t" \
-	"v_mov_b32 v126, s100\n\t" \
-	"12:\n" \
-	"ds_read_b64 v[8:9], v6\n\t" \
-	"v_add_u32 v6, 8256, v6\n\t" \
-	"s_waitcnt lgkmcnt(0)\n\t" \
-	"v_cmp_class_f64 vcc, v[8:9], v10\n\t" \
-	"s_or_b32 s18, s18, vcc_lo\n\t" \
-	"s_or_b32 s18, s18, vcc_hi\n\t" \
-	"s_sub_u32 m0, m0, 1\n\t" \
-	"s_cbranch_scc0 12b\n\t" \
-	"s_memtime s[100:101]\n\t" \
-	"s_waitcnt lgkmcnt(0)\n\t" \
-	"v_sub_u32 v127, s100, v126\n\t" \
-	"v_add_u32 v122, v127, v122\n\t" \
 	"v_mov_b32 v126, s100\n\t" \
 	"s_branch 22b\n\t" \
 	"32:\n" \
@@ -2379,6 +2246,21 @@
 	"s_waitcnt lgkmcnt(0)\n\t" \
 	"v_sub_u32 v127, s100, v126\n\t" \
 	"v_add_u32 v117, v127, v117\n\t" \
+	"v_mov_b32 v126, s100\n\t" \
+	"s_mov_b32 m0, s19\n\t" \
+	"12:\n" \
+	"ds_read_b64 v[8:9], v6\n\t" \
+	"v_add_u32 v6, 128, v6\n\t" \
+	"s_waitcnt lgkmcnt(0)\n\t" \
+	"v_cmp_class_f64 vcc, v[8:9], v10\n\t" \
+	"s_or_b32 s18, s18, vcc_lo\n\t" \
+	"s_or_b32 s18, s18, vcc_hi\n\t" \
+	"s_sub_u32 m0, m0, 1\n\t" \
+	"s_cbranch_scc0 12b\n\t" \
+	"s_memtime s[100:101]\n\t" \
+	"s_waitcnt lgkmcnt(0)\n\t" \
+	"v_sub_u32 v127, s100, v126\n\t" \
+	"v_add_u32 v122, v127, v122\n\t" \
 	"v_mov_b32 v126, s100\n\t" \
 	"s_barrier\n\t" \
 	"s_memtime s[100:101]\n\t" \
@@ -2411,25 +2293,11 @@
 	"s_set_gpr_idx_idx s83\n\t" \
 	"v_fma_f64 v[44:45], s[98:99], v[26:27], v[44:45]\n\t" \
 	"s_set_gpr_idx_off\n\t" \
-	"s_mov_b32 m0, s19\n\t" \
+	"s_waitcnt lgkmcnt(0)\n\t" \
 	"s_memtime s[100:101]\n\t" \
 	"s_waitcnt lgkmcnt(0)\n\t" \
 	"v_sub_u32 v127, s100, v126\n\t" \
 	"v_add_u32 v121, v127, v121\n\t" \
-	"v_mov_b32 v126, s100\n\t" \
-	"12:\n" \
-	"ds_read_b64 v[8:9], v6\n\t" \
-	"v_add_u32 v6, 8256, v6\n\t" \
-	"s_waitcnt lgkmcnt(0)\n\t" \
-	"v_cmp_class_f64 vcc, v[8:9], v10\n\t" \
-	"s_or_b32 s18, s18, vcc_lo\n\t" \
-	"s_or_b32 s18, s18, vcc_hi\n\t" \
-	"s_sub_u32 m0, m0, 1\n\t" \
-	"s_cbranch_scc0 12b\n\t" \
-	"s_memtime s[100:101]\n\t" \
-	"s_waitcnt lgkmcnt(0)\n\t" \
-	"v_sub_u32 v127, s100, v126\n\t" \
-	"v_add_u32 v122, v127, v122\n\t" \
 	"v_mov_b32 v126, s100\n\t" \
 	"s_branch 23b\n\t" \
 	"33:\n" \
@@ -2466,6 +2334,21 @@
 	"s_waitcnt lgkmcnt(0)\n\t" \
 	"v_sub_u32 v127, s100, v126\n\t" \
 	"v_add_u32 v117, v127, v117\n\t" \
+	"v_mov_b32 v126, s100\n\t" \
+	"s_mov_b32 m0, s19\n\t" \
+	"12:\n" \
+	"ds_read_b64 v[8:9], v6\n\t" \
+	"v_add_u32 v6, 128, v6\n\t" \
+	"s_waitcnt lgkmcnt(0)\n\t" \
+	"v_cmp_class_f64 vcc, v[8:9], v10\n\t" \
+	"s_or_b32 s18, s18, vcc_lo\n\t" \
+	"s_or_b32 s18, s18, vcc_hi\n\t" \
+	"s_sub_u32 m0, m0, 1\n\t" \
+	"s_cbranch_scc0 12b\n\t" \
+	"s_memtime s[100:101]\n\t" \
+	"s_waitcnt lgkmcnt(0)\n\t" \
+	"v_sub_u32 v127, s100, v126\n\t" \
+	"v_add_u32 v122, v127, v122\n\t" \
 	"v_mov_b32 v126, s100\n\t" \
 	"s_barrier\n\t" \
 	"s_memtime s[100:101]\n\t" \
@@ -2498,25 +2381,11 @@
 	"s_set_gpr_idx_idx s35\n\t" \
 	"v_fma_f64 v[44:45], s[50:51], v[42:43], v[44:45]\n\t" \
 	"s_set_gpr_idx_off\n\t" \
-	"s_mov_b32 m0, s19\n\t" \
+	"s_waitcnt lgkmcnt(0)\n\t" \
 	"s_memtime s[100:101]\n\t" \
 	"s_waitcnt lgkmcnt(0)\n\t" \
 	"v_sub_u32 v127, s100, v126\n\t" \
 	"v_add_u32 v121, v127, v121\n\t" \
-	"v_mov_b32 v126, s100\n\t" \
-	"12:\n" \
-	"ds_read_b64 v[8:9], v6\n\t" \
-	"v_add_u32 v6, 8256, v6\n\t" \
-	"s_waitcnt lgkmcnt(0)\n\t" \
-	"v_cmp_class_f64 vcc, v[8:9], v10\n\t" \
-	"s_or_b32 s18, s18, vcc_lo\n\t" \
-	"s_or_b32 s18, s18, vcc_hi\n\t" \
-	"s_sub_u32 m0, m0, 1\n\t" \
-	"s_cbranch_scc0 12b\n\t" \
-	"s_memtime s[100:101]\n\t" \
-	"s_waitcnt lgkmcnt(0)\n\t" \
-	"v_sub_u32 v127, s100, v126\n\t" \
-	"v_add_u32 v122, v127, v122\n\t" \
 	"v_mov_b32 v126, s100\n\t" \
 	"s_branch 24b\n\t" \
 	"34:\n" \
@@ -2553,6 +2422,21 @@
 	"s_waitcnt lgkmcnt(0)\n\t" \
 	"v_sub_u32 v127, s100, v126\n\t" \
 	"v_add_u32 v117, v127, v117\n\t" \
+	"v_mov_b32 v126, s100\n\t" \
+	"s_mov_b32 m0, s19\n\t" \
+	"12:\n" \
+	"ds_read_b64 v[8:9], v6\n\t" \
+	"v_add_u32 v6, 128, v6\n\t" \
+	"s_waitcnt lgkmcnt(0)\n\t" \
+	"v_cmp_class_f64 vcc, v[8:9], v10\n\t" \
+	"s_or_b32 s18, s18, vcc_lo\n\t" \
+	"s_or_b32 s18, s18, vcc_hi\n\t" \
+	"s_sub_u32 m0, m0, 1\n\t" \
+	"s_cbranch_scc0 12b\n\t" \
+	"s_memtime s[100:101]\n\t" \
+	"s_waitcnt lgkmcnt(0)\n\t" \
+	"v_sub_u32 v127, s100, v126\n\t" \
+	"v_add_u32 v122, v127, v122\n\t" \
 	"v_mov_b32 v126, s100\n\t" \
 	"s_barrier\n\t" \
 	"s_memtime s[100:101]\n\t" \
@@ -2585,25 +2469,11 @@
 	"s_set_gpr_idx_idx s59\n\t" \
 	"v_fma_f64 v[44:45], s[74:75], v[26:27], v[44:45]\n\t" \
 	"s_set_gpr_idx_off\n\t" \
-	"s_mov_b32 m0, s19\n\t" \
+	"s_waitcnt lgkmcnt(0)\n\t" \
 	"s_memtime s[100:101]\n\t" \
 	"s_waitcnt lgkmcnt(0)\n\t" \
 	"v_sub_u32 v127, s100, v126\n\t" \
 	"v_add_u32 v121, v127, v121\n\t" \
-	"v_mov_b32 v126, s100\n\t" \
-	"12:\n" \
-	"ds_read_b64 v[8:9], v6\n\t" \
-	"v_add_u32 v6, 8256, v6\n\t" \
-	"s_waitcnt lgkmcnt(0)\n\t" \
-	"v_cmp_class_f64 vcc, v[8:9], v10\n\t" \
-	"s_or_b32 s18, s18, vcc_lo\n\t" \
-	"s_or_b32 s18, s18, vcc_hi\n\t" \
-	"s_sub_u32 m0, m0, 1\n\t" \
-	"s_cbranch_scc0 12b\n\t" \
-	"s_memtime s[100:101]\n\t" \
-	"s_waitcnt lgkmcnt(0)\n\t" \
-	"v_sub_u32 v127, s100, v126\n\t" \
-	"v_add_u32 v122, v127, v122\n\t" \
 	"v_mov_b32 v126, s100\n\t" \
 	"s_branch 25b\n\t" \
 	"35:\n" \
@@ -2640,6 +2510,21 @@
 	"s_waitcnt lgkmcnt(0)\n\t" \
 	"v_sub_u32 v127, s100, v126\n\t" \
 	"v_add_u32 v117, v127, v117\n\t" \
+	"v_mov_b32 v126, s100\n\t" \
+	"s_mov_b32 m0, s19\n\t" \
+	"12:\n" \
+	"ds_read_b64 v[8:9], v6\n\t" \
+	"v_add_u32 v6, 128, v6\n\t" \
+	"s_waitcnt lgkmcnt(0)\n\t" \
+	"v_cmp_class_f64 vcc, v[8:9], v10\n\t" \
+	"s_or_b32 s18, s18, vcc_lo\n\t" \
+	"s_or_b32 s18, s18, vcc_hi\n\t" \
+	"s_sub_u32 m0, m0, 1\n\t" \
+	"s_cbranch_scc0 12b\n\t" \
+	"s_memtime s[100:101]\n\t" \
+	"s_waitcnt lgkmcnt(0)\n\t" \
+	"v_sub_u32 v127, s100, v126\n\t" \
+	"v_add_u32 v122, v127, v122\n\t" \
 	"v_mov_b32 v126, s100\n\t" \
 	"s_barrier\n\t" \
 	"s_memtime s[100:101]\n\t" \
@@ -2672,25 +2557,11 @@
 	"s_set_gpr_idx_idx s83\n\t" \
 	"v_fma_f64 v[44:45], s[98:99], v[42:43], v[44:45]\n\t" \
 	"s_set_gpr_idx_off\n\t" \
-	"s_mov_b32 m0, s19\n\t" \
+	"s_waitcnt lgkmcnt(0)\n\t" \
 	"s_memtime s[100:101]\n\t" \
 	"s_waitcnt lgkmcnt(0)\n\t" \
 	"v_sub_u32 v127, s100, v126\n\t" \
 	"v_add_u32 v121, v127, v121\n\t" \
-	"v_mov_b32 v126, s100\n\t" \
-	"12:\n" \
-	"ds_read_b64 v[8:9], v6\n\t" \
-	"v_add_u32 v6, 8256, v6\n\t" \
-	"s_waitcnt lgkmcnt(0)\n\t" \
-	"v_cmp_class_f64 vcc, v[8:9], v10\n\t" \
-	"s_or_b32 s18, s18, vcc_lo\n\t" \
-	"s_or_b32 s18, s18, vcc_hi\n\t" \
-	"s_sub_u32 m0, m0, 1\n\t" \
-	"s_cbranch_scc0 12b\n\t" \
-	"s_memtime s[100:101]\n\t" \
-	"s_waitcnt lgkmcnt(0)\n\t" \
-	"v_sub_u32 v127, s100, v126\n\t" \
-	"v_add_u32 v122, v127, v122\n\t" \
 	"v_mov_b32 v126, s100\n\t" \
 	"s_branch 20b\n\t" \
 	"55:\n" \
@@ -2728,6 +2599,21 @@
 	"v_sub_u32 v127, s100, v126\n\t" \
 	"v_add_u32 v117, v127, v117\n\t" \
 	"v_mov_b32 v126, s100\n\t" \
+	"s_mov_b32 m0, s19\n\t" \
+	"12:\n" \
+	"ds_read_b64 v[8:9], v6\n\t" \
+	"v_add_u32 v6, 128, v6\n\t" \
+	"s_waitcnt lgkmcnt(0)\n\t" \
+	"v_cmp_class_f64 vcc, v[8:9], v10\n\t" \
+	"s_or_b32 s18, s18, vcc_lo\n\t" \
+	"s_or_b32 s18, s18, vcc_hi\n\t" \
+	"s_sub_u32 m0, m0, 1\n\t" \
+	"s_cbranch_scc0 12b\n\t" \
+	"s_memtime s[100:101]\n\t" \
+	"s_waitcnt lgkmcnt(0)\n\t" \
+	"v_sub_u32 v127, s100, v126\n\t" \
+	"v_add_u32 v122, v127, v122\n\t" \
+	"v_mov_b32 v126, s100\n\t" \
 	"s_barrier\n\t" \
 	"s_memtime s[100:101]\n\t" \
 	"s_waitcnt lgkmcnt(0)\n\t" \
@@ -2742,25 +2628,11 @@
 	"ds_read_b64 v[22:23], v22\n\t" \
 	"ds_read_b64 v[24:25], v24\n\t" \
 	"ds_read_b64 v[26:27], v26\n\t" \
-	"s_mov_b32 m0, s19\n\t" \
+	"s_waitcnt lgkmcnt(0)\n\t" \
 	"s_memtime s[100:101]\n\t" \
 	"s_waitcnt lgkmcnt(0)\n\t" \
 	"v_sub_u32 v127, s100, v126\n\t" \
 	"v_add_u32 v121, v127, v121\n\t" \
-	"v_mov_b32 v126, s100\n\t" \
-	"12:\n" \
-	"ds_read_b64 v[8:9], v6\n\t" \
-	"v_add_u32 v6, 8256, v6\n\t" \
-	"s_waitcnt lgkmcnt(0)\n\t" \
-	"v_cmp_class_f64 vcc, v[8:9], v10\n\t" \
-	"s_or_b32 s18, s18, vcc_lo\n\t" \
-	"s_or_b32 s18, s18, vcc_hi\n\t" \
-	"s_sub_u32 m0, m0, 1\n\t" \
-	"s_cbranch_scc0 12b\n\t" \
-	"s_memtime s[100:101]\n\t" \
-	"s_waitcnt lgkmcnt(0)\n\t" \
-	"v_sub_u32 v127, s100, v126\n\t" \
-	"v_add_u32 v122, v127, v122\n\t" \
 	"v_mov_b32 v126, s100\n\t" \
 	"s_branch 20b\n\t" \
 	"40:\n" \
```

After: 58.47, median of 6. About the same (+0.9%).
